# wq2012/SpectralCluster

Hardware: AMD Instinct MI355X
Metric: predict() calls/sec, n=8192 d=256 ICASSP2018 (GraphCut, eigengap k in [2,20], cosine k-means) (higher is better)
Workload: dtype f64; 1 GPU; icassp2018_graphcut_n8192_d256_k8_max20; n_samples=8192, n_features=256, parallelism=replicas x1, collectives=none

## Files before the change

### spectralcluster_amd/csrc/api.hip

```cpp
#include <algorithm>
#include <array>
#include <cmath>
#include <cstdio>
#include <cstdlib>
#include <cstring>
#include <vector>

#include <condition_variable>
#include <mutex>
#include <string>
#include <thread>

#include "handle.h"
#include "host_pool.h"

int ensure_matrices(sc_handle h, int n, int d, bool affinity_copy) {
  h->krylov_m = 0;
  const size_t ldn = matrix_ld(n);
  const size_t nn = (size_t)n * ldn * sizeof(double);
  if (affinity_copy) SC_TRY(grow(h, h->A0, nn));
  SC_TRY(grow(h, h->B1, nn));
  SC_TRY(grow(h, h->B2, nn));
  if (d > 0) {
    const size_t ldx = round_up(d, 16);
    SC_TRY(grow(h, h->X, (size_t)n * ldx * sizeof(double)));
    SC_TRY(grow(h, h->Xn, (size_t)n * ldx * sizeof(double)));
  }
  const size_t nv = (size_t)round_up(n, 16) * sizeof(double);
  SC_TRY(grow(h, h->rowmax, nv));
  SC_TRY(grow(h, h->rowsum, nv));
  SC_TRY(grow(h, h->cvec, nv));
  SC_TRY(grow(h, h->pvec, nv));
  SC_TRY(grow(h, h->tvec, nv));
  SC_TRY(grow(h, h->deg, nv));
  SC_TRY(grow(h, h->splitk, gemm_splitk_workspace_bytes()));
  SC_TRY(grow(h, h->dvec, nv));
  SC_TRY(grow(h, h->cut, nv));
  SC_TRY(grow(h, h->cropval, nv));
  SC_TRY(grow(h, h->statp, (size_t)2 * n * gemm_tile_dim(n) * sizeof(double)));
  SC_TRY(grow(h, h->rmpart, (size_t)n * blur_tile_columns(n, 8) * sizeof(double)));
  SC_TRY(grow(h, h->blurw, (2 * SC_MAX_BLUR_RADIUS + 1) * sizeof(double)));
  return SC_OK;
}

int ensure_tilemap(sc_handle h, int n) {
  const int nt = gemm_tile_dim(n);
  if (nt <= kTilemapTableMax) {
    if (!h->tilemap_table.p) {
      std::vector<int2> all, one;
      for (int t = 1; t <= kTilemapTableMax; ++t) {
        h->tilemap_off[t] = (int)all.size();
        gemm_build_sym_tilemap(t, &one);
        all.insert(all.end(), one.begin(), one.end());
      }
      SC_TRY(grow(h, h->tilemap_table, all.size() * sizeof(int2)));
      SC_HIP(h, hipMemcpyAsync(h->tilemap_table.p, all.data(), all.size() * sizeof(int2),
                               hipMemcpyHostToDevice, h->stream));
      SC_HIP(h, hipStreamSynchronize(h->stream));
    }
    h->tilemap_cur = ptr<int2>(h->tilemap_table) + h->tilemap_off[nt];
    return SC_OK;
  }
  if (h->tilemap_nt != nt) {
    std::vector<int2> map;
    gemm_build_sym_tilemap(nt, &map);
    SC_TRY(grow(h, h->tilemap, map.size() * sizeof(int2)));
    SC_HIP(h, hipMemcpyAsync(h->tilemap.p, map.data(), map.size() * sizeof(int2),
                             hipMemcpyHostToDevice, h->stream));
    SC_HIP(h, hipStreamSynchronize(h->stream));
    h->tilemap_nt = nt;
  }
  h->tilemap_cur = ptr<int2>(h->tilemap);
  return SC_OK;
}

int ensure_eig(sc_handle h, int n) {
  const size_t nq = (size_t)n * kLdq * sizeof(double);
  if (h->Q.bytes < nq) h->krylov_m = 0;
  SC_TRY(grow(h, h->Q, nq));
  SC_TRY(grow(h, h->Q2, nq));
  SC_TRY(grow(h, h->Vs, (size_t)n * kEigBlock * sizeof(double)));
  SC_TRY(grow(h, h->W, (size_t)n * kEigBlock * sizeof(double)));
  SC_TRY(grow(h, h->partial, std::max((size_t)kProjBlocks * kLdq * kEigBlock,
                                       lz_partial_doubles(n)) * sizeof(double)));
  SC_TRY(grow(h, h->T, (size_t)kLdq * kLdq * sizeof(double)));
  SC_TRY(grow(h, h->Y, (size_t)kLdq * kLdq * sizeof(double)));
  SC_TRY(grow(h, h->Yt, (size_t)kLdq * kLdq * sizeof(double)));
  SC_TRY(grow(h, h->theta, kLdq * sizeof(double)));
  SC_TRY(grow(h, h->resid, kLdq * sizeof(double)));
  SC_TRY(grow(h, h->G, 256 * sizeof(double)));
  SC_TRY(grow(h, h->Rinv, 256 * sizeof(double)));
  SC_TRY(grow(h, h->Hbuf, (size_t)kLdq * kEigBlock * sizeof(double)));
  SC_TRY(grow(h, h->hsq, 16 * sizeof(double)));
  SC_TRY(grow(h, h->colnorm, (size_t)kProjBlocks * kMaxVectors * sizeof(double)));
  if (h->flags.bytes < 16 * sizeof(int)) {
    SC_TRY(grow(h, h->flags, 16 * sizeof(int)));
    SC_HIP(h, hipMemsetAsync(h->flags.p, 0, 16 * sizeof(int), h->stream));
  }
  SC_TRY(grow(h, h->mvsym, matvec_sym_workspace_doubles(n) * sizeof(double)));
  SC_TRY(ensure_vectors(h, n, kMaxCols));
  return SC_OK;
}

int ensure_vectors(sc_handle h, int n, int cols) {
  cols = std::max(cols, kMaxCols);
  SC_TRY(grow(h, h->E, (size_t)round_up(n, 16) * cols * sizeof(double)));
  SC_TRY(grow(h, h->Eio, (size_t)n * cols * sizeof(double)));
  return SC_OK;
}

int ensure_gen(sc_handle h, int n) {
  const size_t ldv = round_up(n, 16);
  const size_t nv = ldv * sizeof(double);
  SC_TRY(grow(h, h->crvec, nv));
  SC_TRY(grow(h, h->thetai, kLdq * sizeof(double)));
  SC_TRY(grow(h, h->Vre, ldv * kGenMax * sizeof(double)));
  SC_TRY(grow(h, h->Vim, ldv * kGenMax * sizeof(double)));
  SC_TRY(grow(h, h->gpart, (size_t)gen_residual_blocks(n) * 32 * sizeof(double)));
  SC_TRY(grow(h, h->gsrc, 16 * sizeof(int)));
  SC_TRY(grow(h, h->genL, (size_t)kGenMax * kGenMax * sizeof(double)));
  return SC_OK;
}

extern "C" int sc_abi_version(void) { return SC_ABI_VERSION; }
extern "C" int sc_struct_sizes(int* config_bytes, int* diag_bytes) {
  if (config_bytes) *config_bytes = (int)sizeof(sc_config);
  if (diag_bytes) *diag_bytes = (int)sizeof(sc_diag);
  return SC_OK;
}

extern "C" int sc_device_count(void) {
  int c = 0;
  if (hipGetDeviceCount(&c) != hipSuccess) return 0;
  return c;
}

extern "C" int sc_device_info(int device, char* name, int name_len, char* arch,
                              int arch_len, int* compute_units,
                              int64_t* total_mem_bytes) {
  hipDeviceProp_t prop;
  if (hipGetDeviceProperties(&prop, device) != hipSuccess) return SC_ERR_HIP;
  if (name && name_len > 0) snprintf(name, name_len, "%s", prop.name);
  if (arch && arch_len > 0) snprintf(arch, arch_len, "%s", prop.gcnArchName);
  if (compute_units) *compute_units = prop.multiProcessorCount;
  if (total_mem_bytes) *total_mem_bytes = (int64_t)prop.totalGlobalMem;
  return SC_OK;
}


extern "C" int sc_create(int device, sc_handle* out) {
  if (!out) return SC_ERR_INVALID;
  *out = nullptr;
  int count = 0;
  if (hipGetDeviceCount(&count) != hipSuccess || count <= 0) return SC_ERR_HIP;
  if (device < 0 || device >= count) return SC_ERR_INVALID;
  sc_handle h = new sc_handle_s();
  h->device = device;
  if (hipSetDevice(device) != hipSuccess ||
      hipStreamCreateWithFlags(&h->stream, hipStreamNonBlocking) != hipSuccess) {
    delete h;
    return SC_ERR_HIP;
  }
  const unsigned ev_flags = hipEventDisableSystemFence;
  for (int i = 0; i < 48; ++i) {
    if (hipEventCreateWithFlags(&h->ev[i], ev_flags) != hipSuccess) {
      delete h;
      return SC_ERR_HIP;
    }
  }
  if (hipHostMalloc(reinterpret_cast<void**>(&h->h_theta), 3 * kLdq * sizeof(double)) !=
          hipSuccess ||
      hipHostMalloc(reinterpret_cast<void**>(&h->h_flags), 16 * sizeof(int)) !=
          hipSuccess ||
      hipHostMalloc(reinterpret_cast<void**>(&h->h_rr),
                    (2 * kHostRRSingle * kHostRRSingle + 64) * sizeof(double)) != hipSuccess) {
    delete h;
    return SC_ERR_HIP;
  }
  *out = h;
  return SC_OK;
}

extern "C" int sc_destroy(sc_handle h) {
  if (!h) return SC_OK;
  for (sc_handle sub : h->pool) sc_destroy(sub);
  h->pool.clear();
  for (sc_handle sub : h->gslots) sc_destroy(sub);
  h->gslots.clear();
  for (sc_handle sub : h->gshort) sc_destroy(sub);
  h->gshort.clear();
  hipSetDevice(h->device);
  hipStreamSynchronize(h->stream);
  DevBuf* bufs[] = {&h->X,     &h->Xn,    &h->A0,     &h->B1,      &h->B2,    &h->rowmax,
                    &h->rowsum, &h->cvec,  &h->pvec,   &h->tvec,    &h->deg,   &h->blurw, &h->blur_tmp, &h->dvec, &h->cut, &h->rmpart, &h->splitk, &h->tilemap, &h->tilemap_table, &h->cropval, &h->statp, &h->crvec, &h->thetai, &h->Vre, &h->Vim, &h->gpart, &h->gsrc, &h->genL, &h->ahc_size, &h->ahc_chain, &h->ahc_Z, &h->ahc_lab, &h->ahc_cent, &h->fb_part, &h->fb_small, &h->fb_x, &h->fb_cent, &h->fb_int, &h->Cq, &h->Cband, &h->cp[0], &h->cp[1], &h->cp[2], &h->cp[3], &h->cp[4], &h->symflag,
                    &h->Q,     &h->Q2,    &h->Vs,     &h->W,       &h->partial, &h->T,
                    &h->Y,     &h->Yt,    &h->theta,  &h->resid,   &h->G,     &h->Rinv,
                    &h->Hbuf,  &h->hsq,   &h->colnorm, &h->flags,  &h->E,     &h->Ek,   &h->Eio,
                    &h->td_d,  &h->td_e,  &h->td_theta, &h->td_work, &h->td_tau, &h->td_panel, &h->mvsym,
                    &h->kXc,   &h->kxsq,  &h->kclosest, &h->kcand, &h->kenorm, &h->krnd,
                    &h->kcent, &h->klab32, &h->klab64, &h->kinfo, &h->kchain, &h->gkrnd, &h->gpack, &h->gypack, &h->ginfo, &h->glabels, &h->gjtab,
                    &h->kbig, &h->kbigw, &h->fq, &h->ft32, &h->fy1, &h->fR, &h->fscal, &h->fwords, &h->fcand, &h->fY, &h->fsplit, &h->fypart, &h->frpart, &h->fq2part, &h->fmx64, &h->ftau64, &h->fplan, &h->Xalt, &h->Xstage, &h->gneg};
  for (DevBuf* b : bufs)
    if (b->p) hipFree(b->p);
  for (DevBuf& b : h->kgen)
    if (b.p) hipFree(b.p);
  for (int i = 0; i < 48; ++i) hipEventDestroy(h->ev[i]);
  if (h->h_theta) hipHostFree(h->h_theta);
  if (h->h_flags) hipHostFree(h->h_flags);
  if (h->h_rr) hipHostFree(h->h_rr);
  if (h->h_free) hipHostFree(h->h_free);
  if (h->sync_ev) hipEventDestroy(h->sync_ev);
  for (int b = 0; b < kGroupBanks; ++b) {
    if (h->gbank_ev[b]) hipEventDestroy(h->gbank_ev[b]);
    if (h->gbank_stream[b]) hipStreamDestroy(h->gbank_stream[b]);
  }
  if (h->gchain_stream) hipStreamDestroy(h->gchain_stream);
  if (h->copy_stream) hipStreamDestroy(h->copy_stream);
  if (h->gcheck_ev) hipEventDestroy(h->gcheck_ev);
  for (sc_handle lane : h->glanes) sc_destroy(lane);
  h->glanes.clear();
  delete h->gpool;
  if (h->h_gpack) hipHostFree(h->h_gpack);
  if (h->h_gypack) hipHostFree(h->h_gypack);
  if (h->h_gjtab) hipHostFree(h->h_gjtab);
  if (h->h_ginfo) hipHostFree(h->h_ginfo);
  if (h->h_glabels) hipHostFree(h->h_glabels);
  hipStreamDestroy(h->stream);
  delete h;
  return SC_OK;
}

extern "C" const char* sc_last_error(sc_handle h) { return h ? h->err.c_str() : ""; }

extern "C" int sc_synchronize(sc_handle h) {
  if (!h) return SC_ERR_INVALID;
  SC_HIP(h, hipStreamSynchronize(h->stream));
  return SC_OK;
}

extern "C" int sc_reserve(sc_handle h, int n_max, int d_max) {
  if (!h || n_max <= 0 || d_max < 0) return SC_ERR_INVALID;
  SC_HIP(h, hipSetDevice(h->device));
  SC_TRY(ensure_matrices(h, n_max, d_max));
  SC_TRY(ensure_eig(h, n_max));
  SC_TRY(ensure_kmeans(h, n_max));
  return SC_OK;
}

static double numpy_sum_short(const double* a, int n) {
  if (n < 8) {
    double r = 0.0;
    for (int i = 0; i < n; ++i) r += a[i];
    return r;
  }
  double r[8];
  for (int j = 0; j < 8; ++j) r[j] = a[j];
  int i = 8;
  for (; i < n - (n % 8); i += 8)
    for (int j = 0; j < 8; ++j) r[j] += a[i + j];
  double res = ((r[0] + r[1]) + (r[2] + r[3])) + ((r[4] + r[5]) + (r[6] + r[7]));
  for (; i < n; ++i) res += a[i];
  return res;
}

extern "C" int sc_gaussian_weights(double sigma, int32_t* radius, double* weights) {
  if (!radius || !weights || !(sigma >= 0.0)) return SC_ERR_INVALID;
  if (sigma <= 1e-15) {
    *radius = 0;
    weights[0] = 1.0;
    return SC_OK;
  }
  const int r = (int)(4.0 * sigma + 0.5);
  if (r > SC_MAX_BLUR_RADIUS) return SC_ERR_UNSUPPORTED;
  const double s2 = sigma * sigma;
  for (int x = -r; x <= r; ++x) weights[x + r] = std::exp(-0.5 / s2 * (double)(x * x));
  const double sum = numpy_sum_short(weights, 2 * r + 1);
  for (int i = 0; i < 2 * r + 1; ++i) weights[i] /= sum;
  *radius = r;
  return SC_OK;
}

extern "C" int sc_set_blur_weights(sc_handle h, int radius, const double* weights) {
  if (!h) return SC_ERR_INVALID;
  if (radius <= SC_MAX_BLUR_RADIUS || radius > (1 << 20) || !weights)
    return fail(h, SC_ERR_INVALID, "sc_set_blur_weights: radius must exceed 32; weights 2 r + 1");
  h->blur_ext.assign(weights, weights + 2 * (size_t)radius + 1);
  return SC_OK;
}

extern "C" int sc_config_default(sc_config* cfg) {
  if (!cfg) return SC_ERR_INVALID;
  memset(cfg, 0, sizeof(*cfg));
  sc_gaussian_weights(1.0, &cfg->blur_radius, cfg->blur_weights);
  cfg->p_percentile = 0.95;
  cfg->soft_multiplier = 0.01;
  cfg->threshold_type = SC_THRESHOLD_ROW_MAX;
  cfg->symmetrize_type = SC_SYMMETRIZE_MAX;
  cfg->laplacian_type = SC_LAPLACIAN_NONE;
  cfg->stop_eigenvalue = 1e-2;
  cfg->eigengap_type = SC_EIGENGAP_RATIO;
  cfg->max_iter = 300;
  cfg->constraint_name = SC_CONSTRAINT_NONE;
  cfg->integration_type = SC_INTEGRATION_MAX;
  cfg->constraint_alpha = 0.6;
  return SC_OK;
}

void eigengap_core(const double* w, int count, int max_clusters,
                          double stop_eigenvalue, int eigengap_type, int descend,
// ... 214 lines not shown
  launch_normalize_rows(h->stream, ptr<double>(h->X), h->ldx, h->n, h->d,
                        ptr<double>(h->Xn), ptr<int>(h->symflag) + 1);
  h->affinity_from_embeddings = true;
  GemmRowStats rs{2, ptr<double>(h->statp), nullptr, ptr<double>(h->cropval), nullptr};
  h->aff_ev[0] = h->aff_ev[1] = -1;
  if (h->profile_level >= 1) ev_rec(h, &h->aff_ev[0]);
  launch_gemm_nt(h->stream, ptr<double>(h->Xn), h->ldx, ptr<double>(h->Xn), h->ldx,
                 ptr<double>(h->A0), h->ldn, h->n, h->n, h->d, kEpiAffinity, true,
                 ptr<double>(h->splitk), h->tilemap_cur, &rs);
  if (h->profile_level >= 1) ev_rec(h, &h->aff_ev[1]);
  SC_TRY(check_last(h, "affinity launch"));
  h->have_affinity = true;
  h->have_cropval = true;
  h->affinity_symmetric = true;
  h->constraint_applied = false;
  h->n_vec = 0;
  h->sweep_slot.clear();
  return SC_OK;
}

extern "C" int sc_set_affinity(sc_handle h, const double* a, int n) {
  if (!h) return SC_ERR_INVALID;
  if (!a || n <= 0) return fail(h, SC_ERR_INVALID, "affinity must be (n, n)");
  SC_HIP(h, hipSetDevice(h->device));
  SC_TRY(ensure_matrices(h, n, 0));
  h->n = n;
  h->ldn = matrix_ld(n);
  h->have_x = false;
  h->n_vec = 0;
  h->sweep_slot.clear();
  SC_TRY(h2d_matrix(h, a, n, n, ptr<double>(h->A0), h->ldn));
  SC_TRY(device_is_symmetric(h, ptr<double>(h->A0), n, h->ldn, &h->affinity_symmetric));
  h->have_affinity = true;
  h->have_cropval = false;
  h->constraint_applied = false;
  h->affinity_from_embeddings = false;
  return SC_OK;
}


EigRequest make_eig_request(const sc_config* cfg) {
  EigRequest rq;
  rq.descend = (cfg->laplacian_type == SC_LAPLACIAN_NONE ||
                cfg->laplacian_type == SC_LAPLACIAN_AFFINITY);
  rq.max_clusters = cfg->max_clusters;
  rq.min_clusters = cfg->min_clusters;
  rq.stop_eigenvalue = cfg->stop_eigenvalue;
  rq.eigengap_type = cfg->eigengap_type;
  rq.use_stop = rq.descend;
  rq.value_tol = cfg->eig_value_tol > 0 ? cfg->eig_value_tol : 1e-6;
  rq.vector_tol = cfg->eig_vector_tol > 0 ? cfg->eig_vector_tol : 1e-10;
  rq.max_cycles = cfg->eig_max_cycles > 0 ? cfg->eig_max_cycles : (cfg->eig_max_cycles < 0 ? 0 : 40);
  rq.fixed_count = 0;
  return rq;
}

static void resolve_stage_times(sc_handle h, sc_diag* diag) {
  StageEvents& t = h->stage_events;
  if (!t.pending) return;
  t.pending = false;
  if (!diag) return;
  float dms = 0.f;
  for (int i = 0; i < t.n_diffuse; ++i) dms += ev_ms(h, t.diffuse[i][0], t.diffuse[i][1]);
  diag->stage_ms[SC_STAGE_DIFFUSE] = dms;
  diag->stage_ms[SC_STAGE_REFINE] = ev_ms(h, t.begin, t.after_refine) - dms;
  diag->stage_ms[SC_STAGE_SCALING] = ev_ms(h, t.after_refine, t.after_scaling);
  diag->stage_ms[SC_STAGE_EIG] = ev_ms(h, t.after_scaling, t.after_eig);
  if (t.free_path) {
    diag->stage_ms[SC_STAGE_FREE_QUANTIZE] = ev_ms(h, h->free_ev[0], h->free_ev[1]);
    diag->stage_ms[SC_STAGE_FREE_PRODUCT] = ev_ms(h, h->free_ev[1], h->free_ev[2]);
    diag->stage_ms[SC_STAGE_FREE_SCAN] = ev_ms(h, h->free_ev[2], h->free_ev[3]);
    diag->stage_ms[SC_STAGE_FREE_STATS] = ev_ms(h, h->free_ev[3], h->free_ev[4]);
  }
  if (t.fine) {
    diag->stage_ms[SC_STAGE_BLUR] = ev_ms(h, t.blur[0], t.blur[1]);
    diag->stage_ms[SC_STAGE_THRESHOLD_SYM] = ev_ms(h, t.thr[0], t.thr[1]);
    float mv = 0.f;
    for (int i = 0; i < h->n_mv_ev; ++i) mv += ev_ms(h, h->mv_ev[i][0], h->mv_ev[i][1]);
    diag->stage_ms[SC_STAGE_MATVEC] = mv;
  }
}

int eig_ncluster_impl(sc_handle h, const sc_config* cfg, sc_diag* diag, FrontResult* front_only,
                      const FrontResult* resume, bool defer_timing) {
  const int n = h->n, ld = h->ldn;
  hipStream_t s = h->stream;
  const double* cur = ptr<double>(h->A0);
  double* bufs[2] = {ptr<double>(h->B1), ptr<double>(h->B2)};
  int which = 0;
  bool symmetric = h->affinity_symmetric;
  const bool constrain_after = constraint_active(h, cfg, false);
  bool folded_rownorm = false;
  int e_begin, e_after_refine;
  const bool fine = h->profile_level >= 2;
  int eb0 = -1, eb1 = -1, et0 = -1, et1 = -1;
  h->n_mv_ev = 0;
  bool free_path = false;
  const double* amax_of = nullptr;
  const double* digits_of = nullptr;
  float diffuse_ms_events[SC_MAX_OPS][2];
  int n_diffuse = 0;
  ev_rec(h, &e_begin);
  const bool blur_fast = (cfg->blur_radius == 4 || cfg->blur_radius == 8) && n >= 128;
  const double* pending_diag = nullptr;
  bool have_partials = false;
  bool have_row_stats = false;
  if (resume) {
    cur = resume->matrix;
    symmetric = resume->symmetric;
    folded_rownorm = resume->folded_rownorm;
    which = resume->scratch == bufs[0] ? 0 : 1;
    if (resume->free_op) h->free_checked = false;
  }
  for (int i = 0; i < (resume ? 0 : cfg->n_ops); ++i) {
    const int op = cfg->ops[i];
    const int next = i + 1 < cfg->n_ops ? cfg->ops[i + 1] : 0;
    const int next2 = i + 2 < cfg->n_ops ? cfg->ops[i + 2] : 0;
    const bool thr_sym_fusable = true;
    const bool partials_usable = cfg->threshold_type == SC_THRESHOLD_ROW_MAX &&
                                 !cfg->preserve_diagonal;
    if (op == SC_OP_ROW_WISE_NORMALIZE && symmetric && i == cfg->n_ops - 1 &&
        !constrain_after) {
      folded_rownorm = true;
      continue;
    }
    if (op == SC_OP_CROP_DIAGONAL && next == SC_OP_GAUSSIAN_BLUR && blur_fast) {
      if (cur == ptr<double>(h->A0) && h->have_cropval) {
        pending_diag = ptr<double>(h->cropval);
      } else {
        launch_crop_value(s, cur, n, ld, ptr<double>(h->dvec));
        pending_diag = ptr<double>(h->dvec);
      }
      have_partials = false;
      continue;
    }
    double* out = bufs[which];
    which ^= 1;
    int e0 = -1, e1 = -1;
    bool keep_cur = false;
    if (op == SC_OP_DIFFUSE) ev_rec(h, &e0);
    if (op == SC_OP_GAUSSIAN_BLUR && blur_fast) {
      const bool want = next == SC_OP_ROW_WISE_THRESHOLD && next2 == SC_OP_SYMMETRIZE &&
                        partials_usable;
      SC_TRY(upload_blur_weights(h, cfg));
      if (fine) ev_rec(h, &eb0);
      have_partials = launch_gaussian_blur_fused(s, cur, out, n, ld, cfg->blur_radius,
                                                 ptr<double>(h->blurw), pending_diag,
                                                 want ? ptr<double>(h->rmpart) : nullptr);
      if (fine) ev_rec(h, &eb1);
      pending_diag = nullptr;
      SC_TRY(check_last(h, "blur launch"));
    } else if (op == SC_OP_ROW_WISE_THRESHOLD && next == SC_OP_SYMMETRIZE && thr_sym_fusable) {
      if (cfg->threshold_type == SC_THRESHOLD_PERCENTILE)
        launch_cut_percentile(s, cur, n, ld, cfg->p_percentile, ptr<double>(h->cut),
                              cfg->preserve_diagonal);
      else if (have_partials && partials_usable)
        launch_cut_from_partials(s, ptr<double>(h->rmpart), n,
                                 blur_tile_columns(n, cfg->blur_radius),
                                 cfg->p_percentile, ptr<double>(h->cut));
      else
        launch_cut_from_rows(s, cur, n, ld, cfg->p_percentile, ptr<double>(h->cut),
                             cfg->preserve_diagonal);
      const bool amax_known =
          cfg->threshold_type == SC_THRESHOLD_ROW_MAX && h->affinity_from_embeddings &&
          !h->constraint_applied && cfg->p_percentile > 0.0 && cfg->soft_multiplier >= 0.0 &&
          cfg->soft_multiplier <= 1.0 && i + 2 < cfg->n_ops && cfg->ops[i + 2] == SC_OP_DIFFUSE &&
          free_diffuse_wanted(h, cfg, n, make_eig_request(cfg));
      const bool fuse_digits =
          amax_known && !constrain_after && !front_only &&
          (i + 2 == cfg->n_ops - 1 ||
           (i + 2 == cfg->n_ops - 2 && cfg->ops[i + 3] == SC_OP_ROW_WISE_NORMALIZE));
      const double amax_floor = (cfg->binarize || cfg->preserve_diagonal) ? 1.0 : 0.0;
      if (fuse_digits)
        SC_TRY(free_fused_prepare(h, s, n, ptr<double>(h->cut), cfg->p_percentile, amax_floor));
      if (fine) ev_rec(h, &et0);
      if (fuse_digits)
        launch_threshold_symmetrize_digits(s, cur, out, n, ld, ptr<double>(h->cut),
                                           cfg->soft_multiplier, cfg->binarize,
                                           cfg->symmetrize_type, cfg->preserve_diagonal,
                                           ptr<signed char>(h->fq), ptr<double>(h->fscal),
                                           ptr<double>(h->fypart), ptr<int>(h->frpart),
                                           ptr<double>(h->fq2part), ptr<double>(h->fmx64));
      else
        launch_threshold_symmetrize(s, cur, out, n, ld, ptr<double>(h->cut),
                                    cfg->soft_multiplier, cfg->binarize, cfg->symmetrize_type,
                                    cfg->preserve_diagonal);
      if (fine) ev_rec(h, &et1);
      SC_TRY(check_last(h, "threshold+symmetrize launch"));
      if (fuse_digits) {
        amax_of = out;
        digits_of = out;
      } else if (amax_known) {
        SC_TRY(ensure_free(h, n));
        launch_free_amax_from_cut(s, ptr<double>(h->cut), n, cfg->p_percentile, amax_floor,
                                  ptr<double>(h->fscal));
        amax_of = out;
      }
      have_partials = false;
      cur = out;
      symmetric = true;
      ++i;
      continue;
    } else if (op == SC_OP_DIFFUSE && symmetric && !constrain_after && !front_only &&
               cur != ptr<double>(h->A0) &&
               (i == cfg->n_ops - 1 || (i == cfg->n_ops - 2 && next == SC_OP_ROW_WISE_NORMALIZE)) &&
               free_diffuse_wanted(h, cfg, n, make_eig_request(cfg))) {
      SC_TRY(ensure_eig(h, n));
      SC_TRY(free_diffuse_stats(h, cur, ld, n, amax_of == cur, digits_of == cur));
      free_path = true;
      have_row_stats = true;
      have_partials = false;
      keep_cur = true;
      which ^= 1;
    } else if (op == SC_OP_DIFFUSE) {
      const bool last = i == cfg->n_ops - 1 ||
                        (i == cfg->n_ops - 2 && next == SC_OP_ROW_WISE_NORMALIZE);
      GemmRowStats rs{1, ptr<double>(h->statp), ptr<double>(h->statp) + (size_t)n * gemm_tile_dim(n),
                      ptr<double>(h->rowmax), ptr<double>(h->rowsum)};
      SC_TRY(ensure_tilemap(h, n));
      launch_gemm_nt(s, cur, ld, cur, ld, out, ld, n, n, n, kEpiNone, true,
                     ptr<double>(h->splitk), h->tilemap_cur, last ? &rs : nullptr);
      SC_TRY(check_last(h, "diffuse launch"));
      have_row_stats = last;
      have_partials = false;
    } else {
      SC_TRY(run_refine_op(h, op, cfg, cur, out, n, ld));
      have_partials = false;
    }
    if (op == SC_OP_DIFFUSE) {
      ev_rec(h, &e1);
      diffuse_ms_events[n_diffuse][0] = (float)e0;
      diffuse_ms_events[n_diffuse][1] = (float)e1;
      ++n_diffuse;
    }
    if (!keep_cur) cur = out;
    switch (op) {
      case SC_OP_CROP_DIAGONAL:
      case SC_OP_GAUSSIAN_BLUR:
        break;
      case SC_OP_ROW_WISE_THRESHOLD:
      case SC_OP_ROW_WISE_NORMALIZE:
        symmetric = false;
        break;
      case SC_OP_SYMMETRIZE:
      case SC_OP_DIFFUSE:
        symmetric = true;
        break;
    }
  }
  if (constrain_after && !resume) {
    if (h->qn != n)
      return fail(h, SC_ERR_INVALID,
                  "affinity and constraint matrix must have the same shape");
    double* out = bufs[which];
    which ^= 1;
    SC_TRY(adjust_affinity(h, cfg, cur, symmetric, out, n, ld));
    cur = out;
    symmetric = symmetric && h->constraint_symmetric;
    have_row_stats = false;
  }
  ev_rec(h, &e_after_refine);
  bool flags_by_kernel = false;
  if (resume) {
    SC_TRY(ensure_eig(h, n));
  } else if (!symmetric) {
    SC_TRY(ensure_gen(h, n));
    launch_row_stats(s, cur, n, ld, ptr<double>(h->rowmax), ptr<double>(h->deg));
    launch_scaling_general(s, ptr<double>(h->deg), n, cfg->laplacian_type,
                           ptr<double>(h->cvec), ptr<double>(h->crvec), ptr<double>(h->pvec));
  } else {
    if (!have_row_stats)
      launch_row_stats(s, cur, n, ld, ptr<double>(h->rowmax), ptr<double>(h->rowsum));
    SC_TRY(ensure_eig(h, n));
    launch_scaling_vectors(s, ptr<double>(h->rowmax), ptr<double>(h->rowsum), n,
                           cfg->laplacian_type, folded_rownorm ? 1 : 0, ptr<double>(h->cvec),
                           ptr<double>(h->pvec), ptr<double>(h->tvec), ptr<int>(h->flags),
                           h->affinity_from_embeddings ? ptr<int>(h->symflag) : nullptr);
    flags_by_kernel = true;
  }
  SC_TRY(ensure_eig(h, n));
  if (flags_by_kernel) {
  } else if (h->affinity_from_embeddings)
    SC_HIP(h, hipMemcpyAsync(ptr<int>(h->flags) + 12, ptr<int>(h->symflag) + 1, sizeof(int),
                             hipMemcpyDeviceToDevice, s));
  else
    SC_HIP(h, hipMemsetAsync(ptr<int>(h->flags) + 12, 0, sizeof(int), s));
  launch_check_finite(s, ptr<double>(h->cvec), ptr<double>(h->pvec), n, ptr<int>(h->flags) + 12);
  if (front_only && !flags_by_kernel)
    SC_HIP(h, hipMemsetAsync(ptr<int>(h->flags) + 13, 0, 3 * sizeof(int), s));
  SC_TRY(check_last(h, "scaling launch"));
  if (sw::eig_trace() > 2 && symmetric) {
    std::vector<double> rm(n), rs(n);
    hipMemcpyAsync(rm.data(), h->rowmax.p, n * sizeof(double), hipMemcpyDeviceToHost, s);
    hipMemcpyAsync(rs.data(), h->rowsum.p, n * sizeof(double), hipMemcpyDeviceToHost, s);
    hipStreamSynchronize(s);
    int imin = 0, imax = 0;
    for (int i = 0; i < n; ++i) {
      if (rm[i] < rm[imin]) imin = i;
      if (rm[i] > rm[imax]) imax = i;
    }
    fprintf(stderr, "[sc] scaling: fused stats %d; rowmax min %.6g at %d, max %.6g at %d; "
            "rowsum[%d] %.6g\n", (int)have_row_stats, rm[imin], imin, rm[imax], imax, imin,
            rs[imin]);
  }
  int e_after_scaling;
  ev_rec(h, &e_after_scaling);
  FrontResult op;
  op.matrix = cur;
  op.scratch = bufs[which];
  op.ld = ld;
  op.symmetric = symmetric;
  op.folded_rownorm = folded_rownorm;
  op.free_op = free_path || (resume && resume->free_op);
  op.laplacian_type = cfg->laplacian_type;
  op.chain_flags_cleared = flags_by_kernel;
  op.skip_fused = resume && resume->skip_fused;
  if (front_only) {
    *front_only = op;
    return SC_OK;
  }
  EigRequest rq = make_eig_request(cfg);
  EigDecision dc;
  std::vector<double> w;
  if (symmetric) {
    SC_TRY(sym_topk(h, op, n, rq, diag, &dc, &w));
  } else {
    rq.decision_aware = 1;
    SC_TRY(gen_topk(h, cur, ld, n, cfg->laplacian_type, rq, diag, &dc, &w, bufs[which]));
  }
  int e_after_eig;
  ev_rec(h, &e_after_eig);
  h->last_w = w;
  if (diag) {
    diag->n = n;
    diag->n_clusters_raw = dc.n_clusters_raw;
    diag->max_delta = dc.max_delta;
    diag->eig_descending = rq.descend;
    diag->n_eigenvalues = std::min((int)w.size(), SC_MAX_EIG);
    for (int i = 0; i < diag->n_eigenvalues; ++i) diag->eigenvalues[i] = w[i];
    diag->symmetry_state = !symmetric ? 3 : (folded_rownorm ? 2 : 1);
    if (!free_path && n_diffuse > 0) diag->diffuse_path = SC_DIFFUSE_PATH_EXPLICIT;
  }
  StageEvents& t = h->stage_events;
  t.pending = true;
  t.begin = e_begin;
  t.after_refine = e_after_refine;
  t.after_scaling = e_after_scaling;
  t.after_eig = e_after_eig;
  t.n_diffuse = n_diffuse;
  for (int i = 0; i < n_diffuse; ++i) {
    t.diffuse[i][0] = (int)diffuse_ms_events[i][0];
    t.diffuse[i][1] = (int)diffuse_ms_events[i][1];
  }
  t.fine = fine;
  t.free_path = free_path;
  t.blur[0] = eb0;
  t.blur[1] = eb1;
  t.thr[0] = et0;
  t.thr[1] = et1;
  if (defer_timing) return SC_OK;
  SC_HIP(h, hipStreamSynchronize(s));
  resolve_stage_times(h, diag);
  return SC_OK;
}

extern "C" int sc_eig_ncluster(sc_handle h, const sc_config* cfg, sc_diag* diag) {
  if (!h) return SC_ERR_INVALID;
  SC_TRY(validate_config(h, cfg));
  if (!h->have_affinity) return fail(h, SC_ERR_INVALID, "no affinity resident");
  SC_HIP(h, hipSetDevice(h->device));
  h->nev = 0;
  if (diag) memset(diag, 0, sizeof(*diag));
  return eig_ncluster_impl(h, cfg, diag, nullptr);
}

extern "C" int sc_num_eigenvectors(sc_handle h) { return h ? h->n_vec : 0; }

extern "C" int sc_num_eigenvalues(sc_handle h) { return h ? (int)h->last_w.size() : 0; }

extern "C" int sc_get_eigenvalues(sc_handle h, double* out, int count) {
  if (!h || !out) return SC_ERR_INVALID;
  if (count < 0 || count > (int)h->last_w.size())
    return fail(h, SC_ERR_INVALID, "eigenvalue request out of range");
  for (int i = 0; i < count; ++i) out[i] = h->last_w[i];
  return SC_OK;
}

extern "C" int sc_get_eigenvectors(sc_handle h, double* out, int n, int ncols) {
  if (!h || !out) return SC_ERR_INVALID;
  if (n != h->n || ncols <= 0 || ncols > h->n_vec)
    return fail(h, SC_ERR_INVALID, "eigenvector request out of range");
  SC_HIP(h, hipSetDevice(h->device));
  launch_colmajor_to_rowmajor(h->stream, ptr<double>(h->E), round_up(n, 16), n, ncols,
                              ptr<double>(h->Eio), ncols);
  return d2h_matrix(h, ptr<double>(h->Eio), ncols, n, ncols, out);
}

extern "C" int sc_run_resident(sc_handle h, const sc_config* cfg, int64_t* labels,
                               sc_diag* diag) {
  if (!h) return SC_ERR_INVALID;
  SC_TRY(validate_config(h, cfg));
  if (!labels) return fail(h, SC_ERR_INVALID, "labels is NULL");
  if (!h->have_x) return fail(h, SC_ERR_INVALID, "no embeddings resident");
  SC_HIP(h, hipSetDevice(h->device));
  sc_diag local;
  sc_diag* dg = diag ? diag : &local;
  memset(dg, 0, sizeof(*dg));
  h->nev = 0;
  int e0, e1, e2;
  ev_rec(h, &e0);
  SC_TRY(sc_compute_affinity(h));
  if (constraint_active(h, cfg, true)) SC_TRY(sc_apply_constraint(h, cfg));
  ev_rec(h, &e1);
  SC_TRY(eig_ncluster_impl(h, cfg, dg, nullptr, nullptr, true));
  int k = dg->n_clusters_raw;
  if (cfg->min_clusters > 0 && k < cfg->min_clusters) k = cfg->min_clusters;
  const int rc_cluster = sc_cluster(h, cfg, k, labels, dg);
  if (rc_cluster != SC_OK) {
    h->stage_events.pending = false;
    return rc_cluster;
  }
  ev_rec(h, &e2);
  SC_HIP(h, hipStreamSynchronize(h->stream));
  resolve_stage_times(h, dg);
  dg->stage_ms[SC_STAGE_AFFINITY] = ev_ms(h, e0, e1);
  dg->stage_ms[SC_STAGE_TOTAL] = ev_ms(h, e0, e2);
  if (h->profile_level >= 1)
    dg->stage_ms[SC_STAGE_AFFINITY_GEMM] = ev_ms(h, h->aff_ev[0], h->aff_ev[1]);
  return SC_OK;
}

extern "C" int sc_set_profiling(sc_handle h, int level) {
  if (!h || level < 0 || level > 2) return SC_ERR_INVALID;
  h->profile_level = level;
  return SC_OK;
}

std::vector<sc_array> host_f64_arrays(const double* const* xs, const int* ns, int d, int count) {
  std::vector<sc_array> arrays(std::max(count, 0));
  for (int i = 0; i < count; ++i) arrays[i] = host_f64_array(xs[i], ns[i], d);
  return arrays;
}

int predict_sequence(sc_handle h, const int* idx, int count, const sc_array* xs,
                     const int* ns, int d, const sc_config* cfg, int64_t* const* labels,
                     sc_diag* diags) {
  auto at = [&](int k) { return idx ? idx[k] : k; };
  auto one_call = [&](int i) -> int {
    SC_TRY(validate_config(h, cfg));
    SC_HIP(h, hipSetDevice(h->device));
    h->sweep_slot.clear();
    SC_TRY(ingest_embeddings(h, xs[i], xs[i].location == SC_MEM_HOST));
    return sc_run_resident(h, cfg, labels[i], diags ? diags + i : nullptr);
  };
  int nmax = 0;
  size_t smallest = ~(size_t)0;
  bool prefetchable = true;
  for (int k = 0; k < count; ++k) {
    const int i = at(k);
    if (!xs[i].data || ns[i] <= 0 || d <= 0) { smallest = 0; continue; }
    nmax = std::max(nmax, ns[i]);
    smallest = std::min(smallest, (size_t)ns[i] * d * sizeof(double));
    prefetchable = prefetchable && array_is_host_f64_rows(xs[i]);
  }
  if (nmax > 0) SC_TRY(sc_reserve(h, nmax, d));
  if (count < 2 || smallest < ((size_t)256 << 10) || !prefetchable) {
    for (int k = 0; k < count; ++k) SC_TRY(one_call(at(k)));
    return SC_OK;
  }
  SC_TRY(validate_config(h, cfg));
  SC_HIP(h, hipSetDevice(h->device));
  const size_t ldx = round_up(d, 16);
  SC_TRY(grow(h, h->Xalt, (size_t)nmax * ldx * sizeof(double)));
  SC_TRY(grow(h, h->X, (size_t)nmax * ldx * sizeof(double)));
  if (!h->copy_stream)
    SC_HIP(h, hipStreamCreateWithFlags(&h->copy_stream, hipStreamNonBlocking));
  const DevBuf slot[2] = {h->X, h->Xalt};
  std::mutex mu;
  std::condition_variable cv;
  int uploaded = 0;
  int finished = 0;
  bool stop = false;
  hipError_t upload_err = hipSuccess;
  auto upload_loop = [&]() {
    hipSetDevice(h->device);
    for (int k = 0; k < count; ++k) {
      {
        std::unique_lock<std::mutex> lock(mu);
        cv.wait(lock, [&] { return stop || finished >= k - 1; });
        if (stop) return;
      }
      const int i = at(k);
      hipError_t e = hipMemcpy2DAsync(slot[k & 1].p, ldx * sizeof(double), xs[i].data,
                                      (size_t)(ns[i] == 1 ? d : xs[i].row_stride) * sizeof(double),
                                      (size_t)d * sizeof(double), ns[i], hipMemcpyHostToDevice,
                                      h->copy_stream);
      if (e == hipSuccess) e = hipStreamSynchronize(h->copy_stream);
// ... 328 lines not shown
```

### spectralcluster_amd/csrc/eig.hip

```cpp
#include <algorithm>
#include <cstring>
#include <mutex>

#include "sc_internal.h"

namespace sc {

typedef double v4f64 __attribute__((ext_vector_type(4)));
constexpr int B = kEigBlock;
constexpr int RB = 256 / B;
static_assert(B == 8 || B == 16, "block width must divide the 16-wide MFMA tile");

__device__ __forceinline__ uint64_t splitmix64(uint64_t x) {
  x += 0x9E3779B97F4A7C15ull;
  x = (x ^ (x >> 30)) * 0xBF58476D1CE4E5B9ull;
  x = (x ^ (x >> 27)) * 0x94D049BB133111EBull;
  return x ^ (x >> 31);
}
__device__ __forceinline__ double hash_uniform(uint64_t seed, uint64_t idx) {
  const uint64_t h = splitmix64(seed ^ splitmix64(idx));
  return (double)(h >> 11) * (2.0 / 9007199254740992.0) - 1.0;
}

__global__ void k_random_block(double* W, int n, uint64_t seed) {
// ... 527 lines not shown
  double* Ql = smem;
  double* Hl = Ql + ROWS * mq;
  double* Rl = Hl + kLdq * B;
  double* Wl = Rl + B * B;
  double* Gs = Wl + ROWS * B;
  double* hs = Gs + B * B;
  const int tid = threadIdx.x;
  const int j = tid % B;
  const int r0 = blockIdx.x * ROWS;
  const bool first_wg = blockIdx.x == 0;
  const bool pre_proj = (a.pre >= 1 && a.pre <= 3) && m > 0;
  const bool pre_gram = a.pre >= 2;
  const bool use_h = pre_proj;
  const bool use_r = pre_gram;
  const bool use_q = m > 0 && (use_h || a.want_proj);
  const int nproj = pre_proj ? m * B : 0;
  double hsum[3] = {0.0, 0.0, 0.0};
#pragma unroll
  for (int u = 0; u < 3; ++u) {
    const int e = tid + u * kLzThreads;
    if (e < nproj) hsum[u] = lz_ordered_sum(a.pre_partial + e, a.pre_nparts);
    else if (pre_gram && e < nproj + B * B)
      hsum[u] = lz_ordered_sum(a.pre_partial + kLdq * B + (e - nproj), a.pre_nparts);
  }
  double told[3] = {0.0, 0.0, 0.0};
  double hsq_old = 0.0;
  if (first_wg && a.pre == 2) {
#pragma unroll
    for (int u = 0; u < 3; ++u) {
      const int e = tid + u * kLzThreads;
      if (e < nproj) told[u] = a.T[(size_t)(e / B) * a.ldt + a.col0 + (e % B)];
    }
    if (tid < B) hsq_old = a.hsq[tid];
  }
  if (!first_wg && a.pre == 2 && tid < B) hsq_old = a.hsq[tid];
  if (use_q)
    for (int e = tid; e < ROWS * m; e += kLzThreads) {
      const int rr = e / m, i = e - rr * m;
      Ql[rr * mq + i] = (r0 + rr < a.n) ? a.Q[(size_t)(r0 + rr) * a.ldq + i] : 0.0;
    }
  double w[ROWS / kPass];
#pragma unroll
  for (int q = 0; q < ROWS / kPass; ++q) {
    const int r = r0 + q * kPass + tid / B;
    w[q] = 0.0;
    if (r < a.n)
      w[q] = a.init_random ? hash_uniform(a.seed, (uint64_t)r * B + j) : a.W[(size_t)r * B + j];
  }
#pragma unroll
  for (int u = 0; u < 3; ++u) {
    const int e = tid + u * kLzThreads;
    if (e < nproj) Hl[e] = hsum[u];
    else if (pre_gram && e < nproj + B * B) Gs[e - nproj] = hsum[u];
  }
  if (tid < B * B) Rl[tid] = (tid / B == tid % B) ? 1.0 : 0.0;
  __syncthreads();
  if (pre_proj && a.pre != 3) {
    if (first_wg && a.T != nullptr) {
#pragma unroll
      for (int u = 0; u < 3; ++u) {
        const int e = tid + u * kLzThreads;
        if (e < nproj) {
          const int i = e / B, jc = a.col0 + (e % B);
          if (i <= jc) {
            const double t = a.pre == 2 ? told[u] + hsum[u] : hsum[u];
            a.T[(size_t)i * a.ldt + jc] = t;
            a.T[(size_t)jc * a.ldt + i] = t;
          }
        }
      }
    }
    if (tid < B) {
      double sq = 0.0;
      for (int i = 0; i < m; ++i) sq = __builtin_fma(Hl[i * B + tid], Hl[i * B + tid], sq);
      sq = a.pre == 2 ? hsq_old + sq : sq;
      if (first_wg && a.pre == 1) a.hsq[tid] = sq;
      hs[tid] = sq;
    }
  } else if (tid < B) {
    hs[tid] = 0.0;
  }
  if (first_wg && a.Tzero != nullptr)
    for (int e = tid; e < kLdq * kLdq; e += kLzThreads) a.Tzero[e] = 0.0;
  if (pre_gram) {
    if (pre_proj && tid < B * B) {
      const int a1 = tid / B, b1 = tid % B;
      double g = Gs[tid];
      for (int i = 0; i < m; ++i) g = __builtin_fma(-Hl[i * B + a1], Hl[i * B + b1], g);
      Gs[tid] = g;
    }
    __syncthreads();
    if (first_wg && a.pre == 2 && a.Gsave != nullptr && tid < B * B) a.Gsave[tid] = Gs[tid];
    if (tid < 64)
      chol8_wave(Gs, Rl, a.pre == 2 ? hs : nullptr, first_wg ? a.flags : nullptr,
                 first_wg ? a.flags + (a.pre == 3 ? 10 : 11) : nullptr, a.pre == 3 ? 2 : 1,
                 first_wg ? a.flags + 13 : nullptr, m, a.arm_defect != 0);
    __syncthreads();
  }
#pragma unroll
  for (int q = 0; q < ROWS / kPass; ++q) {
    const int rl = q * kPass + tid / B;
    const int r = r0 + rl;
    double x = w[q];
    if (use_h)
      for (int i = 0; i < m; ++i) x = __builtin_fma(-Ql[rl * mq + i], Hl[i * B + j], x);
    double v = x;
    if (use_r) {
      v = 0.0;
#pragma unroll
      for (int k = 0; k < B; ++k) v = __builtin_fma(__shfl(x, k, B), Rl[k * B + j], v);
    }
    if (r < a.n) {
      a.W[(size_t)r * B + j] = v;
      if (a.Qdst) a.Qdst[(size_t)r * a.ldq + a.store_col + j] = v;
      if (a.Vs) a.Vs[(size_t)r * B + j] = a.vs_scale[r] * v;
    }
    Wl[rl * B + j] = (r < a.n) ? v : 0.0;
  }
  if (!a.want_proj && !a.want_gram) return;
  __syncthreads();
  const int oproj = a.want_proj ? m * B : 0;
  const int nent = oproj + (a.want_gram ? B * B : 0);
  double* mine = a.partial + (size_t)blockIdx.x * kLzPartStride;
  for (int base = 0; base < nent; base += kLzThreads / 2) {
    const int e = base + (tid >> 1), half = tid & 1;
    double acc = 0.0;
    if (e < nent) {
      const int rbeg = half * (ROWS / 2);
      if (e < oproj) {
        const int i = e / B, jj = e % B;
#pragma unroll 8
        for (int rr = 0; rr < ROWS / 2; ++rr)
          acc = __builtin_fma(Ql[(rbeg + rr) * mq + i], Wl[(rbeg + rr) * B + jj], acc);
      } else {
        const int g = e - oproj, a1 = g / B, b1 = g % B;
#pragma unroll 8
        for (int rr = 0; rr < ROWS / 2; ++rr)
          acc = __builtin_fma(Wl[(rbeg + rr) * B + a1], Wl[(rbeg + rr) * B + b1], acc);
      }
    }
    const double other = __shfl_xor(acc, 1);
    if (e < nent && half == 0)
      mine[e < oproj ? e : kLdq * B + (e - oproj)] = acc + other;
  }
}
template <int ROWS>
__global__ __launch_bounds__(kLzThreads) void k_lz_rows(const LzStep a) {
  lz_rows_body<ROWS>(a);
}
template <int ROWS>
__global__ __launch_bounds__(kLzThreads) void k_lz_rows_g(const GroupOf<LzStep> g) {
  const LzStep& a = g.s[blockIdx.y];
  if ((int)blockIdx.x * ROWS >= a.n) return;
  lz_rows_body<ROWS>(a);
}

__device__ __forceinline__ double fast_rcp(double x) {
  double r = __builtin_amdgcn_rcp(x);
  r = __builtin_fma(r, __builtin_fma(-x, r, 1.0), r);
  r = __builtin_fma(r, __builtin_fma(-x, r, 1.0), r);
  return r;
}
__device__ __forceinline__ double fast_rsqrt(double x) {
  double y = __builtin_amdgcn_rsq(x);
  y = __builtin_fma(y, 0.5 * __builtin_fma(-x * y, y, 1.0), y);
  y = __builtin_fma(y, 0.5 * __builtin_fma(-x * y, y, 1.0), y);
// ... 670 lines not shown
```

### spectralcluster_amd/csrc/eig_driver.hip

```cpp
#include <ctime>

#include "handle.h"
#include "host_eig.h"
#include "host_pool.h"


static double value_error_bound(const double* theta, const double* resid, int m, int i,
                                bool symmetric) {
  const double r = resid[i];
  if (!symmetric || !(r > 0.0) || !std::isfinite(r)) return r;
  double delta = __builtin_huge_val();
  if (i > 0) delta = std::min(delta, theta[i - 1] - resid[i - 1] - theta[i]);
  if (i + 1 < m) delta = std::min(delta, theta[i] - theta[i + 1] - resid[i + 1]);
  else return r;
  delta -= r;
  if (!(delta > 0.0) || !std::isfinite(delta)) return r;
  return std::min(r, 2.0 * r * r / delta);
}

extern "C" int sc_host_value_error_bound(const double* theta, const double* resid, int m, int i,
                                         double* bound) {
  if (!theta || !resid || !bound || m < 1 || i < 0 || i >= m) return SC_ERR_INVALID;
  *bound = value_error_bound(theta, resid, m, i, true);
  return SC_OK;
// ... 274 lines not shown

static int dense_spectrum(sc_handle h, const double* S, int ld, int n, double* scratch) {
  hipStream_t s = h->stream;
  if (scratch == nullptr || scratch == S)
    return fail(h, SC_ERR_UNSUPPORTED, "no scratch matrix for the dense eigenvalue path");
  SC_TRY(grow(h, h->td_d, (size_t)n * sizeof(double)));
  SC_TRY(grow(h, h->td_e, (size_t)n * sizeof(double)));
  SC_TRY(grow(h, h->td_theta, (size_t)n * sizeof(double)));
  SC_TRY(grow(h, h->td_work, (size_t)(5 * (size_t)n + 2048) * sizeof(double)));
  SC_TRY(grow(h, h->td_tau, (size_t)n * sizeof(double)));
  SC_TRY(grow(h, h->td_panel, (size_t)n * 128 * sizeof(double)));
  launch_td_materialize(s, S, ld, n, ptr<double>(h->cvec), ptr<double>(h->pvec), scratch);
  launch_tridiagonalize_blocked(s, scratch, ld, n, ptr<double>(h->td_d), ptr<double>(h->td_e),
                                ptr<double>(h->td_tau), ptr<double>(h->td_panel),
                                ptr<double>(h->td_work), ptr<double>(h->splitk));
  launch_tridiagonal_eigenvalues(s, ptr<double>(h->td_d), ptr<double>(h->td_e), n,
                                 ptr<double>(h->td_theta), ptr<double>(h->td_work));
  SC_TRY(check_last(h, "dense eigenvalue launch"));
  h->spectrum.resize(n);
  SC_HIP(h, hipMemcpyAsync(h->spectrum.data(), h->td_theta.p, (size_t)n * sizeof(double),
                           hipMemcpyDeviceToHost, s));
  SC_HIP(h, hipMemcpyAsync(h->h_flags + 12, ptr<int>(h->flags) + 12, sizeof(int),
                           hipMemcpyDeviceToHost, s));
  SC_HIP(h, hipStreamSynchronize(s));
  if (h->h_flags[12] != 0) return fail(h, SC_ERR_NON_FINITE, kNonFiniteMessage);
  for (int i = 0; i < n; ++i)
    if (!std::isfinite(h->spectrum[i])) return fail(h, SC_ERR_NON_FINITE, kNonFiniteMessage);
  return SC_OK;
}

static int dense_vectors(sc_handle h, const double* scratch, int ld, int n, int cols) {
  hipStream_t s = h->stream;
  if (cols < 1 || cols > n)
    return fail(h, SC_ERR_UNSUPPORTED, "dense eigenvector request out of range");
  SC_TRY(ensure_vectors(h, n, cols));
  std::vector<double> de(2 * (size_t)n);
  SC_HIP(h, hipMemcpyAsync(de.data(), h->td_d.p, (size_t)n * sizeof(double),
                           hipMemcpyDeviceToHost, s));
  SC_HIP(h, hipMemcpyAsync(de.data() + n, h->td_e.p, (size_t)n * sizeof(double),
                           hipMemcpyDeviceToHost, s));
  SC_HIP(h, hipStreamSynchronize(s));
  const int lde = round_up(n, 16);
  std::vector<double> z((size_t)lde * cols, 0.0);
  if (!host_tridiag_eigvectors(de.data(), de.data() + n, n, h->spectrum.data(), cols, z.data(),
                               (size_t)lde))
    return fail(h, SC_ERR_NOT_CONVERGED, "inverse iteration on the tridiagonal form failed");
  SC_HIP(h, hipMemcpyAsync(h->E.p, z.data(), z.size() * sizeof(double), hipMemcpyHostToDevice,
                           s));
  launch_td_backtransform(s, scratch, ld, n, ptr<double>(h->td_tau), ptr<double>(h->E), lde,
                          cols);
  back_transform_cols(h, n, cols);
  SC_TRY(check_last(h, "dense eigenvector launch"));
  SC_HIP(h, hipStreamSynchronize(s));
  h->n_vec = cols;
  return SC_OK;
}

bool wants_full_spectrum(const EigRequest& rq) {
  if (rq.fixed_count > 0 || rq.descend) return false;
  return rq.max_clusters == 0 || rq.eigengap_type == SC_EIGENGAP_NORMALIZED_DIFF;
}

static EigWorkspace eig_workspace(sc_handle h) {
  EigWorkspace ws;
  ws.Q = ptr<double>(h->Q);
  ws.Q2 = ptr<double>(h->Q2);
  ws.Vs = ptr<double>(h->Vs);
  ws.W = ptr<double>(h->W);
  ws.partial = ptr<double>(h->partial);
  ws.T = ptr<double>(h->T);
  ws.Y = ptr<double>(h->Y);
  ws.theta = ptr<double>(h->theta);
  ws.resid = ptr<double>(h->resid);
  ws.G = ptr<double>(h->G);
  ws.Rinv = ptr<double>(h->Rinv);
  ws.Hbuf = ptr<double>(h->Hbuf);
  ws.hsq = ptr<double>(h->hsq);
  ws.Yt = ptr<double>(h->Yt);
  ws.colnorm = ptr<double>(h->colnorm);
  ws.flags = ptr<int>(h->flags);
  return ws;
}

int sym_topk(sc_handle h, const FrontResult& op_in, int n, const EigRequest& rq_in,
             sc_diag* diag, EigDecision* out_dc, std::vector<double>* out_w) {
  hipStream_t s = h->stream;
  h->krylov_m = 0;
  SC_TRY(ensure_eig(h, n));
  FrontResult op = op_in;
  const int ld = op.ld;
  auto free_materialize = [&](bool with_stats) -> int {
    if (!op.free_op) return SC_OK;
    if (op.scratch == nullptr || op.scratch == op.matrix)
      return fail(h, SC_ERR_UNSUPPORTED, "no scratch matrix to form the Diffuse product in");
    SC_TRY(ensure_tilemap(h, n));
    GemmRowStats rs{1, ptr<double>(h->statp), ptr<double>(h->statp) + (size_t)n * gemm_tile_dim(n),
                    ptr<double>(h->rowmax), ptr<double>(h->rowsum)};
    launch_gemm_nt(s, op.matrix, ld, op.matrix, ld, op.scratch, ld, n, n, n, kEpiNone, true,
                   ptr<double>(h->splitk), h->tilemap_cur, with_stats ? &rs : nullptr);
    SC_TRY(check_last(h, "diffuse launch"));
    double* a_buffer = const_cast<double*>(op.matrix);
    op.matrix = op.scratch;
    op.scratch = a_buffer;
    op.free_op = false;
    return SC_OK;
  };
  auto free_check = [&](bool* restart) -> int {
    *restart = false;
    if (!op.free_op || h->free_checked) return SC_OK;
    bool changed = false, too_many = false;
    SC_TRY(free_fix_overflow(h, op.matrix, ld, n, &changed, &too_many));
    if (too_many) {
      SC_TRY(free_materialize(true));
      changed = true;
    }
    if (changed) {
      launch_scaling_vectors(s, ptr<double>(h->rowmax), ptr<double>(h->rowsum), n,
                             op.laplacian_type, op.folded_rownorm ? 1 : 0, ptr<double>(h->cvec),
                             ptr<double>(h->pvec), ptr<double>(h->tvec));
      launch_check_finite(s, ptr<double>(h->cvec), ptr<double>(h->pvec), n, ptr<int>(h->flags) + 12);
      SC_TRY(check_last(h, "scaling launch"));
      *restart = true;
    }
    return SC_OK;
  };
  double* theta_d = ptr<double>(h->theta);
  double* resid_d = ptr<double>(h->resid);
  const double* cvec = ptr<double>(h->cvec);
  const double* pvec = ptr<double>(h->pvec);
  EigDecision dc;
  int m = 0, passes = 0, cycles = 0;
  EigRequest rq = rq_in;
  bool fused = !sw::eig_host_chain() && !op.skip_fused;
  bool three_pass = false;
  const int sym_min_n = sw::matvec_sym_min_n();
  const bool sym_mv = n >= sym_min_n;
  EigDecision dense_dc;
  bool dense = false, many_vectors = false;
  auto run_dense = [&]() -> int {
    bool unused = false;
    SC_TRY(free_check(&unused));
    SC_TRY(free_materialize(false));
    SC_TRY(dense_spectrum(h, op.matrix, ld, n, op.scratch));
    std::vector<double> zeros(n, 0.0);
    dense_dc = analyze(rq_in, h->spectrum.data(), zeros.data(), n, n, true);
    if (!dense_dc.enough) return fail(h, SC_ERR_UNSUPPORTED, "eigen request cannot be satisfied");
    many_vectors = dense_dc.kvec > kMaxVectors;
    dense = true;
    rq = rq_in;
    rq.fixed_count = std::max(1, dense_dc.kvec);
    rq.value_tol = std::max(rq_in.value_tol, 1e-6);
    return SC_OK;
  };
  if (n > kDenseMax && wants_full_spectrum(rq_in)) SC_TRY(run_dense());
  bool vectors_from_dense = false;
  int fallback_reason = 0;
  auto dense_fallback = [&](int reason) -> int {
    if (op.scratch == nullptr || op.scratch == op.matrix)
      return fail(h, SC_ERR_NOT_CONVERGED,
                  "block Lanczos did not converge and no scratch matrix is free for the dense path");
    if (sw::eig_trace())
      fprintf(stderr, "[sc] block Lanczos gave up (reason %d, %d passes): dense path\n", reason,
              passes);
    if (!dense) SC_TRY(run_dense());
    SC_TRY(free_materialize(false));
    int cols = dense_dc.kvec;
    if (rq_in.fixed_count > 0 || rq_in.max_clusters > 0)
      cols = std::max(std::min(dense_dc.kw, kMaxVectors), cols);
    cols = std::max(1, cols);
    SC_TRY(dense_vectors(h, op.scratch, ld, n, cols));
    vectors_from_dense = true;
    fallback_reason = reason;
    return SC_OK;
  };

  if (n <= kDenseMax) {
    launch_jacobi(s, op.matrix, ld, n, 1, cvec, pvec, nullptr, theta_d, ptr<double>(h->Y), kLdq,
                  nullptr, ptr<double>(h->Yt), ptr<int>(h->flags));
    SC_TRY(check_last(h, "jacobi launch"));
    SC_HIP(h, hipMemcpyAsync(h->h_theta, theta_d, n * sizeof(double), hipMemcpyDeviceToHost, s));
    SC_HIP(h, hipMemcpyAsync(h->h_flags + 12, ptr<int>(h->flags) + 12, sizeof(int),
                             hipMemcpyDeviceToHost, s));
    if (sw::eig_trace())
      SC_HIP(h, hipMemcpyAsync(h->h_flags + 1, ptr<int>(h->flags) + 1, 7 * sizeof(int),
                               hipMemcpyDeviceToHost, s));
    SC_HIP(h, hipStreamSynchronize(s));
    if (h->h_flags[12] != 0) return fail(h, SC_ERR_NON_FINITE, kNonFiniteMessage);
    trace_jacobi(h);
    for (int i = 0; i < n; ++i) h->h_theta[kLdq + i] = 0.0;
    dc = analyze(rq, h->h_theta, h->h_theta + kLdq, n, n, true);
    if (!dc.enough) return fail(h, SC_ERR_UNSUPPORTED, "eigen request cannot be satisfied");
    m = n;
    const int cols = n;
    launch_rowmajor_to_colmajor(s, ptr<double>(h->Y), kLdq, n, cols, ptr<double>(h->E),
                                round_up(n, 16));
    back_transform_cols(h, n, cols);
    h->n_vec = cols;
    if (diag) diag->eig_path = SC_EIG_PATH_DENSE_JACOBI;
    dc.kw = n;
  } else {
  restart_lanczos:
    m = 0;
    cycles = 0;
    bool done = false;
    uint64_t seed = 0x5eed5eedull;
    LzChain chain;
    if (dense && many_vectors) {
      SC_TRY(dense_fallback(5));
      done = true;
    }
    if (done) {
    } else if (fused) {
      if (!op.chain_flags_cleared)
        SC_HIP(h, hipMemsetAsync(ptr<int>(h->flags) + 13, 0, 3 * sizeof(int), s));
      op.chain_flags_cleared = false;
      const EigWorkspace ws = eig_workspace(h);
      chain = LzChain();
      chain.three_pass = three_pass;
      launch_lz_link(s, ws, &chain, n, 0, 0, 4, -1, cvec, 0, true, seed, false);
      launch_lz_link(s, ws, &chain, n, 0, 4, 3, -1, cvec, 0, false, 0, true);
      launch_lz_link(s, ws, &chain, n, 0, 3, 0, 0, cvec, 0, false, 0, false);
      SC_TRY(check_last(h, "start block launch"));
    } else {
      launch_random_block(s, ptr<double>(h->W), n, seed);
      SC_TRY(orthonormalize(h, n, 0, false, 0, 0, false, cvec));
      const int rc0 = finish_block(h, n, 0, 0, cvec, &seed);
      if (rc0 == SC_ERR_NOT_CONVERGED) {
        SC_TRY(dense_fallback(3));
        done = true;
      } else {
        SC_TRY(rc0);
      }
      SC_HIP(h, hipMemsetAsync(h->T.p, 0, (size_t)kLdq * kLdq * sizeof(double), s));
    }
    if (!done && sw::eig_force_dense()) {
      SC_TRY(dense_fallback(4));
      done = true;
    }
    const int cap = std::min(kEigBasisCap, ((n - kEigBlock) / kEigBlock) * kEigBlock);
    const int first_check = std::min(3 * kEigBlock, cap);
    auto check_due = [&](int mm) {
      return cycles == 0 ? (mm >= first_check && (mm <= 4 * kEigBlock ||
                                                  mm % (2 * kEigBlock) == 0 || mm + kEigBlock > cap))
                         : (mm + kEigBlock > cap);
    };
    auto enqueue_step = [&](int m_before) -> int {
      const bool time_mv = h->profile_level >= 2 && h->n_mv_ev < 16;
      if (time_mv) ev_rec(h, &h->mv_ev[h->n_mv_ev][0]);
      if (op.free_op)
        free_apply_operator(h, op.matrix, ld, n, sym_mv, ptr<double>(h->Q) + m_before, kLdq);
      else if (sym_mv)
        launch_block_matvec_sym(s, op.matrix, ld, n, cvec, pvec, ptr<double>(h->Q) + m_before, kLdq,
                                ptr<double>(h->Vs), ptr<double>(h->W), ptr<double>(h->mvsym));
      else
        launch_block_matvec(s, op.matrix, ld, n, cvec, pvec, ptr<double>(h->Q) + m_before, kLdq,
                            ptr<double>(h->Vs), ptr<double>(h->W));
      if (time_mv) ev_rec(h, &h->mv_ev[h->n_mv_ev++][1]);
      ++passes;
      const int mm = m_before + kEigBlock;
      if (fused) {
        const EigWorkspace ws = eig_workspace(h);
        launch_lz_link(s, ws, &chain, n, mm, 0, 1, -1, cvec, mm - kEigBlock, false, 0, false);
        launch_lz_link(s, ws, &chain, n, mm, 1, 2, -1, cvec, mm - kEigBlock, false, 0, false);
        launch_lz_link(s, ws, &chain, n, mm, 2, 3, -1, cvec, mm - kEigBlock, false, 0, false);
        if (three_pass) launch_lz_link(s, ws, &chain, n, mm, 3, 3, -1, cvec, 0, false, 0, false);
        launch_lz_link(s, ws, &chain, n, mm, 3, 0, mm, cvec, 0, false, 0, false);
        return check_last(h, "block step launch");
      }
      return orthonormalize(h, n, mm, true, mm - kEigBlock, mm, true, cvec);
    };
    int ahead = 0;
    while (!done) {
      if (ahead > 0)
        --ahead;
      else
        SC_TRY(enqueue_step(m));
      m += kEigBlock;
      const bool check = check_due(m);
      const bool host_rr = check && m <= kHostRRSingle && !sw::eig_device_rr();
      if (host_rr) {
        SC_HIP(h, hipMemcpy2DAsync(h->h_rr, (size_t)m * sizeof(double), h->T.p,
                                   (size_t)kLdq * sizeof(double), (size_t)m * sizeof(double), m,
                                   hipMemcpyDeviceToHost, s));
        SC_HIP(h, hipMemcpyAsync(h->h_rr + kHostRRSingle * kHostRRSingle, h->G.p,
                                 kEigBlock * kEigBlock * sizeof(double), hipMemcpyDeviceToHost,
                                 s));
      } else if (check) {
        launch_jacobi(s, ptr<double>(h->T), kLdq, m, 0, nullptr, nullptr, ptr<double>(h->G),
                      theta_d, ptr<double>(h->Y), kLdq, resid_d, ptr<double>(h->Yt),
                      ptr<int>(h->flags));
        SC_TRY(check_last(h, "jacobi launch"));
        SC_HIP(h, hipMemcpyAsync(h->h_theta, theta_d, m * sizeof(double),
                                 hipMemcpyDeviceToHost, s));
        SC_HIP(h, hipMemcpyAsync(h->h_theta + kLdq, resid_d, m * sizeof(double),
                                 hipMemcpyDeviceToHost, s));
      }
      if (!fused) {
        const int rcb = finish_block(h, n, m, m, cvec, &seed);
        if (rcb == SC_ERR_NOT_CONVERGED) {
          SC_TRY(dense_fallback(3));
          break;
        }
        SC_TRY(rcb);
      } else if (check) {
        SC_HIP(h, hipMemcpyAsync(h->h_flags, h->flags.p, 16 * sizeof(int), hipMemcpyDeviceToHost, s));
        if (!h->sync_ev) SC_HIP(h, hipEventCreateWithFlags(&h->sync_ev, hipEventDisableTiming));
        SC_HIP(h, hipEventRecord(h->sync_ev, s));
        if (host_rr && cycles == 0 && m >= 6 * kEigBlock && m + kEigBlock <= cap) {
          int mm = m;
          do {
            SC_TRY(enqueue_step(mm));
            mm += kEigBlock;
            ++ahead;
          } while (!check_due(mm));
        }
        SC_HIP(h, hipEventSynchronize(h->sync_ev));
        if (h->h_flags[12] != 0) return fail(h, SC_ERR_NON_FINITE, kNonFiniteMessage);
        if (h->h_flags[13] != 0) {
          passes = 0;
          if (!three_pass && h->h_flags[15] == 2000) {
            if (sw::eig_trace())
              fprintf(stderr, "[sc] fused chain flagged at m=%d: three-pass chain\n",
                      h->h_flags[14]);
            three_pass = true;
            goto restart_lanczos;
          }
          if (sw::eig_trace()) fprintf(stderr, "[sc] fused chain flagged: host chain\n");
          fused = false;
          goto restart_lanczos;
        }
      }
      if (op.free_op && !h->free_checked && (!fused || check)) {
        bool restart = false;
        SC_TRY(free_check(&restart));
        if (restart) {
          if (sw::eig_trace())
            fprintf(stderr, "[sc] matrix-free diffuse: %d rows evaluated in full, restart\n",
                    h->h_free[0]);
          passes = 0;
          goto restart_lanczos;
        }
      }
      if (host_rr) {
        double* hy = h->h_rr + kHostRRSingle * kHostRRSingle + 64;
        const double* hG = h->h_rr + kHostRRSingle * kHostRRSingle;
        bool rr_ok;
        timespec ts0;
        if (sw::eig_trace()) clock_gettime(CLOCK_MONOTONIC, &ts0);
        if (m <= kHostRR) {
          rr_ok = host_rayleigh_ritz(h->h_rr, m, hG, m, h->h_theta, h->h_theta + kLdq, hy, m);
        } else {
          auto leading = [&](const double* theta) {
            std::vector<double> zero(m, 0.0);
            const EigDecision d0 = analyze(rq, theta, zero.data(), m, n, false);
            const int want = d0.enough ? std::max(d0.kw, d0.kvec) : cap / 4;
            return round_up(want + kEigBlock, kEigBlock) + kEigBlock;
          };
          rr_ok = host_rayleigh_ritz_leading(h->h_rr, m, hG, m, h->h_theta, h->h_theta + kLdq,
                                             hy, m, leading);
        }
        if (sw::eig_trace()) {
          timespec ts1;
          clock_gettime(CLOCK_MONOTONIC, &ts1);
          fprintf(stderr, "[sc]   host Rayleigh-Ritz m=%d: %.0f us\n", m,
                  (ts1.tv_sec - ts0.tv_sec) * 1e6 + (ts1.tv_nsec - ts0.tv_nsec) * 1e-3);
        }
        if (!rr_ok) {
          SC_TRY(dense_fallback(2));
          break;
        }
        for (int i = 0; i < m; ++i)
          if (!std::isfinite(h->h_theta[i])) return fail(h, SC_ERR_NON_FINITE, kNonFiniteMessage);
        SC_HIP(h, hipMemcpy2DAsync(h->Y.p, (size_t)kLdq * sizeof(double), hy,
                                   (size_t)m * sizeof(double), (size_t)m * sizeof(double), m,
                                   hipMemcpyHostToDevice, s));
        SC_HIP(h, hipMemcpyAsync(theta_d, h->h_theta, m * sizeof(double),
                                 hipMemcpyHostToDevice, s));
      }
      if (check) {
        dc = analyze(rq, h->h_theta, h->h_theta + kLdq, m, n, false);
        if (sw::eig_trace()) {
          int worst = 0;
          double wr = 0.0;
          for (int i = 0; i < std::min(m, dc.kw > 0 ? dc.kw : m); ++i) {
            const double r = h->h_theta[kLdq + i] / std::max(std::fabs(h->h_theta[i]), 1e-300);
            if (r > wr) { wr = r; worst = i; }
          }
          fprintf(stderr, "[sc] lanczos pass %d m=%d cycle %d: enough=%d conv=%d kw=%d kvec=%d "
                  "fail kind %d at %d (theta %.6g resid %.2e); far end theta=%.6g resid=%.2e\n",
                  passes, m, cycles, dc.enough, dc.converged, dc.kw, dc.kvec, dc.fail_kind,
                  dc.fail_index, dc.fail_index >= 0 ? h->h_theta[dc.fail_index] : 0.0,
                  dc.fail_index >= 0 ? h->h_theta[kLdq + dc.fail_index] : 0.0, h->h_theta[m - 1],
                  h->h_theta[kLdq + m - 1]);
          (void)wr; (void)worst;
        }
        if (dc.unsupported) {
          if (dense) return fail(h, SC_ERR_UNSUPPORTED, "eigen request cannot be satisfied");
          SC_TRY(run_dense());
          goto restart_lanczos;
        }
        if (dc.enough && dc.converged) {
          if (!dense && m < n && block_multiplicity_suspect(rq, dc, h->h_theta, m)) {
            if (sw::eig_trace())
              fprintf(stderr, "[sc] %d equal Ritz values ahead of the decisive gap: dense path\n",
                      kEigBlock);
            SC_TRY(dense_fallback(7));
            break;
          }
          done = true;
          break;
        }
      }
      if (m + kEigBlock > cap) {
        if (++cycles > rq.max_cycles) {
          SC_TRY(dense_fallback(1));
          break;
        }
        int want = dc.enough ? std::max(dc.kw, dc.kvec) : cap / 4;
        int keep = round_up(want + kEigBlock, kEigBlock);
        keep = std::max(kEigBlock, std::min(keep, cap - 2 * kEigBlock));
        launch_basis_times_Y(s, ptr<double>(h->Q), kLdq, m, ptr<double>(h->Y), kLdq, keep,
                             ptr<double>(h->Q2), kLdq, n, 0);
        launch_copy_block(s, ptr<double>(h->Q) + m, kLdq, ptr<double>(h->Q2) + keep, kLdq, n,
                          kEigBlock);
        std::swap(h->Q, h->Q2);
        launch_set_diag_T(s, ptr<double>(h->T), kLdq, kLdq, theta_d, keep);
        SC_TRY(check_last(h, "restart launch"));
        m = keep;
      }
    }
    if (ahead > 0) passes -= ahead;
    if (vectors_from_dense) {
      dc.max_resid = 0.0;
      if (diag) diag->eig_path = SC_EIG_PATH_DENSE_FULL;
    } else {
      const int cols = std::min(std::max(dc.kw, dc.kvec), kMaxVectors);
      launch_basis_times_Y(s, ptr<double>(h->Q), kLdq, m, ptr<double>(h->Y), kLdq, cols,
                           ptr<double>(h->E), round_up(n, 16), n, 1);
      back_transform_cols(h, n, cols);
      SC_TRY(check_last(h, "ritz vector launch"));
      h->n_vec = cols;
      if (diag) diag->eig_path = dense ? SC_EIG_PATH_DENSE_TRIDIAG : SC_EIG_PATH_BLOCK_LANCZOS;
      if (!dense) {
        h->krylov_m = m;
        h->krylov_n = n;
        h->krylov_cycles = cycles;
        h->krylov_ahead = ahead;
        h->krylov_free = op.free_op;
      }
    }
  }
  if (dense) {
    const double vec_resid = dc.max_resid;
    dc = dense_dc;
    dc.converged = true;
    dc.max_resid = vec_resid;
    if (out_w) {
      out_w->resize(n);
      for (int i = 0; i < n; ++i) (*out_w)[i] = rq.descend ? h->spectrum[i] : -h->spectrum[i];
// ... 497 lines not shown
  SC_HIP(h, hipMemsetAsync(h->td_tau.p, 0, (size_t)n * sizeof(double), s));
  launch_hessenberg(s, scratch, ld, n, ptr<double>(h->td_tau), ptr<double>(h->td_work));
  SC_TRY(check_last(h, "Hessenberg reduction launch"));
  std::vector<double> packed((size_t)n * ld), tau(n);
  SC_HIP(h, hipMemcpyAsync(packed.data(), scratch, packed.size() * sizeof(double),
                           hipMemcpyDeviceToHost, s));
  SC_HIP(h, hipMemcpyAsync(tau.data(), h->td_tau.p, (size_t)n * sizeof(double),
                           hipMemcpyDeviceToHost, s));
  SC_HIP(h, hipMemcpyAsync(h->h_flags + 12, ptr<int>(h->flags) + 12, sizeof(int),
                           hipMemcpyDeviceToHost, s));
  SC_HIP(h, hipStreamSynchronize(s));
  if (h->h_flags[12] != 0) return fail(h, SC_ERR_NON_FINITE, kNonFiniteMessage);
  const double t_reduced = sw::eig_trace() ? now_us() : 0.0;
  HostHessenberg hw;
  if (!host_hessenberg_unpack(packed.data(), (size_t)ld, n, tau.data(), &hw))
    return fail(h, SC_ERR_NON_FINITE, kNonFiniteMessage);
  packed.clear();
  packed.shrink_to_fit();
  std::vector<double> wr(n), wi(n);
  if (!host_hessenberg_eigenvalues(hw, wr.data(), wi.data()))
    return fail(h, SC_ERR_NOT_CONVERGED, "QR iteration on the Hessenberg form failed");
  const double t_values = sw::eig_trace() ? now_us() : 0.0;
  const double sign = is_lap ? -1.0 : 1.0;
  std::vector<int> order(n);
  for (int i = 0; i < n; ++i) order[i] = i;
  std::stable_sort(order.begin(), order.end(),
                   [&](int a, int b) { return sign * wr[a] > sign * wr[b]; });
  std::vector<double> theta(n), zeros(n, 0.0);
  for (int i = 0; i < n; ++i) theta[i] = sign * wr[order[i]] * eig_scale;
  EigDecision dc = analyze(rq, theta.data(), zeros.data(), n, n, true, false);
  if (!dc.enough) return fail(h, SC_ERR_UNSUPPORTED, "eigen request cannot be satisfied");
  const int cols = std::max(1, std::min(n, dc.kvec));
  SC_TRY(ensure_vectors(h, n, cols));
  const int ldv = round_up(n, 16);
  SC_TRY(grow(h, h->Vre, (size_t)ldv * std::max(cols, kGenMax) * sizeof(double)));
  SC_TRY(grow(h, h->Vim, (size_t)ldv * std::max(cols, kGenMax) * sizeof(double)));
  std::vector<double> pr(cols), pi(cols), vre((size_t)ldv * cols, 0.0), vim((size_t)ldv * cols, 0.0);
  for (int q = 0; q < cols; ++q) {
    pr[q] = wr[order[q]];
    pi[q] = wi[order[q]];
  }
  double max_resid = 0.0;
  if (!host_hessenberg_vectors(hw, pr.data(), pi.data(), cols, vre.data(), vim.data(), (size_t)ldv,
                               &max_resid))
    return fail(h, SC_ERR_NOT_CONVERGED, "inverse iteration on the Hessenberg form failed");
  SC_HIP(h, hipMemcpyAsync(h->Vre.p, vre.data(), vre.size() * sizeof(double), hipMemcpyHostToDevice, s));
  SC_HIP(h, hipMemcpyAsync(h->Vim.p, vim.data(), vim.size() * sizeof(double), hipMemcpyHostToDevice, s));
  launch_gen_phase(s, ptr<double>(h->Vre), ptr<double>(h->Vim), ldv, n, cols, ptr<double>(h->E), ldv);
  SC_TRY(check_last(h, "eigenvector normalisation launch"));
  SC_HIP(h, hipStreamSynchronize(s));
  if (sw::eig_trace())
    fprintf(stderr, "[sc] dense general route n=%d: Hessenberg reduction (device, incl. the copy "
            "back) %.1f ms, %d eigenvalues by QR (host) %.1f ms, %d eigenvectors by inverse "
            "iteration + back-transform (host) and phase (device) %.1f ms\n", n,
            (t_reduced - t_begin) * 1e-3, n, (t_values - t_reduced) * 1e-3, cols,
            (now_us() - t_values) * 1e-3);
  h->n_vec = cols;
  dc.kw = n;
  dc.converged = true;
  dc.max_resid = max_resid * std::max(hw.norm, 1e-300) * eig_scale;
  if (out_w) {
    out_w->resize(n);
    for (int i = 0; i < n; ++i) (*out_w)[i] = rq.descend ? theta[i] : -theta[i];
  }
  if (diag) {
    diag->eig_path = SC_EIG_PATH_DENSE_HESSENBERG;
    diag->eig_matvec_passes = 0;
    diag->eig_block = kEigBlock;
    diag->eig_basis = n;
    diag->eig_cycles = 0;
    diag->eig_max_residual = dc.max_resid;
    diag->eig_fallback = reason;
  }
  *out_dc = dc;
  return SC_OK;
}

int gen_topk(sc_handle h, const double* M, int ld, int n, int laplacian_type,
                    const EigRequest& rq_in, sc_diag* diag, EigDecision* out_dc,
                    std::vector<double>* out_w, double* scratch) {
  h->krylov_m = 0;
  EigRequest rq = rq_in;
  hipStream_t s = h->stream;
  SC_TRY(ensure_eig(h, n));
  SC_TRY(ensure_gen(h, n));
  double* theta_d = ptr<double>(h->theta);
  double* thetai_d = ptr<double>(h->thetai);
  double* resid_d = ptr<double>(h->resid);
  double* Yre = ptr<double>(h->Y);
  double* Yim = ptr<double>(h->Yt);
  double* Vre = ptr<double>(h->Vre);
  double* Vim = ptr<double>(h->Vim);
  int* info_d = ptr<int>(h->flags) + 8;
  const int ldv = round_up(n, 16);
  double* th = h->h_theta;
  double* thi = h->h_theta + 2 * kLdq;
  EigDecision dc;
  int m = 0, passes = 0, cycles = 0;
  const bool is_lap = laplacian_type >= SC_LAPLACIAN_UNNORMALIZED;
  bool far_end = !rq.descend && rq.eigengap_type == SC_EIGENGAP_NORMALIZED_DIFF &&
                 rq.fixed_count == 0;
  int far_passes = 0, far_cycles = 0;

  auto fetch_ritz = [&](int count) -> int {
    SC_HIP(h, hipMemcpyAsync(th, theta_d, count * sizeof(double), hipMemcpyDeviceToHost, s));
    SC_HIP(h, hipMemcpyAsync(thi, thetai_d, count * sizeof(double), hipMemcpyDeviceToHost, s));
    SC_HIP(h, hipMemcpyAsync(h->h_flags + 8, info_d, 2 * sizeof(int), hipMemcpyDeviceToHost, s));
    SC_HIP(h, hipMemcpyAsync(h->h_flags + 12, ptr<int>(h->flags) + 12, sizeof(int),
                             hipMemcpyDeviceToHost, s));
    SC_HIP(h, hipStreamSynchronize(s));
    if (h->h_flags[12] != 0) return fail(h, SC_ERR_NON_FINITE, kNonFiniteMessage);
    if (h->h_flags[8] != 0)
      return fail(h, SC_ERR_NOT_CONVERGED, "QR iteration of the projected eigenproblem failed");
    return SC_OK;
  };

  if (n <= kGenMax) {
    const double* src = M;
    if (is_lap) {
      launch_laplacian(s, M, ptr<double>(h->genL), n, ld, laplacian_type, ptr<double>(h->deg));
      src = ptr<double>(h->genL);
    }
    launch_gen_eig(s, src, ld, n, is_lap ? -1.0 : 1.0, n, theta_d, thetai_d, Yre, Yim, kLdq,
                   info_d);
    SC_TRY(check_last(h, "dense general eigensolver launch"));
    SC_TRY(fetch_ritz(n));
    for (int i = 0; i < n; ++i) th[kLdq + i] = 0.0;
    dc = analyze(rq, th, th + kLdq, n, n, true, false);
    if (!dc.enough) return fail(h, SC_ERR_UNSUPPORTED, "eigen request cannot be satisfied");
    launch_gen_ritz(s, nullptr, 0, n, n, Yre, Yim, kLdq, n, Vre, Vim, ldv);
    launch_gen_phase(s, Vre, Vim, ldv, n, n, ptr<double>(h->E), ldv);
    SC_TRY(check_last(h, "eigenvector normalisation launch"));
    h->n_vec = n;
    m = n;
    dc.kw = n;
    if (diag) diag->eig_path = SC_EIG_PATH_DENSE_GENERAL;
  } else {
    if (sw::eig_force_dense())
      return gen_dense_large(h, M, ld, n, laplacian_type, rq, diag, out_dc, out_w, scratch, 4);
    if (rq.fixed_count == 0 && n <= sw::gen_dense_max_n())
      return gen_dense_large(h, M, ld, n, laplacian_type, rq, diag, out_dc, out_w, scratch, 8);
    if (rq.fixed_count == 0 && rq.max_clusters == 0 && !rq.descend)
      return gen_dense_large(h, M, ld, n, laplacian_type, rq, diag, out_dc, out_w, scratch, 6);
    if (far_end) {
      EigRequest fr = rq;
      fr.fixed_count = 1;
      fr.descend = 1;
      fr.negate = !rq.negate;
      fr.no_dense = 1;
      fr.decision_aware = 0;
      fr.value_tol = 0.1 * rq.value_tol;
      fr.vector_tol = fr.value_tol;
      fr.max_cycles = std::max(rq.max_cycles, 60);
      EigDecision fdc;
      std::vector<double> fw;
      sc_diag fdiag;
      memset(&fdiag, 0, sizeof(fdiag));
      const int rc_far = gen_topk(h, M, ld, n, laplacian_type, fr, &fdiag, &fdc, &fw, scratch);
      if (rc_far == SC_OK && !fw.empty()) {
        rq.have_far = 1;
        rq.far_value = fw[0];
        far_end = false;
        far_passes = fdiag.eig_matvec_passes;
        far_cycles = fdiag.eig_cycles;
        if (sw::eig_trace())
          fprintf(stderr, "[sc] general eigen path: far end %.12g in %d passes, %d cycles\n",
// ... 216 lines not shown
```

### spectralcluster_amd/csrc/free_api.hip

```cpp
#include <limits>

#include "handle.h"

namespace {
constexpr int kOvfWords = 80;
constexpr int kOvfRowsMax = 64;
}

extern "C" int sc_set_diffuse_mode(sc_handle h, int mode) {
  if (!h || mode < -1 || mode > 2) return SC_ERR_INVALID;
  h->diffuse_mode = mode;
  return SC_OK;
}

extern "C" int sc_set_free_prune(sc_handle h, int on) {
  if (!h || on < -1 || on > 1) return SC_ERR_INVALID;
  h->free_prune = on;
  return SC_OK;
}
static bool free_prune_on(sc_handle h) {
  return h->free_prune >= 0 ? h->free_prune != 0 : !sw::free_no_prune();
}

bool free_diffuse_wanted(sc_handle h, const sc_config* cfg, int n, const EigRequest& rq,
                         bool in_group) {
  const int mode = cfg->diffuse_mode == 1 || cfg->diffuse_mode == 2
                       ? cfg->diffuse_mode
                       : (h->diffuse_mode >= 0 ? h->diffuse_mode : sw::diffuse_mode());
  if (mode == 1) return false;
  if (n <= kDenseMax || n > 65536 || wants_full_spectrum(rq)) return false;
  if (mode == 2) return true;
  return n >= (in_group ? sw::diffuse_free_min_n_group() : sw::diffuse_free_min_n());
}

int ensure_free(sc_handle h, int n) {
  const size_t nv = (size_t)round_up(n, 16) * sizeof(double);
  SC_TRY(grow(h, h->fq, free_q_bytes(n)));
  SC_TRY(grow(h, h->ft32, free_t32_bytes(n)));
  SC_TRY(grow(h, h->fy1, nv));
  SC_TRY(grow(h, h->fR, nv));
  SC_TRY(grow(h, h->fscal, 4 * sizeof(double)));
  SC_TRY(grow(h, h->fwords, ((size_t)2 * n + kOvfWords) * sizeof(int)));
  SC_TRY(grow(h, h->fcand, (size_t)n * free_candidate_cap() * sizeof(int)));
  SC_TRY(grow(h, h->fY, (size_t)n * kEigBlock * sizeof(double)));
  SC_TRY(grow(h, h->fq2part, free_q2part_bytes(n)));
  SC_TRY(grow(h, h->fmx64, free_mx64_bytes(n)));
  SC_TRY(grow(h, h->ftau64, free_tau64_bytes(n)));
  SC_TRY(grow(h, h->fplan, free_plan_bytes(n)));
  if (!h->h_free)
    SC_HIP(h, hipHostMalloc(reinterpret_cast<void**>(&h->h_free), kOvfWords * sizeof(int)));
  return SC_OK;
}

static FreeSegs free_segs(sc_handle h) {
  return FreeSegs{ptr<double>(h->fq2part), ptr<double>(h->fmx64), ptr<float>(h->ftau64)};
}

int free_product(sc_handle h, hipStream_t s, int n) {
  SC_TRY(grow(h, h->fsplit, free_i8_split_bytes_plan()));
  launch_free_tile_flags(s, ptr<double>(h->fmx64), ptr<float>(h->ftau64), n, ptr<int>(h->fplan),
                         free_prune_on(h), ptr<int>(h->fwords));
  launch_gemm_i8_sym(s, ptr<signed char>(h->fq), n, h->tilemap_cur, ptr<float>(h->ft32),
                     ptr<unsigned>(h->fwords), ptr<int>(h->fsplit), ptr<int>(h->fplan));
  return SC_OK;
}

int free_stats_begin(sc_handle h, hipStream_t s, const double* A, int ld, int n, bool have_amax) {
  SC_TRY(ensure_free(h, n));
  SC_HIP(h, hipMemsetAsync(ptr<double>(h->fscal) + (have_amax ? 1 : 0), 0,
                           (have_amax ? 3 : 4) * sizeof(double), s));
  SC_HIP(h, hipMemsetAsync(h->fwords.p, 0, ((size_t)2 * n + kOvfWords) * sizeof(int), s));
  if (!have_amax) launch_free_absmax(s, A, n, ld, ptr<double>(h->fscal));
  launch_free_quantize(s, A, n, ld, ptr<signed char>(h->fq), ptr<double>(h->fscal),
                       ptr<double>(h->fy1), ptr<double>(h->fR), ptr<double>(h->fq2part));
  launch_free_seg_reduce(s, ptr<double>(h->fR), n, free_segs(h));
  return SC_OK;
}
int free_stats_end(sc_handle h, hipStream_t s, const double* A, int ld, int n, bool timed,
                   const int* plan) {
  unsigned* M = ptr<unsigned>(h->fwords);
  int* count = ptr<int>(h->fwords) + n;
  int* ovf = ptr<int>(h->fwords) + 2 * (size_t)n;
  launch_t32_candidates(s, ptr<float>(h->ft32), n, M, ptr<double>(h->fR), ptr<double>(h->fscal),
                        count, ptr<int>(h->fcand), plan);
  if (timed) ev_rec(h, &h->free_ev[3]);
  launch_free_row_stats(s, A, n, ld, ptr<double>(h->fy1), count, ptr<int>(h->fcand),
                        ptr<double>(h->rowmax), ptr<double>(h->rowsum), ovf);
  if (timed) ev_rec(h, &h->free_ev[4]);
  SC_TRY(check_last(h, "matrix-free diffuse launch"));
  SC_HIP(h, hipMemcpyAsync(h->h_free, ovf, kOvfWords * sizeof(int), hipMemcpyDeviceToHost, s));
  h->free_checked = false;
  return SC_OK;
}

int free_group_prepare(sc_handle* hs, const double* const* A, const double* const* cuts,
                       const double* ps, int count, const int* lds, const int* ns, hipStream_t s,
                       double floor_value, FreeItem* items, TsDigits* digits) {
  for (int z = 0; z < count; ++z) {
    sc_handle h = hs[z];
    const int n = ns[z], ld = lds[z];
    SC_TRY(ensure_free(h, n));
    const size_t rows64 = (size_t)round_up(n, 64), nblk = rows64 / 64;
    SC_TRY(grow(h, h->fypart, rows64 * nblk * sizeof(double)));
    SC_TRY(grow(h, h->frpart, rows64 * nblk * sizeof(int)));
    items[z] = FreeItem{A[z], n, ld, ptr<signed char>(h->fq), ptr<float>(h->ft32),
                        ptr<int>(h->fwords), ptr<double>(h->fscal), ptr<double>(h->fy1),
                        ptr<double>(h->fR), ptr<int>(h->fcand), ptr<double>(h->rowmax),
                        ptr<double>(h->rowsum), cuts[z], ps[z]};
    items[z].q2part = ptr<double>(h->fq2part);
    items[z].mx64 = ptr<double>(h->fmx64);
    items[z].tau64 = ptr<float>(h->ftau64);
    items[z].plan = ptr<int>(h->fplan);
    items[z].ypart = ptr<double>(h->fypart);
    items[z].rpart = ptr<int>(h->frpart);
    digits[z] = TsDigits{ptr<signed char>(h->fq), (size_t)2 * rows64, (int)nblk,
                         ptr<double>(h->fscal), ptr<double>(h->fypart), ptr<int>(h->frpart),
                         ptr<double>(h->fq2part), ptr<double>(h->fmx64)};
  }
  launch_free_begin_group(s, items, count, floor_value, true);
  return SC_OK;
}
int free_group_digits(sc_handle* hs, const FreeItem* items, int count, hipStream_t s) {
  launch_free_partials_reduce_group(s, items, count);
  launch_free_tile_flags_group(s, items, count, free_prune_on(hs[0]));
  return SC_OK;
}

int free_group_end(sc_handle* hs, const FreeItem* items, int count, hipStream_t s) {
  launch_free_scan_stats_group(s, items, count);
  SC_TRY(check_last(hs[0], "matrix-free diffuse launch"));
  for (int z = 0; z < count; ++z) {
    sc_handle h = hs[z];
    SC_HIP(h, hipMemcpyAsync(h->h_free, items[z].words + 2 * (size_t)items[z].n,
                             kOvfWords * sizeof(int), hipMemcpyDeviceToHost, s));
    h->free_checked = false;
  }
  return SC_OK;
}

int free_fused_prepare(sc_handle h, hipStream_t s, int n, const double* cut, double p,
                       double floor_value) {
  SC_TRY(ensure_free(h, n));
  const size_t rows64 = (size_t)round_up(n, 64), nblk = rows64 / 64;
  SC_TRY(grow(h, h->fypart, rows64 * nblk * sizeof(double)));
  SC_TRY(grow(h, h->frpart, rows64 * nblk * sizeof(int)));
  FreeItem item{};
  item.n = n;
  item.words = ptr<int>(h->fwords);
  item.scal = ptr<double>(h->fscal);
  item.cut = cut;
  item.p = p;
  launch_free_begin_group(s, &item, 1, floor_value);
  return SC_OK;
}

int free_diffuse_stats(sc_handle h, const double* A, int ld, int n, bool have_amax,
                       bool digits_ready) {
  hipStream_t s = h->stream;
  SC_TRY(ensure_tilemap(h, n));
  ev_rec(h, &h->free_ev[0]);
  if (digits_ready)
    launch_free_partials_reduce(s, ptr<double>(h->fypart), ptr<int>(h->frpart), n,
                                ptr<double>(h->fy1), ptr<double>(h->fR), ptr<double>(h->fscal),
                                free_segs(h));
  else
    SC_TRY(free_stats_begin(h, s, A, ld, n, have_amax));
  ev_rec(h, &h->free_ev[1]);
  SC_TRY(free_product(h, s, n));
  ev_rec(h, &h->free_ev[2]);
  return free_stats_end(h, s, A, ld, n, true, ptr<int>(h->fplan));
}

static void plain_matvec(hipStream_t s, const double* A, int ld, int n, bool sym_mv,
                         const double* Vs, double* W, double* slabs) {
  if (sym_mv)
    launch_block_matvec_sym(s, A, ld, n, nullptr, nullptr, Vs, kEigBlock, Vs, W, slabs);
  else
    launch_block_matvec(s, A, ld, n, nullptr, nullptr, Vs, kEigBlock, Vs, W);
}

int free_fix_overflow(sc_handle h, const double* A, int ld, int n, bool* changed,
                      bool* too_many) {
  *changed = *too_many = false;
  hipStream_t s = h->stream;
  SC_HIP(h, hipStreamSynchronize(s));
  h->free_checked = true;
  const int rows = h->h_free[0];
  if (rows <= 0) return SC_OK;
  if (rows > kOvfRowsMax) {
    *too_many = true;
    return SC_OK;
  }
  SC_TRY(ensure_eig(h, n));
  const bool sym_mv = n >= sw::matvec_sym_min_n();
  const int* ids = ptr<int>(h->fwords) + 2 * (size_t)n + 1;
  for (int r0 = 0; r0 < rows; r0 += kEigBlock) {
    const int nr = std::min(kEigBlock, rows - r0);
    launch_free_gather_rows(s, A, n, ld, ids + r0, nr, ptr<double>(h->Vs));
    plain_matvec(s, A, ld, n, sym_mv, ptr<double>(h->Vs), ptr<double>(h->W),
                 ptr<double>(h->mvsym));
    launch_free_colmax(s, ptr<double>(h->W), n, ids + r0, nr, ptr<double>(h->rowmax));
  }
  SC_TRY(check_last(h, "matrix-free diffuse: exact rows"));
  *changed = true;
  return SC_OK;
}

void free_apply_operator(hipStream_t s, const double* A, int ld, int n, bool sym_mv,
                         const double* cvec, const double* pvec, const double* V, int ldv,
                         const double* Vs, double* fY, double* W, double* slabs) {
  plain_matvec(s, A, ld, n, sym_mv, Vs, fY, slabs);
  if (sym_mv)
    launch_block_matvec_sym(s, A, ld, n, cvec, pvec, V, ldv, fY, W, slabs);
  else
    launch_block_matvec(s, A, ld, n, cvec, pvec, V, ldv, fY, W);
}
void free_apply_operator(sc_handle h, const double* A, int ld, int n, bool sym_mv,
                         const double* V, int ldv) {
  free_apply_operator(h->stream, A, ld, n, sym_mv, ptr<double>(h->cvec), ptr<double>(h->pvec), V,
                      ldv, ptr<double>(h->Vs), ptr<double>(h->fY), ptr<double>(h->W),
                      ptr<double>(h->mvsym));
}

extern "C" int sc_stage_diffuse_rowstats(sc_handle h, const double* a, int n, int mode,
                                         double* rowmax, double* rowsum, int32_t* info) {
  if (!h) return SC_ERR_INVALID;
  if (!a || n <= 0 || !rowmax || !rowsum || (mode != 1 && mode != 2))
    return fail(h, SC_ERR_INVALID, "bad diffuse row statistics request");
  if (mode == 2 && n > 65536) return fail(h, SC_ERR_UNSUPPORTED, "matrix-free diffuse: n <= 65536");
  SC_HIP(h, hipSetDevice(h->device));
  SC_TRY(ensure_matrices(h, n, 0));
  SC_TRY(ensure_eig(h, n));
  SC_TRY(ensure_tilemap(h, n));
  const int ld = matrix_ld(n);
  h->n = n;
  h->ldn = ld;
  h->have_affinity = h->have_cropval = false;
  h->have_x = false;
  h->n_vec = 0;
  h->nev = 0;
  hipStream_t s = h->stream;
  double* A = ptr<double>(h->B2);
  SC_TRY(h2d_matrix(h, a, n, n, A, ld));
  int inf[6] = {0, 0, 0, 0, 0, 0};
  auto explicit_stats = [&]() -> int {
    GemmRowStats rs{1, ptr<double>(h->statp), ptr<double>(h->statp) + (size_t)n * gemm_tile_dim(n),
                    ptr<double>(h->rowmax), ptr<double>(h->rowsum)};
    launch_gemm_nt(s, A, ld, A, ld, ptr<double>(h->B1), ld, n, n, n, kEpiNone, true,
                   ptr<double>(h->splitk), h->tilemap_cur, &rs);
    return check_last(h, "diffuse launch");
  };
  if (mode == 1) {
    SC_TRY(explicit_stats());
  } else {
    SC_TRY(free_diffuse_stats(h, A, ld, n));
    bool changed = false, too_many = false;
    SC_TRY(free_fix_overflow(h, A, ld, n, &changed, &too_many));
    inf[0] = h->h_free[65];
    inf[1] = h->h_free[0];
    inf[2] = h->h_free[66];
    inf[4] = h->h_free[67];
    inf[5] = gemm_tile_dim(n) * (gemm_tile_dim(n) + 1) / 2;
    if (too_many) {
      inf[3] = 1;
      SC_TRY(explicit_stats());
    }
  }
// ... 119 lines not shown
```

### spectralcluster_amd/csrc/handle.h

```cpp
#ifndef SPECTRALCLUSTER_AMD_HANDLE_H_
#define SPECTRALCLUSTER_AMD_HANDLE_H_

#include <algorithm>
#include <array>
#include <cmath>
#include <cstdio>
#include <cstdlib>
#include <cstring>
#include <string>
#include <vector>

#include "sc_internal.h"

using namespace sc;

struct DevBuf {
  void* p = nullptr;
  size_t bytes = 0;
};

constexpr int kKgenBufs = 12;
constexpr int kGroupBanks = 2;
constexpr int kGroupLanes = 3;

struct StageEvents {
  bool pending = false, fine = false, free_path = false;
  int begin = -1, after_refine = -1, after_scaling = -1, after_eig = -1;
  int diffuse[SC_MAX_OPS][2];
  int n_diffuse = 0;
  int blur[2] = {-1, -1}, thr[2] = {-1, -1};
};

struct sc_handle_s {
  int device = 0;
  hipStream_t stream = nullptr;
  std::string err;
  int n = 0, d = 0, ldn = 0, ldx = 0;
  bool have_x = false, have_affinity = false;
  bool have_cropval = false;
  int n_vec = 0;
  DevBuf X, Xn, A0, B1, B2;
  DevBuf Xalt;
  hipStream_t copy_stream = nullptr;
  DevBuf Xstage;
  DevBuf rowmax, rowsum, cvec, pvec, tvec, deg, dvec, cut, rmpart, splitk, tilemap;
  DevBuf cropval, statp;
  DevBuf Cq, cp[5], symflag;
  DevBuf Cband;
  bool have_constraint = false, constraint_symmetric = false, constraint_applied = false;
  bool constraint_banded = false;
  bool affinity_symmetric = true;
  bool affinity_from_embeddings = false;
  int qn = 0;
  int tilemap_nt = 0;
  DevBuf tilemap_table;
  int tilemap_off[65] = {0};
  const int2* tilemap_cur = nullptr;
  DevBuf blurw;
  DevBuf blur_tmp;
  std::vector<double> blur_ext;
  DevBuf Q, Q2, Vs, W, partial, T, Y, Yt, theta, resid, G, Rinv, Hbuf, hsq, colnorm,
      flags;
  DevBuf E, Ek, Eio;
  DevBuf mvsym;
  DevBuf td_d, td_e, td_theta, td_work, td_tau, td_panel;
  std::vector<double> spectrum;
  std::vector<double> last_w;
  DevBuf crvec, thetai, Vre, Vim, gpart, gsrc, genL, gneg;
  DevBuf ahc_size, ahc_chain, ahc_Z, ahc_lab, ahc_cent;
  DevBuf fb_part, fb_small, fb_x, fb_cent, fb_int;
  DevBuf kXc, kxsq, kclosest, kcand, kenorm, krnd, kcent, klab32, klab64, kinfo, kchain;
  DevBuf kbig, kbigw;
  DevBuf kgen[kKgenBufs];
  double* h_theta = nullptr;
  int* h_flags = nullptr;
  double* h_rr = nullptr;
  std::vector<sc_handle_s*> pool;
  std::vector<sc_handle_s*> gslots;
  std::vector<int> sweep_slot;
  std::vector<sc_diag> sweep_diags;
  std::vector<double> sweep_p;
  sc_config sweep_cfg;
  int sweep_n = 0;
  hipEvent_t sync_ev = nullptr;
  DevBuf gkrnd;
  bool gkrnd_ready = false;
  DevBuf gpack, gypack, ginfo, glabels;
  double* h_gpack = nullptr;
  double* h_gypack = nullptr;
  int* h_ginfo = nullptr;
  long long* h_glabels = nullptr;
  size_t h_glabels_count = 0;
  hipEvent_t gcheck_ev = nullptr;
  std::vector<sc_handle_s*> gshort;
  DevBuf gjtab;
  JacobiItem* h_gjtab = nullptr;
  std::vector<int32_t> last_routes;
  int32_t* groutes = nullptr;
  std::vector<sc_handle_s*> glanes;
  class HostPool* gpool = nullptr;
  hipStream_t gbank_stream[kGroupBanks] = {nullptr};
  hipStream_t gchain_stream = nullptr;
  hipEvent_t gbank_ev[kGroupBanks] = {nullptr};
  int gconv_hist[16] = {0};
  int gconv_seen = 0;
  hipEvent_t ev[48];
  int nev = 0;
  StageEvents stage_events;
  int profile_level = 1;
  int mv_ev[16][2];
  int n_mv_ev = 0;
  int aff_ev[2] = {-1, -1};
  int blurw_radius = -1;
  double blurw_host[2 * SC_MAX_BLUR_RADIUS + 1];
  int krnd_k = -1, krnd_trials = -1;
  int kfirst_n = -1, kfirst = 0;
  int diffuse_mode = -1;
  DevBuf fq, ft32, fy1, fR, fscal, fwords, fcand, fY, fsplit, fypart, frpart;
  int free_prune = -1;
  DevBuf fq2part, fmx64, ftau64, fplan;
  int* h_free = nullptr;
  bool free_checked = false;
  int free_ev[5] = {-1, -1, -1, -1, -1};
  int krylov_m = 0, krylov_n = 0, krylov_cycles = 0, krylov_ahead = 0;
  bool krylov_free = false;
};

inline void ev_rec(sc_handle h, int* slot) {
  if (h->nev < 48) {
    hipEventRecord(h->ev[h->nev], h->stream);
    *slot = h->nev++;
  } else {
    *slot = -1;
  }
}
inline float ev_ms(sc_handle h, int a, int b) {
  if (a < 0 || b < 0) return 0.f;
  float ms = 0.f;
  hipEventElapsedTime(&ms, h->ev[a], h->ev[b]);
  return ms;
}

constexpr int kTilemapTableMax = 64;
constexpr int kMaxCols = 128;
inline int matrix_ld(int n) {
  int ld = round_up(n, 16);
  if (ld % 512 == 0) ld += 16;
  return ld;
}


#define SC_HIP(h, call)                                                         \
  do {                                                                          \
    hipError_t e_ = (call);                                                     \
    if (e_ != hipSuccess) {                                                     \
      (h)->err = std::string(#call) + ": " + hipGetErrorString(e_);             \
      return e_ == hipErrorOutOfMemory ? SC_ERR_OOM : SC_ERR_HIP;               \
    }                                                                           \
  } while (0)

#define SC_TRY(expr)                \
  do {                              \
    int rc_ = (expr);               \
    if (rc_ != SC_OK) return rc_;   \
  } while (0)

inline int fail(sc_handle h, int code, const std::string& msg) {
  if (h) h->err = msg;
  return code;
}

inline int grow(sc_handle h, DevBuf& b, size_t bytes) {
  if (b.bytes >= bytes) return SC_OK;
  if (b.p) {
    SC_HIP(h, hipStreamSynchronize(h->stream));
    SC_HIP(h, hipFree(b.p));
    b.p = nullptr;
    b.bytes = 0;
  }
  SC_HIP(h, hipMalloc(&b.p, bytes));
  b.bytes = bytes;
  return SC_OK;
}
template <typename T>
inline T* ptr(const DevBuf& b) {
  return reinterpret_cast<T*>(b.p);
}

int ensure_matrices(sc_handle h, int n, int d, bool affinity_copy = true);

int ensure_tilemap(sc_handle h, int n);
int predict_sequence(sc_handle h, const int* idx, int count, const sc_array* xs,
                     const int* ns, int d, const sc_config* cfg, int64_t* const* labels,
                     sc_diag* diags);
int validate_array(sc_handle h, const sc_array* a);
sc_array host_f64_array(const double* x, int n, int d);
std::vector<sc_array> host_f64_arrays(const double* const* xs, const int* ns, int d, int count);
bool array_is_host_f64_rows(const sc_array& a);
int ingest_embeddings(sc_handle h, const sc_array& a, bool sync, hipStream_t stream = nullptr);
int predict_batch_streams_impl(sc_handle h, const sc_array* xs, const int* ns, int d, int count,
                               const sc_config* cfg, int64_t* const* labels, sc_diag* diags,
                               int streams);
int predict_batch_grouped_impl(sc_handle h, const sc_array* xs, const int* ns, int d, int count,
                               const sc_config* cfg, int64_t* const* labels, sc_diag* diags,
                               int group);

int ensure_eig(sc_handle h, int n);

int ensure_gen(sc_handle h, int n);

int ensure_kmeans(sc_handle h, int n, int k = kMaxVectors);
int ensure_vectors(sc_handle h, int n, int cols);

inline int check_last(sc_handle h, const char* what) {
  hipError_t e = hipGetLastError();
  if (e != hipSuccess) {
    h->err = std::string(what) + ": " + hipGetErrorString(e);
    return SC_ERR_HIP;
  }
  return SC_OK;
}


int h2d_matrix(sc_handle h, const double* src, int rows, int cols, double* dst, int ld);
int d2h_matrix(sc_handle h, const double* src, int ld, int rows, int cols, double* dst);
int validate_config(sc_handle h, const sc_config* cfg);
void eigengap_core(const double* w, int count, int max_clusters, double stop_eigenvalue,
                   int eigengap_type, int descend, double wmax, int* n_clusters,
                   double* max_delta);

struct EigRequest {
  int descend;
  int max_clusters;
  int min_clusters;
  double stop_eigenvalue;
  int eigengap_type;
  int use_stop;
  double value_tol, vector_tol;
  int max_cycles;
  int fixed_count;
  int decision_aware = 0;
  int negate = 0;
  int no_dense = 0;
  int have_far = 0;
  double far_value = 0.0;
};

struct EigDecision {
  bool enough = false;
  bool converged = false;
  int kw = 0;
  int kvec = 0;
  int n_clusters_raw = 0;
  double max_delta = 0.0;
  double max_resid = 0.0;
  bool unsupported = false;
  int fail_kind = 0;
  int fail_index = -1;
};

struct FrontResult {
  const double* matrix = nullptr;
  double* scratch = nullptr;
  int ld = 0;
  bool symmetric = false, folded_rownorm = false;
  bool free_op = false;
  int laplacian_type = 0;
  bool chain_flags_cleared = false;
  bool skip_fused = false;
};
EigRequest make_eig_request(const sc_config* cfg);
int upload_blur_weights(sc_handle h, const sc_config* cfg);
int eig_ncluster_impl(sc_handle h, const sc_config* cfg, sc_diag* diag, FrontResult* front_only,
                      const FrontResult* resume = nullptr, bool defer_timing = false);
void kmeans_seed_constants(int k, double* u_first, int* trials, std::vector<double>* rnd);
KmeansWorkspace kmeans_workspace(sc_handle h);

struct GroupEigMember {
  sc_handle h = nullptr;
  const double* S = nullptr;
  int ld = 0, n = 0;
  EigRequest rq;
  int status = 0;
  EigDecision dc;
  std::vector<double> w;
  int basis = 0, passes = 0;
  bool skip_fused = false;
  bool free_op = false;
};
int sym_topk_group(sc_handle lead, GroupEigMember* mem, int count, bool want_vectors = true);
int dense_topk_group(sc_handle lead, GroupEigMember* mem, int count);
bool sym_group_eligible(int n, const EigRequest& rq, bool any_size = false);

int sym_topk(sc_handle h, const FrontResult& op, int n, const EigRequest& rq, sc_diag* diag,
             EigDecision* out_dc, std::vector<double>* out_w);
int gen_topk(sc_handle h, const double* M, int ld, int n, int laplacian_type,
             const EigRequest& rq, sc_diag* diag, EigDecision* out_dc,
             std::vector<double>* out_w, double* scratch);

bool free_diffuse_wanted(sc_handle h, const sc_config* cfg, int n, const EigRequest& rq,
                         bool in_group = false);
int free_group_prepare(sc_handle* hs, const double* const* A, const double* const* cuts,
                       const double* ps, int count, const int* lds, const int* ns, hipStream_t s,
                       double floor_value, struct FreeItem* items, struct TsDigits* digits);
int free_group_digits(sc_handle* hs, const struct FreeItem* items, int count, hipStream_t s);
int free_group_end(sc_handle* hs, const struct FreeItem* items, int count, hipStream_t s);
int free_fused_prepare(sc_handle h, hipStream_t s, int n, const double* cut, double p,
                       double floor_value);
int free_diffuse_stats(sc_handle h, const double* A, int ld, int n, bool have_amax = false,
                       bool digits_ready = false);
int ensure_free(sc_handle h, int n);
int free_product(sc_handle h, hipStream_t s, int n);
int free_stats_begin(sc_handle h, hipStream_t s, const double* A, int ld, int n, bool have_amax);
int free_stats_end(sc_handle h, hipStream_t s, const double* A, int ld, int n, bool timed,
                   const int* plan = nullptr);
int free_fix_overflow(sc_handle h, const double* A, int ld, int n, bool* changed, bool* too_many);
void free_apply_operator(sc_handle h, const double* A, int ld, int n, bool sym_mv,
                         const double* V, int ldv);
void free_apply_operator(hipStream_t s, const double* A, int ld, int n, bool sym_mv,
                         const double* cvec, const double* pvec, const double* V, int ldv,
                         const double* Vs, double* fY, double* W, double* slabs);
bool wants_full_spectrum(const EigRequest& rq);

int device_is_symmetric(sc_handle h, const double* m, int n, int ld, bool* out);
int adjust_affinity(sc_handle h, const sc_config* cfg, const double* a, bool sym_a, double* out,
                    int n, int ld);
bool constraint_active(sc_handle h, const sc_config* cfg, bool before);
struct CpGroupMember {
  int n = 0, ld = 0;
  double* A = nullptr;
  double *P = nullptr, *T = nullptr, *Pn = nullptr, *Tn = nullptr;
  double *deg = nullptr, *rowmax = nullptr;
  const double* band = nullptr;
  const int2* tilemap = nullptr;
};
int constraint_propagation_group(sc_handle lead, hipStream_t s, const CpGroupMember* mem,
                                 int count, double alpha);
int predict_batch_constrained_impl(sc_handle h, const sc_array* xs, const double* const* bands,
                                   const int* ns, int d, int count, const sc_config* cfg,
                                   int64_t* const* labels, sc_diag* diags, int group);

#endif
```

### spectralcluster_amd/csrc/kmeans_api.hip

```cpp
#include <algorithm>
#include <cmath>
#include <cstdio>
#include <vector>

#include "handle.h"

int ensure_kmeans(sc_handle h, int n, int k) {
  const int cols = std::max(k, kMaxCols), kk = std::max(k, kMaxVectors);
  SC_TRY(grow(h, h->Ek, (size_t)round_up(n, 16) * cols * sizeof(double)));
  SC_TRY(grow(h, h->Eio, (size_t)n * cols * sizeof(double)));
  SC_TRY(grow(h, h->kXc, (size_t)n * kk * sizeof(double)));
  SC_TRY(grow(h, h->kxsq, (size_t)n * sizeof(double)));
  SC_TRY(grow(h, h->kclosest, (size_t)n * sizeof(double)));
  SC_TRY(grow(h, h->kcand, (size_t)(k > kMaxVectors ? 16 : 8) * n * sizeof(double)));
  SC_TRY(grow(h, h->kenorm, (size_t)n * sizeof(double)));
  SC_TRY(grow(h, h->krnd, (size_t)std::max(1024, 16 * kk) * sizeof(double)));
  SC_TRY(grow(h, h->kcent, (size_t)kk * kk * sizeof(double)));
  if (k > kMaxVectors) {
    SC_TRY(grow(h, h->kbig, kmeans_big_workspace_doubles(k) * sizeof(double)));
    SC_TRY(grow(h, h->kbigw, (size_t)3 * k * sizeof(int)));
  }
  SC_TRY(grow(h, h->klab32, (size_t)n * sizeof(int)));
  SC_TRY(grow(h, h->klab64, (size_t)n * sizeof(long long)));
  SC_TRY(grow(h, h->kinfo, 16 * sizeof(int)));
  SC_TRY(grow(h, h->kchain, kmeans_chain_workspace_doubles(n) * sizeof(double)));
  return SC_OK;
}

KmeansWorkspace kmeans_workspace(sc_handle h) {
  KmeansWorkspace ws;
  ws.Xc = ptr<double>(h->kXc);
  ws.xsq = ptr<double>(h->kxsq);
  ws.closest = ptr<double>(h->kclosest);
  ws.cand = ptr<double>(h->kcand);
  ws.enorm = ptr<double>(h->kenorm);
  ws.rnd = ptr<double>(h->krnd);
  ws.centroids = ptr<double>(h->kcent);
  ws.labels32 = ptr<int>(h->klab32);
  ws.labels64 = ptr<long long>(h->klab64);
  ws.info = ptr<int>(h->kinfo);
  ws.chain = ptr<double>(h->kchain);
  ws.big = ptr<double>(h->kbig);
  ws.big_words = ptr<int>(h->kbigw);
  return ws;
}

enum { kgX, kgIo, kgRow, kgVec, kgCd, kgPart, kgRnd, kgLab32, kgLab64, kgInt, kgCount };
static_assert(kgCount <= kKgenBufs, "handle.h kgen buffers");

static int ensure_kmeans_general(sc_handle h, int n, int dim, int k, int trials,
                                 KmeansGeneralWorkspace* ws) {
  constexpr int TS = kKgenTrialSlots;
  const size_t ld = round_up(n, 16);
  SC_TRY(grow(h, h->kgen[kgX], ld * dim * sizeof(double)));
  SC_TRY(grow(h, h->kgen[kgIo], (size_t)n * dim * sizeof(double)));
  SC_TRY(grow(h, h->kgen[kgRow], 4 * ld * sizeof(double)));
  SC_TRY(grow(h, h->kgen[kgVec],
              ((size_t)dim * (1 + k + TS) + 2 * (size_t)k + TS + kKgenScalars) * sizeof(double)));
  SC_TRY(grow(h, h->kgen[kgCd], 2 * (size_t)TS * n * sizeof(double)));
  SC_TRY(grow(h, h->kgen[kgPart], (size_t)kmeans_general_grid(n) * TS * sizeof(double)));
  SC_TRY(grow(h, h->kgen[kgRnd], (size_t)std::max(1, (k - 1) * trials) * sizeof(double)));
  SC_TRY(grow(h, h->kgen[kgLab32], (size_t)n * sizeof(int)));
  SC_TRY(grow(h, h->kgen[kgLab64], (size_t)n * sizeof(long long)));
  SC_TRY(grow(h, h->kgen[kgInt], ((size_t)k + TS + kKgenWords) * sizeof(int)));
  ws->X = ptr<double>(h->kgen[kgX]);
  ws->ld = (int)ld;
  ws->xsq = ptr<double>(h->kgen[kgRow]);
  ws->enorm = ws->xsq + ld;
  ws->rmx = ws->xsq + 2 * ld;
  ws->cnu = ws->xsq + 3 * ld;
  ws->mean = ptr<double>(h->kgen[kgVec]);
  ws->cent = ws->mean + dim;
  ws->cval = ws->cent + (size_t)k * dim;
  ws->cmx = ws->cval + k;
  ws->crow = ws->cmx + k;
  ws->csq = ws->crow + (size_t)TS * dim;
  ws->scal = ws->csq + TS;
  ws->cd = ptr<double>(h->kgen[kgCd]);
  ws->part = ptr<double>(h->kgen[kgPart]);
  ws->rnd = ptr<double>(h->kgen[kgRnd]);
  ws->lab32 = ptr<int>(h->kgen[kgLab32]);
  ws->lab64 = ptr<long long>(h->kgen[kgLab64]);
  ws->seeds = ptr<int>(h->kgen[kgInt]);
  ws->cand = ws->seeds + k;
  ws->words = ws->cand + TS;
  return SC_OK;
}

void kmeans_seed_constants(int k, double* u_first, int* trials, std::vector<double>* rnd) {
  *trials = 2 + (int)std::log((double)k);
  const size_t nrnd = (size_t)std::max(1, (k - 1) * *trials);
  std::vector<double> stream(1 + nrnd);
  sc_random_state_doubles(0, (int)stream.size(), stream.data());
  *u_first = stream[0];
  rnd->assign(stream.begin() + 1, stream.end());
}

static int check_kmeans_request(sc_handle h, int n, int k, int max_iter, int metric, int slots) {
  if (metric < kKmeansCosine || metric > kKmeansCanberra)
    return fail(h, SC_ERR_UNSUPPORTED,
                "custom_dist on the device: cosine, euclidean (minkowski), sqeuclidean, "
                "cityblock, chebyshev, correlation, braycurtis, canberra");
  if (max_iter <= 0)
    return fail(h, SC_ERR_INVALID, "Number of iterations should be a positive number");
  if (n < k) return fail(h, SC_ERR_INVALID, "n_samples should be >= n_clusters");
  if (k < 1) return fail(h, SC_ERR_INVALID, "n_clusters must be positive");
  if (2 + (int)std::log((double)k) > slots)
    return fail(h, SC_ERR_UNSUPPORTED, "too many k-means++ trials");
  return SC_OK;
}

static int kmeans_on_device(sc_handle h, const double* E, int lde, int n, int k, int max_iter,
                            int64_t* labels, double* centroids_out, int* iterations,
                            int metric = kKmeansCosine) {
  SC_TRY(check_kmeans_request(h, n, k, max_iter, metric, k > kMaxVectors ? 16 : 8));
  SC_TRY(ensure_kmeans(h, n, k));
  if (h->kfirst_n != n || h->krnd_k != k) {
    double u_first;
    int trials;
    std::vector<double> rnd;
    kmeans_seed_constants(k, &u_first, &trials, &rnd);
    if (h->kfirst_n != n) {
      h->kfirst = sc_uniform_choice(n, u_first);
      h->kfirst_n = n;
    }
    if (h->krnd_k != k) {
      SC_HIP(h, hipMemcpyAsync(h->krnd.p, rnd.data(), rnd.size() * sizeof(double),
                               hipMemcpyHostToDevice, h->stream));
      SC_HIP(h, hipStreamSynchronize(h->stream));
      h->krnd_k = k;
      h->krnd_trials = trials;
    }
  }
  const int first = h->kfirst, trials = h->krnd_trials;
  const KmeansWorkspace ws = kmeans_workspace(h);
  int info[16] = {0};
  if (metric == kKmeansCosine && kmeans_chain_supported(n, k, trials) &&
      !sw::kmeans_single()) {
    for (int it = 0;; it += 4) {
      launch_kmeans_chain(h->stream, E, lde, n, k, max_iter, first, trials, ws, it, 4);
      SC_TRY(check_last(h, "kmeans launch"));
      SC_HIP(h, hipMemcpyAsync(labels, h->klab64.p, (size_t)n * sizeof(int64_t),
                               hipMemcpyDeviceToHost, h->stream));
      SC_HIP(h, hipMemcpyAsync(info, h->kinfo.p, 9 * sizeof(int), hipMemcpyDeviceToHost,
                               h->stream));
      SC_HIP(h, hipStreamSynchronize(h->stream));
      if (info[8] != 0) break;
      if (it > max_iter + 4)
        return fail(h, SC_ERR_HIP, "k-means chain did not reach its stop rule");
    }
    if (centroids_out) {
      SC_HIP(h, hipMemcpyAsync(centroids_out, h->kcent.p, (size_t)k * k * sizeof(double),
                               hipMemcpyDeviceToHost, h->stream));
      SC_HIP(h, hipStreamSynchronize(h->stream));
    }
    if (iterations) *iterations = info[0];
    return SC_OK;
  }
  SC_HIP(h, hipMemsetAsync(h->kinfo.p, 0, 8 * sizeof(int), h->stream));
  launch_kmeans(h->stream, E, lde, n, k, max_iter, first, trials, ws, metric);
  SC_TRY(check_last(h, "kmeans launch"));
  SC_HIP(h, hipMemcpyAsync(labels, h->klab64.p, (size_t)n * sizeof(int64_t),
                           hipMemcpyDeviceToHost, h->stream));
  SC_HIP(h, hipMemcpyAsync(info, h->kinfo.p, 6 * sizeof(int), hipMemcpyDeviceToHost,
                           h->stream));
  if (centroids_out)
    SC_HIP(h, hipMemcpyAsync(centroids_out, h->kcent.p, (size_t)k * k * sizeof(double),
                             hipMemcpyDeviceToHost, h->stream));
  SC_HIP(h, hipStreamSynchronize(h->stream));
  if (iterations) *iterations = info[0];
  if (sw::kmeans_trace())
    fprintf(stderr, "[sc] kmeans n=%d k=%d iters=%d  us: centre %.1f  kmeans++ %.1f  lloyd %.1f"
            "  cosine-loop %.1f\n", n, k, info[0], info[1] * 0.01, (info[2] - info[1]) * 0.01,
            (info[3] - info[2]) * 0.01, (info[4] - info[3]) * 0.01);
  if (sw::kmeans_trace() && k > kMaxVectors) {
    std::vector<int> seeds(k);
    hipMemcpy(seeds.data(), h->kbigw.p, (size_t)k * sizeof(int), hipMemcpyDeviceToHost);
    fprintf(stderr, "[sc] kmeans++ seeds:");
    for (int i = 0; i < k; ++i) fprintf(stderr, " %d", seeds[i]);
    fprintf(stderr, "\n");
  }
  return SC_OK;
}

extern "C" int sc_cluster(sc_handle h, const sc_config* cfg, int n_clusters, int64_t* labels,
                          sc_diag* diag) {
  if (!h) return SC_ERR_INVALID;
  if (!cfg || !labels) return fail(h, SC_ERR_INVALID, "NULL argument");
  if (h->n_vec <= 0) return fail(h, SC_ERR_INVALID, "no eigenvectors resident");
  if (n_clusters < 1 || n_clusters > h->n_vec)
    return fail(h, SC_ERR_INVALID, "n_clusters exceeds the resident eigenvectors");
  SC_HIP(h, hipSetDevice(h->device));
  const int n = h->n;
  int e0, e1;
  ev_rec(h, &e0);
  const double* E = ptr<double>(h->E);
  const int lde = round_up(n, 16);
  if (cfg->row_wise_renorm) {
    SC_TRY(ensure_kmeans(h, n, n_clusters));
    SC_HIP(h, hipMemcpyAsync(h->Ek.p, h->E.p, (size_t)lde * n_clusters * sizeof(double),
                             hipMemcpyDeviceToDevice, h->stream));
    launch_row_renorm(h->stream, ptr<double>(h->Ek), lde, n, n_clusters);
    E = ptr<double>(h->Ek);
  }
  int iters = 0;
  SC_TRY(kmeans_on_device(h, E, lde, n, n_clusters, cfg->max_iter, labels, nullptr, &iters,
                          cfg->kmeans_metric));
  ev_rec(h, &e1);
  SC_HIP(h, hipStreamSynchronize(h->stream));
  if (diag) {
    diag->n_clusters = n_clusters;
    diag->kmeans_iterations = iters;
    diag->stage_ms[SC_STAGE_KMEANS] = ev_ms(h, e0, e1);
  }
  return SC_OK;
}

extern "C" int sc_stage_kmeans_metric(sc_handle h, const double* e, int n, int k, int max_iter,
                                      int metric, int64_t* labels, double* centroids_out,
                                      int* iterations) {
  if (!h) return SC_ERR_INVALID;
  if (!e || !labels || n <= 0 || k <= 0) return fail(h, SC_ERR_INVALID, "bad k-means input");
  SC_HIP(h, hipSetDevice(h->device));
  SC_TRY(ensure_kmeans(h, n, k));
  SC_HIP(h, hipMemcpyAsync(h->Eio.p, e, (size_t)n * k * sizeof(double), hipMemcpyHostToDevice,
                           h->stream));
  launch_to_colmajor(h->stream, ptr<double>(h->Eio), n, k, ptr<double>(h->Ek),
                     round_up(n, 16));
  return kmeans_on_device(h, ptr<double>(h->Ek), round_up(n, 16), n, k, max_iter, labels,
                          centroids_out, iterations, metric);
}

extern "C" int sc_stage_kmeans(sc_handle h, const double* e, int n, int k, int max_iter,
                               int64_t* labels, double* centroids_out, int* iterations) {
  return sc_stage_kmeans_metric(h, e, n, k, max_iter, SC_KMEANS_COSINE, labels, centroids_out,
                                iterations);
}

extern "C" int sc_stage_kmeans_general(sc_handle h, const double* x, int n, int dim, int k,
                                       int max_iter, int metric, double tol,
                                       const double* init_centroids, int64_t* labels,
                                       double* centroids_out, int* iterations) {
  constexpr int kItersPerSync = 4;
  if (!h) return SC_ERR_INVALID;
  if (!x || !labels || n <= 0 || dim <= 0 || k <= 0)
    return fail(h, SC_ERR_INVALID, "bad k-means input");
  if ((long long)n * dim > 0x7fffffffLL)
// ... 47 lines not shown
```

### spectralcluster_amd/csrc/rowops.hip

```cpp
#include <algorithm>
#include <cstring>

#include "dpp.h"
#include "sc_internal.h"

namespace sc {

constexpr int kRowThreads = 256;

__device__ __forceinline__ double wave_max(double v) {
#pragma unroll
  for (int o = 32; o > 0; o >>= 1) v = fmax(v, __shfl_xor(v, o));
  return v;
}
__device__ __forceinline__ double wave_sum(double v) {
#pragma unroll
  for (int o = 32; o > 0; o >>= 1) v += __shfl_xor(v, o);
  return v;
}
__device__ __forceinline__ double block_max(double v, double* sm) {
  v = wave_max(v);
  __syncthreads();
  if ((threadIdx.x & 63) == 0) sm[threadIdx.x >> 6] = v;
  __syncthreads();
// ... 542 lines not shown
    }
    m = fmax(m, v.x);
    if (j + 1 < n) m = fmax(m, v.y);
  }
  m = block_max(m, sm);
  const double cut = m * p;
  for (int j = 2 * threadIdx.x; j < n; j += 2 * kRowThreads) {
    double2 v = *reinterpret_cast<const double2*>(x + j);
    if (preserve_diag) {
      if (j == row) v.x = 0.0;
      if (j + 1 == row) v.y = 0.0;
    }
    double2 r;
    r.x = v.x < cut ? v.x * mult : (binarize ? 1.0 : v.x);
    r.y = v.y < cut ? v.y * mult : (binarize ? 1.0 : v.y);
    if (preserve_diag) {
      if (j == row) r.x = 1.0;
      if (j + 1 == row) r.y = 1.0;
    }
    *reinterpret_cast<double2*>(o + j) = r;
  }
}

__global__ __launch_bounds__(kRowThreads) void k_row_normalize(
    const double* __restrict__ in, double* __restrict__ out, int n, int ld) {
  __shared__ double sm[4];
  const int row = blockIdx.x;
  const double* x = in + (size_t)row * ld;
  double* o = out + (size_t)row * ld;
  double m = -INFINITY;
  for (int j = 2 * threadIdx.x; j < n; j += 2 * kRowThreads) {
    const double2 v = *reinterpret_cast<const double2*>(x + j);
    m = fmax(m, v.x);
    if (j + 1 < n) m = fmax(m, v.y);
  }
  m = block_max(m, sm);
  for (int j = 2 * threadIdx.x; j < n; j += 2 * kRowThreads) {
    double2 v = *reinterpret_cast<const double2*>(x + j);
    v.x = v.x / m;
    v.y = v.y / m;
    *reinterpret_cast<double2*>(o + j) = v;
  }
}

__device__ __forceinline__ void row_stats_body(
    const double* __restrict__ in, int n, int ld, double* __restrict__ rowmax,
    double* __restrict__ rowsum) {
  __shared__ double sm[4];
  const int row = blockIdx.x;
  const double* x = in + (size_t)row * ld;
  double m = -INFINITY, s = 0.0;
  for (int j = 2 * threadIdx.x; j < n; j += 2 * kRowThreads) {
    const double2 v = *reinterpret_cast<const double2*>(x + j);
    m = fmax(m, v.x);
    s += v.x;
    if (j + 1 < n) {
      m = fmax(m, v.y);
      s += v.y;
    }
  }
  m = block_max(m, sm);
  s = block_sum(s, sm);
  if (threadIdx.x == 0) {
    rowmax[row] = m;
    rowsum[row] = s;
  }
}
__global__ __launch_bounds__(kRowThreads) void k_row_stats(
    const double* __restrict__ in, int n, int ld, double* __restrict__ rowmax,
    double* __restrict__ rowsum) {
  row_stats_body(in, n, ld, rowmax, rowsum);
}
__global__ __launch_bounds__(kRowThreads) void k_row_stats_g(const GroupOf<FrontItem> g) {
  const FrontItem& a = g.s[blockIdx.y];
  if ((int)blockIdx.x >= a.n) return;
  row_stats_body(a.B2, a.n, a.ldn, const_cast<double*>(a.rowmax), const_cast<double*>(a.rowsum));
}

__device__ __forceinline__ void scaling_vectors_body(const double* __restrict__ rowmax,
                                                     const double* __restrict__ rowsum, int n,
                                                     int lap, int rownorm,
                                                     double* __restrict__ c,
                                                     double* __restrict__ p,
                                                     double* __restrict__ t) {
  const int i = blockIdx.x * blockDim.x + threadIdx.x;
  if (i >= n) return;
  const double eps = 1e-10;
  const double a = rownorm ? 1.0 / rowmax[i] : 1.0;
  const double sa = sqrt(a);
  const double deg = rownorm ? rowsum[i] / rowmax[i] : rowsum[i];
  double cv = sa, pv = 0.0, tv = sa;
  if (lap == SC_LAPLACIAN_UNNORMALIZED) {
    pv = -deg;
  } else if (lap == SC_LAPLACIAN_RANDOM_WALK) {
    const double g = 1.0 / (deg + eps);
    cv = sqrt(g * a);
    pv = -(g * deg);
    tv = cv;
  } else if (lap == SC_LAPLACIAN_GRAPH_CUT) {
    const double h = 1.0 / (sqrt(deg) + eps);
    cv = h * sa;
    pv = -((h * deg) * h);
  }
  c[i] = cv;
  p[i] = pv;
  t[i] = tv;
}
__global__ void k_scaling_vectors(const double* __restrict__ rowmax,
                                  const double* __restrict__ rowsum, int n,
                                  int lap, int rownorm, double* __restrict__ c,
                                  double* __restrict__ p, double* __restrict__ t,
                                  int* __restrict__ flags, int* __restrict__ symflag) {
  scaling_vectors_body(rowmax, rowsum, n, lap, rownorm, c, p, t);
  if (flags != nullptr && blockIdx.x == 0 && threadIdx.x == 0) {
    flags[12] = symflag != nullptr ? symflag[1] : 0;
    flags[13] = 0;
    flags[14] = 0;
    flags[15] = 0;
  }
}
__global__ void k_scaling_vectors_g(const GroupOf<FrontItem> g, int lap, int rownorm) {
  const FrontItem& a = g.s[blockIdx.y];
  const int i = blockIdx.x * blockDim.x + threadIdx.x;
  if (i >= a.n) return;
  scaling_vectors_body(a.rowmax, a.rowsum, a.n, lap, rownorm, a.cvec, a.pvec, a.tvec);
  if (!isfinite(a.cvec[i]) || !isfinite(a.pvec[i]) ||
      (i == 0 && a.symflag != nullptr && a.symflag[1] != 0))
    a.flags[12] = 1;
}

__global__ void k_check_finite(const double* __restrict__ a, const double* __restrict__ b,
                               int n, int* __restrict__ flag) {
  const int i = blockIdx.x * blockDim.x + threadIdx.x;
  if (i >= n) return;
  if (!isfinite(a[i]) || !isfinite(b[i])) *flag = 1;
}

__global__ __launch_bounds__(kRowThreads) void k_row_sum(
    const double* __restrict__ in, int n, int ld, double* __restrict__ rowsum) {
  __shared__ double sm[4];
  const int row = blockIdx.x;
  const double* x = in + (size_t)row * ld;
  double s = 0.0;
  for (int j = threadIdx.x; j < n; j += kRowThreads) s += x[j];
  s = block_sum(s, sm);
  if (threadIdx.x == 0) rowsum[row] = s;
}

__global__ __launch_bounds__(kRowThreads) void k_laplacian(
    const double* __restrict__ in, double* __restrict__ out, int n, int ld,
    int lap, const double* __restrict__ deg) {
  const int row = blockIdx.x;
  const double eps = 1e-10;
  const double* x = in + (size_t)row * ld;
  double* o = out + (size_t)row * ld;
  const double di = deg[row];
  double ri = 1.0;
  if (lap == SC_LAPLACIAN_RANDOM_WALK) ri = 1.0 / (di + eps);
  if (lap == SC_LAPLACIAN_GRAPH_CUT) ri = 1.0 / (sqrt(di) + eps);
  for (int j = threadIdx.x; j < n; j += kRowThreads) {
    double l = (j == row ? di : 0.0) - x[j];
    if (lap == SC_LAPLACIAN_RANDOM_WALK) {
      l = ri * l;
    } else if (lap == SC_LAPLACIAN_GRAPH_CUT) {
      const double rj = 1.0 / (sqrt(deg[j]) + eps);
      l = (ri * l) * rj;
    }
    o[j] = l;
  }
}

__global__ __launch_bounds__(256) void k_symmetrize(const double* __restrict__ in,
                                                    double* __restrict__ out,
                                                    int n, int ld, int type) {
  __shared__ double tile[32][33];
  const int bi = blockIdx.y * 32, bj = blockIdx.x * 32;
  const int tx = threadIdx.x & 31, ty = threadIdx.x >> 5;
#pragma unroll
  for (int r = ty; r < 32; r += 8) {
    const int gi = bj + r, gj = bi + tx;
    tile[r][tx] = (gi < n && gj < n) ? in[(size_t)gi * ld + gj] : 0.0;
  }
  __syncthreads();
#pragma unroll
  for (int r = ty; r < 32; r += 8) {
    const int gi = bi + r, gj = bj + tx;
    if (gi < n && gj < n) {
      const double a = in[(size_t)gi * ld + gj];
      const double b = tile[tx][r];
      out[(size_t)gi * ld + gj] =
          type == SC_SYMMETRIZE_MAX ? fmax(a, b) : 0.5 * (a + b);
    }
  }
}

void launch_normalize_rows(hipStream_t s, const double* X, int ldx, int n, int d,
                           double* Xn, int* bad_rows) {
  hipLaunchKernelGGL(k_normalize_rows, dim3((n + 3) / 4), dim3(kRowThreads), 0, s, X, ldx, n,
                     d, Xn, bad_rows);
}
void launch_crop_diagonal(hipStream_t s, const double* in, double* out, int n,
                          int ld) {
  hipLaunchKernelGGL(k_crop_diagonal, dim3(n), dim3(kRowThreads), 0, s, in, out, n,
                     ld);
}
void launch_row_threshold(hipStream_t s, const double* in, double* out, int n,
                          int ld, double p, double mult, int binarize,
                          int preserve_diag) {
  hipLaunchKernelGGL(k_row_threshold, dim3(n), dim3(kRowThreads), 0, s, in, out, n,
                     ld, p, mult, binarize, preserve_diag);
}
void launch_crop_value(hipStream_t s, const double* in, int n, int ld, double* dvec) {
  hipLaunchKernelGGL(k_crop_value, dim3(n), dim3(kRowThreads), 0, s, in, n, ld, dvec);
}
void launch_cut_from_partials(hipStream_t s, const double* partials, int n, int ntiles,
                              double p, double* cut) {
  hipLaunchKernelGGL(k_cut_from_partials, dim3((n + 3) / 4), dim3(256), 0, s, partials, n,
                     ntiles, p, cut);
}
void launch_cut_from_rows(hipStream_t s, const double* in, int n, int ld, double p,
                          double* cut, int zero_diag) {
  hipLaunchKernelGGL(k_cut_from_rows, dim3(n), dim3(kRowThreads), 0, s, in, n, ld, p, cut,
                     zero_diag);
}
void launch_cut_percentile(hipStream_t s, const double* in, int n, int ld, double p,
                           double* cut, int zero_diag) {
  int prev, next;
  double gamma;
  percentile_position(n, p, &prev, &next, &gamma);
  const size_t bytes = (size_t)n * sizeof(unsigned long long);
  const int in_lds = bytes <= 128 * 1024;
  SC_OPT_IN_LDS(k_row_percentile_cut, 128 * 1024);
  hipLaunchKernelGGL(k_row_percentile_cut, dim3(n), dim3(256), in_lds ? bytes : 0, s, in, n,
                     ld, zero_diag, prev, next, gamma, cut, in_lds);
}
void launch_row_threshold_cut(hipStream_t s, const double* in, double* out, int n, int ld,
                              const double* cut, double mult, int binarize,
                              int preserve_diag) {
  hipLaunchKernelGGL(k_row_threshold_cut, dim3(n), dim3(kRowThreads), 0, s, in, out, n, ld,
                     cut, mult, binarize, preserve_diag);
}
void launch_threshold_symmetrize(hipStream_t s, const double* in, double* out, int n, int ld,
                                 const double* cut, double mult, int binarize, int symtype,
                                 int preserve_diag) {
  const int t = (n + kTsTile - 1) / kTsTile;
  hipLaunchKernelGGL(k_threshold_symmetrize, dim3(t * (t + 1) / 2), dim3(256), 0, s, in, out,
                     n, ld, cut, mult, binarize, symtype, t, preserve_diag);
}
void launch_threshold_symmetrize_digits(hipStream_t s, const double* in, double* out, int n, int ld,
                                        const double* cut, double mult, int binarize, int symtype,
                                        int preserve_diag, signed char* Q, double* scal,
                                        double* ypart, int* rpart, double* q2part,
                                        double* mx64) {
  const int t = (n + kTsTile - 1) / kTsTile;
  const size_t pitch = (size_t)2 * t * kTsTile;
  const int rows_padded = (n + 127) / 128 * 128;
  if (rows_padded > t * kTsTile)
    hipMemsetAsync(Q + (size_t)t * kTsTile * pitch, 0, (size_t)(rows_padded - t * kTsTile) * pitch, s);
  const TsDigits dg{Q, pitch, t, scal, ypart, rpart, q2part, mx64};
  hipLaunchKernelGGL(k_threshold_symmetrize_digits, dim3(t * (t + 1) / 2), dim3(256), 0, s, in,
                     out, n, ld, cut, mult, binarize, symtype, t, preserve_diag, dg);
}
void launch_free_partials_reduce(hipStream_t s, const double* ypart, const int* rpart, int n,
                                 double* y1, double* R, double* scal, const FreeSegs& segs) {
  const int nblk = (n + kTsTile - 1) / kTsTile;
  hipLaunchKernelGGL(k_free_partials_reduce, dim3(nblk), dim3(256), 0, s, ypart, rpart, n,
                     nblk, y1, R, reinterpret_cast<unsigned long long*>(scal) + 2, segs);
}
void launch_row_normalize(hipStream_t s, const double* in, double* out, int n,
                          int ld) {
  hipLaunchKernelGGL(k_row_normalize, dim3(n), dim3(kRowThreads), 0, s, in, out, n,
                     ld);
}
void launch_row_stats(hipStream_t s, const double* in, int n, int ld,
                      double* rowmax, double* rowsum) {
  hipLaunchKernelGGL(k_row_stats, dim3(n), dim3(kRowThreads), 0, s, in, n, ld,
                     rowmax, rowsum);
}
void launch_scaling_vectors(hipStream_t s, const double* rowmax,
                            const double* rowsum, int n, int laplacian_type,
                            int row_normalized, double* c, double* p, double* t, int* flags,
                            int* symflag) {
  hipLaunchKernelGGL(k_scaling_vectors, dim3((n + 255) / 256), dim3(256), 0, s,
                     rowmax, rowsum, n, laplacian_type, row_normalized, c, p, t, flags, symflag);
}
static GroupOf<FrontItem> front_pack(const FrontItem* items, int count, int* nmax) {
  GroupOf<FrontItem> g;
  memset(&g, 0, sizeof(g));
  *nmax = 0;
  for (int z = 0; z < count; ++z) {
    g.s[z] = items[z];
    *nmax = std::max(*nmax, items[z].n);
  }
  return g;
}
void launch_front_begin_group(hipStream_t s, const FrontItem* items, int count,
                              bool normalize_rows) {
  int nmax;
  const GroupOf<FrontItem> g = front_pack(items, count, &nmax);
  if (nmax == 0) return;
  hipLaunchKernelGGL(k_front_words_init_g, dim3(count), dim3(64), 0, s, g);
  if (normalize_rows)
    hipLaunchKernelGGL(k_normalize_rows_g, dim3((nmax + 3) / 4, count), dim3(kRowThreads), 0, s,
                       g);
}
void launch_cut_percentile_group(hipStream_t s, const FrontItem* items, int count, int zero_diag) {
  int nmax;
  const GroupOf<FrontItem> g = front_pack(items, count, &nmax);
  if (nmax == 0) return;
  const size_t bytes = (size_t)nmax * sizeof(unsigned long long);
  const int in_lds = bytes <= 128 * 1024;
  SC_OPT_IN_LDS(k_row_percentile_cut_g, 128 * 1024);
  hipLaunchKernelGGL(k_row_percentile_cut_g, dim3(nmax, count), dim3(256), in_lds ? bytes : 0, s,
                     g, zero_diag, in_lds);
}
void launch_row_stats_group(hipStream_t s, const FrontItem* items, int count) {
  int nmax;
  const GroupOf<FrontItem> g = front_pack(items, count, &nmax);
  if (nmax == 0) return;
  hipLaunchKernelGGL(k_row_stats_g, dim3(nmax, count), dim3(kRowThreads), 0, s, g);
}
void launch_threshold_symmetrize_group(hipStream_t s, const FrontItem* items, int count,
                                       double p, double mult, int binarize, int symtype,
                                       int preserve_diag, bool cut_ready, const TsDigits* digits) {
  int nmax;
  const GroupOf<FrontItem> g = front_pack(items, count, &nmax);
  if (nmax == 0) return;
  if (!cut_ready)
    hipLaunchKernelGGL(k_cut_from_partials_g, dim3((nmax + 3) / 4, count), dim3(256), 0, s, g, p);
  const int t = (nmax + kTsTile - 1) / kTsTile;
  if (digits != nullptr) {
    GroupOf<TsDigits> dg;
    memset(&dg, 0, sizeof(dg));
    for (int z = 0; z < count; ++z) dg.s[z] = digits[z];
    hipLaunchKernelGGL(k_threshold_symmetrize_digits_g, dim3(t * (t + 1) / 2, count), dim3(256), 0,
                       s, g, dg, mult, binarize, symtype, preserve_diag);
    return;
  }
  hipLaunchKernelGGL(k_threshold_symmetrize_g, dim3(t * (t + 1) / 2, count), dim3(256), 0, s, g,
                     mult, binarize, symtype, preserve_diag);
}
void launch_cut_from_partials_group(hipStream_t s, const FrontItem* items, int count, double p) {
  int nmax;
  const GroupOf<FrontItem> g = front_pack(items, count, &nmax);
  if (nmax == 0) return;
  hipLaunchKernelGGL(k_cut_from_partials_g, dim3((nmax + 3) / 4, count), dim3(256), 0, s, g, p);
}
void launch_free_partials_reduce_group(hipStream_t s, const FreeItem* items, int count) {
  GroupOf<FreeItem> g;
  memset(&g, 0, sizeof(g));
  int nmax = 0;
  for (int z = 0; z < count; ++z) {
    g.s[z] = items[z];
    nmax = std::max(nmax, items[z].n);
  }
  if (nmax == 0) return;
  hipLaunchKernelGGL(k_free_partials_reduce_g, dim3((nmax + kTsTile - 1) / kTsTile, count),
                     dim3(256), 0, s, g);
}
void launch_scaling_vectors_group(hipStream_t s, const FrontItem* items, int count,
                                  int laplacian_type, int row_normalized) {
  int nmax;
  const GroupOf<FrontItem> g = front_pack(items, count, &nmax);
  if (nmax == 0) return;
  hipLaunchKernelGGL(k_scaling_vectors_g, dim3((nmax + 255) / 256, count), dim3(256), 0, s, g,
                     laplacian_type, row_normalized);
}
// ... 19 lines not shown
```

### spectralcluster_amd/csrc/sc_internal.h

```cpp
#pragma once

#include <hip/hip_runtime.h>

#include "switches.h"
#include <stdint.h>

#include <mutex>
#include <string>
#include <vector>

#include "../../include/spectralcluster_amd.h"

namespace sc {

constexpr int kWave = 64;
constexpr int kEigBlock = 8;
constexpr int kEigBasisCap = 128;
constexpr int kLdq = kEigBasisCap + kEigBlock;
constexpr int kDenseMax = 128;
constexpr int kHostRR = 64;
constexpr int kHostRRSingle = kEigBasisCap;
constexpr int kGenMax = 64;
constexpr int kMaxVectors = 64;
constexpr int kProjBlocks = 128;
// ... 34 lines not shown
  const int2* tilemap = nullptr;
  double* partial_max = nullptr;
  double* partial_sum = nullptr;
  double* rowmax = nullptr;
  double* rowsum = nullptr;
};
void launch_gemm_nt_group(hipStream_t s, const GemmGroupItem* items, int count, int epilogue,
                          int stats_mode);
struct GemmPairItem {
  const double* A = nullptr;
  int lda = 0;
  const double* B = nullptr;
  int ldb = 0;
  double* C = nullptr;
  int ldc = 0;
  int n = 0;
  const int2* tilemap = nullptr;
  const double* addend = nullptr;
};
void launch_gemm_nt_pair_group(hipStream_t s, const GemmPairItem* items, int count, int epilogue);
void gemm_build_sym_tilemap(int nt, std::vector<int2>* out);
int gemm_tile_dim(int n);
int gemm_resident_slots();
size_t gemm_splitk_workspace_bytes();

void launch_normalize_rows(hipStream_t s, const double* X, int ldx, int n, int d,
                           double* Xn, int* bad_rows = nullptr);
void launch_crop_diagonal(hipStream_t s, const double* in, double* out, int n,
                          int ld);
void launch_gaussian_blur(hipStream_t s, const double* in, double* out, int n,
                          int ld, int radius, const double* weights_dev);
bool launch_gaussian_blur_fused(hipStream_t s, const double* in, double* out, int n, int ld,
                                int radius, const double* weights_dev, const double* diag,
                                double* rowmax_partials);
int blur_tile_columns(int n, int radius);
void launch_gaussian_blur_any_radius(hipStream_t s, const double* in, double* tmp, double* out,
                                     int n, int ld, int radius, const double* weights_dev);
void launch_crop_value(hipStream_t s, const double* in, int n, int ld, double* dvec);
void launch_cut_from_partials(hipStream_t s, const double* partials, int n, int ntiles,
                              double p, double* cut);
void launch_cut_from_rows(hipStream_t s, const double* in, int n, int ld, double p,
                          double* cut, int zero_diag);
void launch_cut_percentile(hipStream_t s, const double* in, int n, int ld, double p,
                           double* cut, int zero_diag);
void launch_row_threshold_cut(hipStream_t s, const double* in, double* out, int n, int ld,
                              const double* cut, double mult, int binarize,
                              int preserve_diag);
void launch_threshold_symmetrize(hipStream_t s, const double* in, double* out, int n, int ld,
                                 const double* cut, double mult, int binarize, int symtype,
                                 int preserve_diag);
void launch_threshold_symmetrize_digits(hipStream_t s, const double* in, double* out, int n, int ld,
                                        const double* cut, double mult, int binarize, int symtype,
                                        int preserve_diag, signed char* Q, double* scal,
                                        double* ypart, int* rpart, double* q2part,
                                        double* mx64);
struct FreeSegs;
void launch_free_partials_reduce(hipStream_t s, const double* ypart, const int* rpart, int n,
                                 double* y1, double* R, double* scal, const FreeSegs& segs);
void launch_row_threshold(hipStream_t s, const double* in, double* out, int n,
                          int ld, double p, double mult, int binarize,
                          int preserve_diag);
void launch_symmetrize(hipStream_t s, const double* in, double* out, int n, int ld,
                       int type);

void launch_affinity_integration(hipStream_t s, const double* a, const double* q, double* out,
                                 int n, int ld, int type);
void launch_affinity_integration_band(hipStream_t s, const double* a, const double* band,
                                      double* out, int n, int ld, int type);
void launch_cp_band_product(hipStream_t s, const double* tt, const double* band, double* x,
                            int n, int ld);
void launch_cp_prepare(hipStream_t s, const double* a, const double* deg, double alpha,
                       double* p, double* t0, int n, int ld);
void launch_cp_adjust(hipStream_t s, const double* tqt, const double* a, double scale,
                      double* out, int n, int ld);
void launch_transpose(hipStream_t s, const double* in, double* out, int n, int ld);
void launch_symmetry_flag(hipStream_t s, const double* in, int n, int ld, int* flag);
void launch_row_normalize(hipStream_t s, const double* in, double* out, int n,
                          int ld);
void launch_row_stats(hipStream_t s, const double* in, int n, int ld,
                      double* rowmax, double* rowsum);
void launch_scaling_vectors(hipStream_t s, const double* rowmax,
                            const double* rowsum, int n, int laplacian_type,
                            int row_normalized, double* c, double* p, double* t,
                            int* flags = nullptr, int* symflag = nullptr);
void launch_laplacian(hipStream_t s, const double* in, double* out, int n, int ld,
                      int laplacian_type, double* deg_ws);
void launch_check_finite(hipStream_t s, const double* a, const double* b, int n, int* flag);

struct EigWorkspace {
  double* Q = nullptr;
  double* Q2 = nullptr;
  double* Vs = nullptr;
  double* W = nullptr;
  double* partial = nullptr;
  double* T = nullptr;
  double* Y = nullptr;
  double* theta = nullptr;
  double* resid = nullptr;
  double* G = nullptr;
  double* Rinv = nullptr;
  double* Hbuf = nullptr;
  double* hsq = nullptr;
  double* Yt = nullptr;
  double* colnorm = nullptr;
  int* flags = nullptr;
};

void launch_random_block(hipStream_t s, double* W, int n, uint64_t seed);
void launch_block_matvec(hipStream_t s, const double* S, int ld, int n,
                         const double* cvec, const double* pvec, const double* V,
                         int ldv, const double* Vs, double* W);
size_t matvec_sym_workspace_doubles(int n);
void launch_block_matvec_sym(hipStream_t s, const double* S, int ld, int n, const double* cvec,
                             const double* pvec, const double* V, int ldv, const double* Vs,
                             double* W, double* ws);
void launch_proj_partial(hipStream_t s, const double* Q, int ldq, int m,
                         const double* W, int n, double* partial);
int proj_blocks(int n);
void launch_reduce_H(hipStream_t s, const double* partial, int nparts, int m, double* Hbuf,
                     double* T, int ldt, int col0, int accumulate, double* hsq);
void launch_update_block(hipStream_t s, const double* Q, int ldq, int m,
                         const double* Hbuf, double* W, int n);
void launch_reduce_chol(hipStream_t s, const double* partial, int nparts, double* Rinv,
                        double* Gsave, const double* hsq, int* flags,
                        int* defect_flag = nullptr, int flag_mode = 1);
void launch_apply_rinv(hipStream_t s, double* W, int n, const double* Rinv,
                       double* Qdst, int ldq, int col0, const double* cvec,
                       double* Vs);
void launch_refill_deficient(hipStream_t s, double* W, int n, const int* flags,
                             uint64_t seed);
struct LzChain {
  int parity = 0;
  int nparts = 0;
  bool three_pass = false;
};
size_t lz_partial_doubles(int n);
void launch_lz_link(hipStream_t s, const EigWorkspace& ws, LzChain* chain, int n, int m,
                    int pre, int next, int store_col, const double* vs_scale, int col0,
                    bool init_random, uint64_t seed, bool zero_T);
constexpr int kGroupMax = 16;
#ifndef SC_SHORT_WIDTH
#define SC_SHORT_WIDTH 64
#endif
constexpr int kShortWidth = SC_SHORT_WIDTH;
static_assert(kShortWidth >= 1 && kShortWidth <= 256, "one workgroup per CU");
template <typename T>
struct GroupOf {
  T s[kGroupMax];
};
struct MatvecItem {
  const double* S;
  int ld, n;
  const double* cvec;
  const double* pvec;
  const double* V;
  int ldv;
  const double* Vs;
  double* W;
  double* slabs;
};
struct RitzItem {
  const double* Q;
  int ldq, m;
  const double* Y;
  int ldy, cols;
  double* E;
  int lde, n;
// ... 310 lines not shown
```

Baseline: 392.2 calls/s.

## Overlap Lanczos start block on side stream and pack small device-host transfers

Launches the random Lanczos start block on a separate non-blocking stream before the affinity refinement, then joins it before the eigen solve so that work overlaps the front stages. The scaling-vector kernel now folds the finite check and chain-flag clearing into a last-block-arrives reduction, which removes a separate check kernel. T, G, flags and theta are packed into contiguous buffers so each Rayleigh-Ritz check needs one host copy instead of several. K-means labels and info are read back with one pinned copy, and some timing events are reused instead of recorded again. The cost is extra stream and event management, and there is a risk of races if the start-ahead state is misused.

```diff
diff --git a/spectralcluster_amd/csrc/api.hip b/spectralcluster_amd/csrc/api.hip
--- a/spectralcluster_amd/csrc/api.hip
+++ b/spectralcluster_amd/csrc/api.hip
@@ -83,20 +83,25 @@
   SC_TRY(grow(h, h->W, (size_t)n * kEigBlock * sizeof(double)));
   SC_TRY(grow(h, h->partial, std::max((size_t)kProjBlocks * kLdq * kEigBlock,
                                        lz_partial_doubles(n)) * sizeof(double)));
-  SC_TRY(grow(h, h->T, (size_t)kLdq * kLdq * sizeof(double)));
-  SC_TRY(grow(h, h->Y, (size_t)kLdq * kLdq * sizeof(double)));
+  if (!h->rrpack.p) {
+    SC_TRY(grow(h, h->rrpack, kRrPackDoubles * sizeof(double)));
+    SC_TRY(grow(h, h->rypack, kRyPackDoubles * sizeof(double)));
+    double* rr = ptr<double>(h->rrpack);
+    double* ry = ptr<double>(h->rypack);
+    h->G = DevBuf{rr, 256 * sizeof(double)};
+    h->flags = DevBuf{rr + kRrFlagsAt, 16 * sizeof(int)};
+    h->T = DevBuf{rr + kRrTAt, (size_t)kLdq * kLdq * sizeof(double)};
+    h->theta = DevBuf{ry, kLdq * sizeof(double)};
+    h->Y = DevBuf{ry + kRyYAt, (size_t)kLdq * kLdq * sizeof(double)};
+    SC_HIP(h, hipMemsetAsync(h->flags.p, 0, (kRrTAt - kRrFlagsAt) * sizeof(double), h->stream));
+    SC_HIP(h, hipStreamSynchronize(h->stream));
+  }
   SC_TRY(grow(h, h->Yt, (size_t)kLdq * kLdq * sizeof(double)));
-  SC_TRY(grow(h, h->theta, kLdq * sizeof(double)));
   SC_TRY(grow(h, h->resid, kLdq * sizeof(double)));
-  SC_TRY(grow(h, h->G, 256 * sizeof(double)));
   SC_TRY(grow(h, h->Rinv, 256 * sizeof(double)));
   SC_TRY(grow(h, h->Hbuf, (size_t)kLdq * kEigBlock * sizeof(double)));
   SC_TRY(grow(h, h->hsq, 16 * sizeof(double)));
   SC_TRY(grow(h, h->colnorm, (size_t)kProjBlocks * kMaxVectors * sizeof(double)));
-  if (h->flags.bytes < 16 * sizeof(int)) {
-    SC_TRY(grow(h, h->flags, 16 * sizeof(int)));
-    SC_HIP(h, hipMemsetAsync(h->flags.p, 0, 16 * sizeof(int), h->stream));
-  }
   SC_TRY(grow(h, h->mvsym, matvec_sym_workspace_doubles(n) * sizeof(double)));
   SC_TRY(ensure_vectors(h, n, kMaxCols));
   return SC_OK;
@@ -193,12 +198,12 @@
   hipStreamSynchronize(h->stream);
   DevBuf* bufs[] = {&h->X,     &h->Xn,    &h->A0,     &h->B1,      &h->B2,    &h->rowmax,
                     &h->rowsum, &h->cvec,  &h->pvec,   &h->tvec,    &h->deg,   &h->blurw, &h->blur_tmp, &h->dvec, &h->cut, &h->rmpart, &h->splitk, &h->tilemap, &h->tilemap_table, &h->cropval, &h->statp, &h->crvec, &h->thetai, &h->Vre, &h->Vim, &h->gpart, &h->gsrc, &h->genL, &h->ahc_size, &h->ahc_chain, &h->ahc_Z, &h->ahc_lab, &h->ahc_cent, &h->fb_part, &h->fb_small, &h->fb_x, &h->fb_cent, &h->fb_int, &h->Cq, &h->Cband, &h->cp[0], &h->cp[1], &h->cp[2], &h->cp[3], &h->cp[4], &h->symflag,
-                    &h->Q,     &h->Q2,    &h->Vs,     &h->W,       &h->partial, &h->T,
-                    &h->Y,     &h->Yt,    &h->theta,  &h->resid,   &h->G,     &h->Rinv,
-                    &h->Hbuf,  &h->hsq,   &h->colnorm, &h->flags,  &h->E,     &h->Ek,   &h->Eio,
+                    &h->Q,     &h->Q2,    &h->Vs,     &h->W,       &h->partial, &h->rrpack,
+                    &h->rypack, &h->Yt,   &h->resid,  &h->Rinv,
+                    &h->Hbuf,  &h->hsq,   &h->colnorm, &h->E,     &h->Ek,   &h->Eio,
                     &h->td_d,  &h->td_e,  &h->td_theta, &h->td_work, &h->td_tau, &h->td_panel, &h->mvsym,
                     &h->kXc,   &h->kxsq,  &h->kclosest, &h->kcand, &h->kenorm, &h->krnd,
-                    &h->kcent, &h->klab32, &h->klab64, &h->kinfo, &h->kchain, &h->gkrnd, &h->gpack, &h->gypack, &h->ginfo, &h->glabels, &h->gjtab,
+                    &h->kcent, &h->klab32, &h->klab64, &h->kchain, &h->gkrnd, &h->gpack, &h->gypack, &h->ginfo, &h->glabels, &h->gjtab,
                     &h->kbig, &h->kbigw, &h->fq, &h->ft32, &h->fy1, &h->fR, &h->fscal, &h->fwords, &h->fcand, &h->fY, &h->fsplit, &h->fypart, &h->frpart, &h->fq2part, &h->fmx64, &h->ftau64, &h->fplan, &h->Xalt, &h->Xstage, &h->gneg};
   for (DevBuf* b : bufs)
     if (b->p) hipFree(b->p);
@@ -208,6 +213,8 @@
   if (h->h_theta) hipHostFree(h->h_theta);
   if (h->h_flags) hipHostFree(h->h_flags);
   if (h->h_rr) hipHostFree(h->h_rr);
+  if (h->h_rrpack) hipHostFree(h->h_rrpack);
+  if (h->h_rypack) hipHostFree(h->h_rypack);
   if (h->h_free) hipHostFree(h->h_free);
   if (h->sync_ev) hipEventDestroy(h->sync_ev);
   for (int b = 0; b < kGroupBanks; ++b) {
@@ -216,6 +223,8 @@
   }
   if (h->gchain_stream) hipStreamDestroy(h->gchain_stream);
   if (h->copy_stream) hipStreamDestroy(h->copy_stream);
+  if (h->side_stream) hipStreamDestroy(h->side_stream);
+  if (h->start_ev) hipEventDestroy(h->start_ev);
   if (h->gcheck_ev) hipEventDestroy(h->gcheck_ev);
   for (sc_handle lane : h->glanes) sc_destroy(lane);
   h->glanes.clear();
@@ -225,6 +234,7 @@
   if (h->h_gjtab) hipHostFree(h->h_gjtab);
   if (h->h_ginfo) hipHostFree(h->h_ginfo);
   if (h->h_glabels) hipHostFree(h->h_glabels);
+  if (h->h_klab) hipHostFree(h->h_klab);
   hipStreamDestroy(h->stream);
   delete h;
   return SC_OK;
@@ -605,7 +615,7 @@
 }
 
 int eig_ncluster_impl(sc_handle h, const sc_config* cfg, sc_diag* diag, FrontResult* front_only,
-                      const FrontResult* resume, bool defer_timing) {
+                      const FrontResult* resume, bool defer_timing, int begin_ev) {
   const int n = h->n, ld = h->ldn;
   hipStream_t s = h->stream;
   const double* cur = ptr<double>(h->A0);
@@ -623,7 +633,12 @@
   const double* digits_of = nullptr;
   float diffuse_ms_events[SC_MAX_OPS][2];
   int n_diffuse = 0;
-  ev_rec(h, &e_begin);
+  bool diffuse_was_last = false;
+  if (begin_ev >= 0) e_begin = begin_ev; else ev_rec(h, &e_begin);
+  SC_TRY(start_block_join(h));
+  h->start_ready_n = 0;
+  if (!resume && !front_only && n > kDenseMax && cfg->n_ops > 0 && !sw::eig_host_chain())
+    SC_TRY(start_block_ahead(h, n));
   const bool blur_fast = (cfg->blur_radius == 4 || cfg->blur_radius == 8) && n >= 128;
   const double* pending_diag = nullptr;
   bool have_partials = false;
@@ -655,12 +670,14 @@
         pending_diag = ptr<double>(h->dvec);
       }
       have_partials = false;
+      diffuse_was_last = false;
       continue;
     }
     double* out = bufs[which];
     which ^= 1;
     int e0 = -1, e1 = -1;
     bool keep_cur = false;
+    diffuse_was_last = false;
     if (op == SC_OP_DIFFUSE) ev_rec(h, &e0);
     if (op == SC_OP_GAUSSIAN_BLUR && blur_fast) {
       const bool want = next == SC_OP_ROW_WISE_THRESHOLD && next2 == SC_OP_SYMMETRIZE &&
@@ -729,7 +746,7 @@
                (i == cfg->n_ops - 1 || (i == cfg->n_ops - 2 && next == SC_OP_ROW_WISE_NORMALIZE)) &&
                free_diffuse_wanted(h, cfg, n, make_eig_request(cfg))) {
       SC_TRY(ensure_eig(h, n));
-      SC_TRY(free_diffuse_stats(h, cur, ld, n, amax_of == cur, digits_of == cur));
+      SC_TRY(free_diffuse_stats(h, cur, ld, n, amax_of == cur, digits_of == cur, e0));
       free_path = true;
       have_row_stats = true;
       have_partials = false;
@@ -751,7 +768,8 @@
       have_partials = false;
     }
     if (op == SC_OP_DIFFUSE) {
-      ev_rec(h, &e1);
+      if (keep_cur && h->free_ev[4] >= 0) e1 = h->free_ev[4]; else ev_rec(h, &e1);
+      diffuse_was_last = true;
       diffuse_ms_events[n_diffuse][0] = (float)e0;
       diffuse_ms_events[n_diffuse][1] = (float)e1;
       ++n_diffuse;
@@ -778,11 +796,15 @@
     double* out = bufs[which];
     which ^= 1;
     SC_TRY(adjust_affinity(h, cfg, cur, symmetric, out, n, ld));
+    diffuse_was_last = false;
     cur = out;
     symmetric = symmetric && h->constraint_symmetric;
     have_row_stats = false;
   }
-  ev_rec(h, &e_after_refine);
+  if (diffuse_was_last && n_diffuse > 0 && (int)diffuse_ms_events[n_diffuse - 1][1] >= 0)
+    e_after_refine = (int)diffuse_ms_events[n_diffuse - 1][1];
+  else
+    ev_rec(h, &e_after_refine);
   bool flags_by_kernel = false;
   if (resume) {
     SC_TRY(ensure_eig(h, n));
@@ -798,7 +820,9 @@
     launch_scaling_vectors(s, ptr<double>(h->rowmax), ptr<double>(h->rowsum), n,
                            cfg->laplacian_type, folded_rownorm ? 1 : 0, ptr<double>(h->cvec),
                            ptr<double>(h->pvec), ptr<double>(h->tvec), ptr<int>(h->flags),
-                           h->affinity_from_embeddings ? ptr<int>(h->symflag) : nullptr);
+                           h->affinity_from_embeddings ? ptr<int>(h->symflag) : nullptr,
+                           h->start_ready_n != n,
+                           reinterpret_cast<int*>(ptr<double>(h->rrpack) + kRrArriveAt));
     flags_by_kernel = true;
   }
   SC_TRY(ensure_eig(h, n));
@@ -808,7 +832,8 @@
                              hipMemcpyDeviceToDevice, s));
   else
     SC_HIP(h, hipMemsetAsync(ptr<int>(h->flags) + 12, 0, sizeof(int), s));
-  launch_check_finite(s, ptr<double>(h->cvec), ptr<double>(h->pvec), n, ptr<int>(h->flags) + 12);
+  if (!flags_by_kernel)
+    launch_check_finite(s, ptr<double>(h->cvec), ptr<double>(h->pvec), n, ptr<int>(h->flags) + 12);
   if (front_only && !flags_by_kernel)
     SC_HIP(h, hipMemsetAsync(ptr<int>(h->flags) + 13, 0, 3 * sizeof(int), s));
   SC_TRY(check_last(h, "scaling launch"));
@@ -838,19 +863,24 @@
   op.laplacian_type = cfg->laplacian_type;
   op.chain_flags_cleared = flags_by_kernel;
   op.skip_fused = resume && resume->skip_fused;
+  op.start_ahead = h->start_ready_n == n;
   if (front_only) {
     *front_only = op;
     return SC_OK;
   }
   EigRequest rq = make_eig_request(cfg);
+  SC_TRY(start_block_join(h));
   EigDecision dc;
   std::vector<double> w;
+  int eig_rc;
   if (symmetric) {
-    SC_TRY(sym_topk(h, op, n, rq, diag, &dc, &w));
+    eig_rc = sym_topk(h, op, n, rq, diag, &dc, &w);
   } else {
     rq.decision_aware = 1;
-    SC_TRY(gen_topk(h, cur, ld, n, cfg->laplacian_type, rq, diag, &dc, &w, bufs[which]));
-  }
+    eig_rc = gen_topk(h, cur, ld, n, cfg->laplacian_type, rq, diag, &dc, &w, bufs[which]);
+  }
+  h->start_ready_n = 0;
+  SC_TRY(eig_rc);
   int e_after_eig;
   ev_rec(h, &e_after_eig);
   h->last_w = w;
@@ -933,9 +963,10 @@
   int e0, e1, e2;
   ev_rec(h, &e0);
   SC_TRY(sc_compute_affinity(h));
-  if (constraint_active(h, cfg, true)) SC_TRY(sc_apply_constraint(h, cfg));
-  ev_rec(h, &e1);
-  SC_TRY(eig_ncluster_impl(h, cfg, dg, nullptr, nullptr, true));
+  const bool constrained = constraint_active(h, cfg, true);
+  if (constrained) SC_TRY(sc_apply_constraint(h, cfg));
+  if (!constrained && h->aff_ev[1] >= 0) e1 = h->aff_ev[1]; else ev_rec(h, &e1);
+  SC_TRY(eig_ncluster_impl(h, cfg, dg, nullptr, nullptr, true, e1));
   int k = dg->n_clusters_raw;
   if (cfg->min_clusters > 0 && k < cfg->min_clusters) k = cfg->min_clusters;
   const int rc_cluster = sc_cluster(h, cfg, k, labels, dg);
diff --git a/spectralcluster_amd/csrc/eig.hip b/spectralcluster_amd/csrc/eig.hip
--- a/spectralcluster_amd/csrc/eig.hip
+++ b/spectralcluster_amd/csrc/eig.hip
@@ -633,6 +633,7 @@
   }
   if (first_wg && a.Tzero != nullptr)
     for (int e = tid; e < kLdq * kLdq; e += kLzThreads) a.Tzero[e] = 0.0;
+  if (first_wg && a.init_random && a.flags != nullptr && tid < 3) a.flags[13 + tid] = 0;
   if (pre_gram) {
     if (pre_proj && tid < B * B) {
       const int a1 = tid / B, b1 = tid % B;
diff --git a/spectralcluster_amd/csrc/eig_driver.hip b/spectralcluster_amd/csrc/eig_driver.hip
--- a/spectralcluster_amd/csrc/eig_driver.hip
+++ b/spectralcluster_amd/csrc/eig_driver.hip
@@ -380,11 +380,43 @@
   return ws;
 }
 
+int start_block_ahead(sc_handle h, int n) {
+  SC_TRY(ensure_eig(h, n));
+  if (!h->side_stream) {
+    SC_HIP(h, hipStreamCreateWithFlags(&h->side_stream, hipStreamNonBlocking));
+    SC_HIP(h, hipEventCreateWithFlags(&h->start_ev, hipEventDisableTiming));
+  }
+  const EigWorkspace ws = eig_workspace(h);
+  h->start_chain = LzChain();
+  const uint64_t seed = 0x5eed5eedull;
+  launch_lz_link(h->side_stream, ws, &h->start_chain, n, 0, 0, 4, -1, nullptr, 0, true, seed,
+                 false);
+  launch_lz_link(h->side_stream, ws, &h->start_chain, n, 0, 4, 3, -1, nullptr, 0, false, 0, true);
+  h->start_pending = true;
+  SC_TRY(check_last(h, "start block launch"));
+  SC_HIP(h, hipEventRecord(h->start_ev, h->side_stream));
+  h->start_ready_n = n;
+  return SC_OK;
+}
+int start_block_join(sc_handle h) {
+  if (!h->start_pending) return SC_OK;
+  h->start_pending = false;
+  SC_HIP(h, hipStreamWaitEvent(h->stream, h->start_ev, 0));
+  return SC_OK;
+}
+
 int sym_topk(sc_handle h, const FrontResult& op_in, int n, const EigRequest& rq_in,
              sc_diag* diag, EigDecision* out_dc, std::vector<double>* out_w) {
   hipStream_t s = h->stream;
   h->krylov_m = 0;
+  SC_TRY(start_block_join(h));
   SC_TRY(ensure_eig(h, n));
+  if (!h->h_rrpack) {
+    SC_HIP(h, hipHostMalloc(reinterpret_cast<void**>(&h->h_rrpack),
+                            kRrPackDoubles * sizeof(double)));
+    SC_HIP(h, hipHostMalloc(reinterpret_cast<void**>(&h->h_rypack),
+                            kRyPackDoubles * sizeof(double)));
+  }
   FrontResult op = op_in;
   const int ld = op.ld;
   auto free_materialize = [&](bool with_stats) -> int {
@@ -509,14 +541,21 @@
     }
     if (done) {
     } else if (fused) {
-      if (!op.chain_flags_cleared)
+      const bool take_ahead = op.start_ahead && h->start_ready_n == n && !three_pass;
+      if (!op.chain_flags_cleared && !take_ahead)
         SC_HIP(h, hipMemsetAsync(ptr<int>(h->flags) + 13, 0, 3 * sizeof(int), s));
       op.chain_flags_cleared = false;
       const EigWorkspace ws = eig_workspace(h);
       chain = LzChain();
       chain.three_pass = three_pass;
-      launch_lz_link(s, ws, &chain, n, 0, 0, 4, -1, cvec, 0, true, seed, false);
-      launch_lz_link(s, ws, &chain, n, 0, 4, 3, -1, cvec, 0, false, 0, true);
+      if (take_ahead) {
+        chain = h->start_chain;
+      } else {
+        launch_lz_link(s, ws, &chain, n, 0, 0, 4, -1, cvec, 0, true, seed, false);
+        launch_lz_link(s, ws, &chain, n, 0, 4, 3, -1, cvec, 0, false, 0, true);
+      }
+      op.start_ahead = false;
+      h->start_ready_n = 0;
       launch_lz_link(s, ws, &chain, n, 0, 3, 0, 0, cvec, 0, false, 0, false);
       SC_TRY(check_last(h, "start block launch"));
     } else {
@@ -576,14 +615,12 @@
       m += kEigBlock;
       const bool check = check_due(m);
       const bool host_rr = check && m <= kHostRRSingle && !sw::eig_device_rr();
-      if (host_rr) {
-        SC_HIP(h, hipMemcpy2DAsync(h->h_rr, (size_t)m * sizeof(double), h->T.p,
-                                   (size_t)kLdq * sizeof(double), (size_t)m * sizeof(double), m,
-                                   hipMemcpyDeviceToHost, s));
-        SC_HIP(h, hipMemcpyAsync(h->h_rr + kHostRRSingle * kHostRRSingle, h->G.p,
-                                 kEigBlock * kEigBlock * sizeof(double), hipMemcpyDeviceToHost,
-                                 s));
-      } else if (check) {
+      if (op.free_op && !h->free_checked && (!fused || check)) SC_TRY(free_flush_ovf(h));
+      if (host_rr && !fused) {
+        SC_HIP(h, hipMemcpyAsync(h->h_rrpack, h->rrpack.p,
+                                 (kRrTAt + (size_t)m * kLdq) * sizeof(double),
+                                 hipMemcpyDeviceToHost, s));
+      } else if (check && !host_rr) {
         launch_jacobi(s, ptr<double>(h->T), kLdq, m, 0, nullptr, nullptr, ptr<double>(h->G),
                       theta_d, ptr<double>(h->Y), kLdq, resid_d, ptr<double>(h->Yt),
                       ptr<int>(h->flags));
@@ -601,7 +638,13 @@
         }
         SC_TRY(rcb);
       } else if (check) {
-        SC_HIP(h, hipMemcpyAsync(h->h_flags, h->flags.p, 16 * sizeof(int), hipMemcpyDeviceToHost, s));
+        if (host_rr)
+          SC_HIP(h, hipMemcpyAsync(h->h_rrpack, h->rrpack.p,
+                                   (kRrTAt + (size_t)m * kLdq) * sizeof(double),
+                                   hipMemcpyDeviceToHost, s));
+        else
+          SC_HIP(h, hipMemcpyAsync(h->h_flags, h->flags.p, 16 * sizeof(int),
+                                   hipMemcpyDeviceToHost, s));
         if (!h->sync_ev) SC_HIP(h, hipEventCreateWithFlags(&h->sync_ev, hipEventDisableTiming));
         SC_HIP(h, hipEventRecord(h->sync_ev, s));
         if (host_rr && cycles == 0 && m >= 6 * kEigBlock && m + kEigBlock <= cap) {
@@ -613,6 +656,7 @@
           } while (!check_due(mm));
         }
         SC_HIP(h, hipEventSynchronize(h->sync_ev));
+        if (host_rr) memcpy(h->h_flags, h->h_rrpack + kRrFlagsAt, 16 * sizeof(int));
         if (h->h_flags[12] != 0) return fail(h, SC_ERR_NON_FINITE, kNonFiniteMessage);
         if (h->h_flags[13] != 0) {
           passes = 0;
@@ -640,13 +684,14 @@
         }
       }
       if (host_rr) {
-        double* hy = h->h_rr + kHostRRSingle * kHostRRSingle + 64;
-        const double* hG = h->h_rr + kHostRRSingle * kHostRRSingle;
+        const double* hT = h->h_rrpack + kRrTAt;
+        const double* hG = h->h_rrpack;
+        double* hy = h->h_rypack + kRyYAt;
         bool rr_ok;
         timespec ts0;
         if (sw::eig_trace()) clock_gettime(CLOCK_MONOTONIC, &ts0);
         if (m <= kHostRR) {
-          rr_ok = host_rayleigh_ritz(h->h_rr, m, hG, m, h->h_theta, h->h_theta + kLdq, hy, m);
+          rr_ok = host_rayleigh_ritz(hT, kLdq, hG, m, h->h_theta, h->h_theta + kLdq, hy, kLdq);
         } else {
           auto leading = [&](const double* theta) {
             std::vector<double> zero(m, 0.0);
@@ -654,8 +699,8 @@
             const int want = d0.enough ? std::max(d0.kw, d0.kvec) : cap / 4;
             return round_up(want + kEigBlock, kEigBlock) + kEigBlock;
           };
-          rr_ok = host_rayleigh_ritz_leading(h->h_rr, m, hG, m, h->h_theta, h->h_theta + kLdq,
-                                             hy, m, leading);
+          rr_ok = host_rayleigh_ritz_leading(hT, kLdq, hG, m, h->h_theta, h->h_theta + kLdq,
+                                             hy, kLdq, leading);
         }
         if (sw::eig_trace()) {
           timespec ts1;
@@ -669,10 +714,9 @@
         }
         for (int i = 0; i < m; ++i)
           if (!std::isfinite(h->h_theta[i])) return fail(h, SC_ERR_NON_FINITE, kNonFiniteMessage);
-        SC_HIP(h, hipMemcpy2DAsync(h->Y.p, (size_t)kLdq * sizeof(double), hy,
-                                   (size_t)m * sizeof(double), (size_t)m * sizeof(double), m,
-                                   hipMemcpyHostToDevice, s));
-        SC_HIP(h, hipMemcpyAsync(theta_d, h->h_theta, m * sizeof(double),
+        memcpy(h->h_rypack, h->h_theta, m * sizeof(double));
+        SC_HIP(h, hipMemcpyAsync(h->rypack.p, h->h_rypack,
+                                 (kRyYAt + (size_t)m * kLdq) * sizeof(double),
                                  hipMemcpyHostToDevice, s));
       }
       if (check) {
@@ -1336,6 +1380,7 @@
   h->krylov_m = 0;
   EigRequest rq = rq_in;
   hipStream_t s = h->stream;
+  SC_TRY(start_block_join(h));
   SC_TRY(ensure_eig(h, n));
   SC_TRY(ensure_gen(h, n));
   double* theta_d = ptr<double>(h->theta);
diff --git a/spectralcluster_amd/csrc/free_api.hip b/spectralcluster_amd/csrc/free_api.hip
--- a/spectralcluster_amd/csrc/free_api.hip
+++ b/spectralcluster_amd/csrc/free_api.hip
@@ -76,8 +76,16 @@
   launch_free_seg_reduce(s, ptr<double>(h->fR), n, free_segs(h));
   return SC_OK;
 }
+int free_flush_ovf(sc_handle h) {
+  if (!h->free_copy_pending) return SC_OK;
+  h->free_copy_pending = false;
+  SC_HIP(h, hipMemcpyAsync(h->h_free, ptr<int>(h->fwords) + 2 * (size_t)h->free_copy_n,
+                           kOvfWords * sizeof(int), hipMemcpyDeviceToHost, h->stream));
+  return SC_OK;
+}
+
 int free_stats_end(sc_handle h, hipStream_t s, const double* A, int ld, int n, bool timed,
-                   const int* plan) {
+                   const int* plan, bool defer_copy) {
   unsigned* M = ptr<unsigned>(h->fwords);
   int* count = ptr<int>(h->fwords) + n;
   int* ovf = ptr<int>(h->fwords) + 2 * (size_t)n;
@@ -88,7 +96,13 @@
                         ptr<double>(h->rowmax), ptr<double>(h->rowsum), ovf);
   if (timed) ev_rec(h, &h->free_ev[4]);
   SC_TRY(check_last(h, "matrix-free diffuse launch"));
-  SC_HIP(h, hipMemcpyAsync(h->h_free, ovf, kOvfWords * sizeof(int), hipMemcpyDeviceToHost, s));
+  h->free_copy_pending = false;
+  if (defer_copy && s == h->stream) {
+    h->free_copy_pending = true;
+    h->free_copy_n = n;
+  } else {
+    SC_HIP(h, hipMemcpyAsync(h->h_free, ovf, kOvfWords * sizeof(int), hipMemcpyDeviceToHost, s));
+  }
   h->free_checked = false;
   return SC_OK;
 }
@@ -133,6 +147,7 @@
     sc_handle h = hs[z];
     SC_HIP(h, hipMemcpyAsync(h->h_free, items[z].words + 2 * (size_t)items[z].n,
                              kOvfWords * sizeof(int), hipMemcpyDeviceToHost, s));
+    h->free_copy_pending = false;
     h->free_checked = false;
   }
   return SC_OK;
@@ -155,10 +170,12 @@
 }
 
 int free_diffuse_stats(sc_handle h, const double* A, int ld, int n, bool have_amax,
-                       bool digits_ready) {
+                       bool digits_ready, int begin_ev) {
   hipStream_t s = h->stream;
+  const int2* tilemap_before = h->tilemap_cur;
   SC_TRY(ensure_tilemap(h, n));
-  ev_rec(h, &h->free_ev[0]);
+  if (begin_ev >= 0 && h->tilemap_cur == tilemap_before) h->free_ev[0] = begin_ev;
+  else ev_rec(h, &h->free_ev[0]);
   if (digits_ready)
     launch_free_partials_reduce(s, ptr<double>(h->fypart), ptr<int>(h->frpart), n,
                                 ptr<double>(h->fy1), ptr<double>(h->fR), ptr<double>(h->fscal),
@@ -168,7 +185,7 @@
   ev_rec(h, &h->free_ev[1]);
   SC_TRY(free_product(h, s, n));
   ev_rec(h, &h->free_ev[2]);
-  return free_stats_end(h, s, A, ld, n, true, ptr<int>(h->fplan));
+  return free_stats_end(h, s, A, ld, n, true, ptr<int>(h->fplan), true);
 }
 
 static void plain_matvec(hipStream_t s, const double* A, int ld, int n, bool sym_mv,
@@ -183,6 +200,7 @@
                       bool* too_many) {
   *changed = *too_many = false;
   hipStream_t s = h->stream;
+  SC_TRY(free_flush_ovf(h));
   SC_HIP(h, hipStreamSynchronize(s));
   h->free_checked = true;
   const int rows = h->h_free[0];
diff --git a/spectralcluster_amd/csrc/handle.h b/spectralcluster_amd/csrc/handle.h
--- a/spectralcluster_amd/csrc/handle.h
+++ b/spectralcluster_amd/csrc/handle.h
@@ -61,6 +61,7 @@
   std::vector<double> blur_ext;
   DevBuf Q, Q2, Vs, W, partial, T, Y, Yt, theta, resid, G, Rinv, Hbuf, hsq, colnorm,
       flags;
+  DevBuf rrpack, rypack;
   DevBuf E, Ek, Eio;
   DevBuf mvsym;
   DevBuf td_d, td_e, td_theta, td_work, td_tau, td_panel;
@@ -69,12 +70,16 @@
   DevBuf crvec, thetai, Vre, Vim, gpart, gsrc, genL, gneg;
   DevBuf ahc_size, ahc_chain, ahc_Z, ahc_lab, ahc_cent;
   DevBuf fb_part, fb_small, fb_x, fb_cent, fb_int;
-  DevBuf kXc, kxsq, kclosest, kcand, kenorm, krnd, kcent, klab32, klab64, kinfo, kchain;
+  DevBuf kXc, kxsq, kclosest, kcand, kenorm, krnd, kcent, klab32, klab64, kchain;
+  long long* h_klab = nullptr;
+  size_t h_klab_count = 0;
   DevBuf kbig, kbigw;
   DevBuf kgen[kKgenBufs];
   double* h_theta = nullptr;
   int* h_flags = nullptr;
   double* h_rr = nullptr;
+  double* h_rrpack = nullptr;
+  double* h_rypack = nullptr;
   std::vector<sc_handle_s*> pool;
   std::vector<sc_handle_s*> gslots;
   std::vector<int> sweep_slot;
@@ -121,9 +126,16 @@
   DevBuf fq2part, fmx64, ftau64, fplan;
   int* h_free = nullptr;
   bool free_checked = false;
+  bool free_copy_pending = false;
+  int free_copy_n = 0;
   int free_ev[5] = {-1, -1, -1, -1, -1};
   int krylov_m = 0, krylov_n = 0, krylov_cycles = 0, krylov_ahead = 0;
   bool krylov_free = false;
+  hipStream_t side_stream = nullptr;
+  hipEvent_t start_ev = nullptr;
+  bool start_pending = false;
+  int start_ready_n = 0;
+  LzChain start_chain;
 };
 
 inline void ev_rec(sc_handle h, int* slot) {
@@ -142,6 +154,10 @@
 }
 
 constexpr int kTilemapTableMax = 64;
+constexpr int kKlabHead = 8;
+constexpr int kRrFlagsAt = 256, kRrArriveAt = 264, kRrTAt = 272, kRyYAt = kLdq;
+constexpr size_t kRrPackDoubles = kRrTAt + (size_t)kLdq * kLdq;
+constexpr size_t kRyPackDoubles = kRyYAt + (size_t)kLdq * kLdq;
 constexpr int kMaxCols = 128;
 inline int matrix_ld(int n) {
   int ld = round_up(n, 16);
@@ -206,6 +222,8 @@
                                int group);
 
 int ensure_eig(sc_handle h, int n);
+int start_block_ahead(sc_handle h, int n);
+int start_block_join(sc_handle h);
 
 int ensure_gen(sc_handle h, int n);
 
@@ -268,11 +286,13 @@
   int laplacian_type = 0;
   bool chain_flags_cleared = false;
   bool skip_fused = false;
+  bool start_ahead = false;
 };
 EigRequest make_eig_request(const sc_config* cfg);
 int upload_blur_weights(sc_handle h, const sc_config* cfg);
 int eig_ncluster_impl(sc_handle h, const sc_config* cfg, sc_diag* diag, FrontResult* front_only,
-                      const FrontResult* resume = nullptr, bool defer_timing = false);
+                      const FrontResult* resume = nullptr, bool defer_timing = false,
+                      int begin_ev = -1);
 void kmeans_seed_constants(int k, double* u_first, int* trials, std::vector<double>* rnd);
 KmeansWorkspace kmeans_workspace(sc_handle h);
 
@@ -308,12 +328,13 @@
 int free_fused_prepare(sc_handle h, hipStream_t s, int n, const double* cut, double p,
                        double floor_value);
 int free_diffuse_stats(sc_handle h, const double* A, int ld, int n, bool have_amax = false,
-                       bool digits_ready = false);
+                       bool digits_ready = false, int begin_ev = -1);
 int ensure_free(sc_handle h, int n);
 int free_product(sc_handle h, hipStream_t s, int n);
 int free_stats_begin(sc_handle h, hipStream_t s, const double* A, int ld, int n, bool have_amax);
 int free_stats_end(sc_handle h, hipStream_t s, const double* A, int ld, int n, bool timed,
-                   const int* plan = nullptr);
+                   const int* plan = nullptr, bool defer_copy = false);
+int free_flush_ovf(sc_handle h);
 int free_fix_overflow(sc_handle h, const double* A, int ld, int n, bool* changed, bool* too_many);
 void free_apply_operator(sc_handle h, const double* A, int ld, int n, bool sym_mv,
                          const double* V, int ldv);
diff --git a/spectralcluster_amd/csrc/kmeans_api.hip b/spectralcluster_amd/csrc/kmeans_api.hip
--- a/spectralcluster_amd/csrc/kmeans_api.hip
+++ b/spectralcluster_amd/csrc/kmeans_api.hip
@@ -21,8 +21,7 @@
     SC_TRY(grow(h, h->kbigw, (size_t)3 * k * sizeof(int)));
   }
   SC_TRY(grow(h, h->klab32, (size_t)n * sizeof(int)));
-  SC_TRY(grow(h, h->klab64, (size_t)n * sizeof(long long)));
-  SC_TRY(grow(h, h->kinfo, 16 * sizeof(int)));
+  SC_TRY(grow(h, h->klab64, (size_t)(kKlabHead + n) * sizeof(long long)));
   SC_TRY(grow(h, h->kchain, kmeans_chain_workspace_doubles(n) * sizeof(double)));
   return SC_OK;
 }
@@ -37,8 +36,8 @@
   ws.rnd = ptr<double>(h->krnd);
   ws.centroids = ptr<double>(h->kcent);
   ws.labels32 = ptr<int>(h->klab32);
-  ws.labels64 = ptr<long long>(h->klab64);
-  ws.info = ptr<int>(h->kinfo);
+  ws.labels64 = ptr<long long>(h->klab64) + kKlabHead;
+  ws.info = ptr<int>(h->klab64);
   ws.chain = ptr<double>(h->kchain);
   ws.big = ptr<double>(h->kbig);
   ws.big_words = ptr<int>(h->kbigw);
@@ -137,18 +136,26 @@
   int info[16] = {0};
   if (metric == kKmeansCosine && kmeans_chain_supported(n, k, trials) &&
       !sw::kmeans_single()) {
+    const size_t need = (size_t)kKlabHead + n;
+    if (h->h_klab_count < need) {
+      if (h->h_klab) SC_HIP(h, hipHostFree(h->h_klab));
+      h->h_klab = nullptr;
+      h->h_klab_count = 0;
+      SC_HIP(h, hipHostMalloc(reinterpret_cast<void**>(&h->h_klab), need * sizeof(long long)));
+      h->h_klab_count = need;
+    }
     for (int it = 0;; it += 4) {
       launch_kmeans_chain(h->stream, E, lde, n, k, max_iter, first, trials, ws, it, 4);
       SC_TRY(check_last(h, "kmeans launch"));
-      SC_HIP(h, hipMemcpyAsync(labels, h->klab64.p, (size_t)n * sizeof(int64_t),
+      SC_HIP(h, hipMemcpyAsync(h->h_klab, h->klab64.p, need * sizeof(long long),
                                hipMemcpyDeviceToHost, h->stream));
-      SC_HIP(h, hipMemcpyAsync(info, h->kinfo.p, 9 * sizeof(int), hipMemcpyDeviceToHost,
-                               h->stream));
       SC_HIP(h, hipStreamSynchronize(h->stream));
+      memcpy(info, h->h_klab, 9 * sizeof(int));
       if (info[8] != 0) break;
       if (it > max_iter + 4)
         return fail(h, SC_ERR_HIP, "k-means chain did not reach its stop rule");
     }
+    memcpy(labels, h->h_klab + kKlabHead, (size_t)n * sizeof(int64_t));
     if (centroids_out) {
       SC_HIP(h, hipMemcpyAsync(centroids_out, h->kcent.p, (size_t)k * k * sizeof(double),
                                hipMemcpyDeviceToHost, h->stream));
@@ -157,12 +164,12 @@
     if (iterations) *iterations = info[0];
     return SC_OK;
   }
-  SC_HIP(h, hipMemsetAsync(h->kinfo.p, 0, 8 * sizeof(int), h->stream));
+  SC_HIP(h, hipMemsetAsync(ws.info, 0, 8 * sizeof(int), h->stream));
   launch_kmeans(h->stream, E, lde, n, k, max_iter, first, trials, ws, metric);
   SC_TRY(check_last(h, "kmeans launch"));
-  SC_HIP(h, hipMemcpyAsync(labels, h->klab64.p, (size_t)n * sizeof(int64_t),
+  SC_HIP(h, hipMemcpyAsync(labels, ws.labels64, (size_t)n * sizeof(int64_t),
                            hipMemcpyDeviceToHost, h->stream));
-  SC_HIP(h, hipMemcpyAsync(info, h->kinfo.p, 6 * sizeof(int), hipMemcpyDeviceToHost,
+  SC_HIP(h, hipMemcpyAsync(info, ws.info, 6 * sizeof(int), hipMemcpyDeviceToHost,
                            h->stream));
   if (centroids_out)
     SC_HIP(h, hipMemcpyAsync(centroids_out, h->kcent.p, (size_t)k * k * sizeof(double),
diff --git a/spectralcluster_amd/csrc/rowops.hip b/spectralcluster_amd/csrc/rowops.hip
--- a/spectralcluster_amd/csrc/rowops.hip
+++ b/spectralcluster_amd/csrc/rowops.hip
@@ -648,8 +648,7 @@
                                                      int lap, int rownorm,
                                                      double* __restrict__ c,
                                                      double* __restrict__ p,
-                                                     double* __restrict__ t) {
-  const int i = blockIdx.x * blockDim.x + threadIdx.x;
+                                                     double* __restrict__ t, int i) {
   if (i >= n) return;
   const double eps = 1e-10;
   const double a = rownorm ? 1.0 / rowmax[i] : 1.0;
@@ -675,11 +674,27 @@
 __global__ void k_scaling_vectors(const double* __restrict__ rowmax,
                                   const double* __restrict__ rowsum, int n,
                                   int lap, int rownorm, double* __restrict__ c,
-                                  double* __restrict__ p, double* __restrict__ t,
-                                  int* __restrict__ flags, int* __restrict__ symflag) {
-  scaling_vectors_body(rowmax, rowsum, n, lap, rownorm, c, p, t);
-  if (flags != nullptr && blockIdx.x == 0 && threadIdx.x == 0) {
-    flags[12] = symflag != nullptr ? symflag[1] : 0;
+                                  double* __restrict__ p, double* __restrict__ t) {
+  scaling_vectors_body(rowmax, rowsum, n, lap, rownorm, c, p, t,
+                       blockIdx.x * blockDim.x + threadIdx.x);
+}
+__global__ __launch_bounds__(256) void k_scaling_vectors_flags(
+    const double* __restrict__ rowmax, const double* __restrict__ rowsum, int n, int lap,
+    int rownorm, double* __restrict__ c, double* __restrict__ p, double* __restrict__ t,
+    int* __restrict__ flags, const int* __restrict__ symflag, int clear_chain,
+    int* __restrict__ arrive) {
+  const int i = blockIdx.x * 256 + threadIdx.x;
+  scaling_vectors_body(rowmax, rowsum, n, lap, rownorm, c, p, t, i);
+  const int bad = __syncthreads_or(i < n && (!isfinite(c[i]) || !isfinite(p[i])) ? 1 : 0);
+  if (threadIdx.x != 0) return;
+  if (bad) atomicOr(&arrive[1], 1);
+  __threadfence();
+  if (atomicAdd(&arrive[0], 1) != (int)gridDim.x - 1) return;
+  __threadfence();
+  const int any_bad = atomicExch(&arrive[1], 0);
+  atomicExch(&arrive[0], 0);
+  flags[12] = any_bad ? 1 : (symflag != nullptr ? symflag[1] : 0);
+  if (clear_chain) {
     flags[13] = 0;
     flags[14] = 0;
     flags[15] = 0;
@@ -689,7 +704,7 @@
   const FrontItem& a = g.s[blockIdx.y];
   const int i = blockIdx.x * blockDim.x + threadIdx.x;
   if (i >= a.n) return;
-  scaling_vectors_body(a.rowmax, a.rowsum, a.n, lap, rownorm, a.cvec, a.pvec, a.tvec);
+  scaling_vectors_body(a.rowmax, a.rowsum, a.n, lap, rownorm, a.cvec, a.pvec, a.tvec, i);
   if (!isfinite(a.cvec[i]) || !isfinite(a.pvec[i]) ||
       (i == 0 && a.symflag != nullptr && a.symflag[1] != 0))
     a.flags[12] = 1;
@@ -846,9 +861,14 @@
 void launch_scaling_vectors(hipStream_t s, const double* rowmax,
                             const double* rowsum, int n, int laplacian_type,
                             int row_normalized, double* c, double* p, double* t, int* flags,
-                            int* symflag) {
-  hipLaunchKernelGGL(k_scaling_vectors, dim3((n + 255) / 256), dim3(256), 0, s,
-                     rowmax, rowsum, n, laplacian_type, row_normalized, c, p, t, flags, symflag);
+                            int* symflag, bool clear_chain, int* arrive) {
+  if (flags != nullptr)
+    hipLaunchKernelGGL(k_scaling_vectors_flags, dim3((n + 255) / 256), dim3(256), 0, s, rowmax,
+                       rowsum, n, laplacian_type, row_normalized, c, p, t, flags, symflag,
+                       clear_chain ? 1 : 0, arrive);
+  else
+    hipLaunchKernelGGL(k_scaling_vectors, dim3((n + 255) / 256), dim3(256), 0, s,
+                       rowmax, rowsum, n, laplacian_type, row_normalized, c, p, t);
 }
 static GroupOf<FrontItem> front_pack(const FrontItem* items, int count, int* nmax) {
   GroupOf<FrontItem> g;
diff --git a/spectralcluster_amd/csrc/sc_internal.h b/spectralcluster_amd/csrc/sc_internal.h
--- a/spectralcluster_amd/csrc/sc_internal.h
+++ b/spectralcluster_amd/csrc/sc_internal.h
@@ -140,7 +140,8 @@
 void launch_scaling_vectors(hipStream_t s, const double* rowmax,
                             const double* rowsum, int n, int laplacian_type,
                             int row_normalized, double* c, double* p, double* t,
-                            int* flags = nullptr, int* symflag = nullptr);
+                            int* flags = nullptr, int* symflag = nullptr,
+                            bool clear_chain = true, int* arrive = nullptr);
 void launch_laplacian(hipStream_t s, const double* in, double* out, int n, int ld,
                       int laplacian_type, double* deg_ws);
 void launch_check_finite(hipStream_t s, const double* a, const double* b, int n, int* flag);
```

Measured after the change: 400.7 calls/s, median of 6. 1.02x the previous value.
